# openai/robogym

Hardware: AMD Instinct MI355X
Metric: env-steps/sec (whole node) dactyl/locked batch 8192; qpos L∞ vs MuJoCo (as restated by the in-repo CPU oracle: parity unpinned) (higher is better)
Workload: dtype f32

## Files before the change

### include/rgstep.h

```cpp
#ifndef RGSTEP_H
#define RGSTEP_H
#include <stddef.h>
#include <stdint.h>

#ifdef __cplusplus
extern "C" {
#endif

typedef struct rg_model rg_model;
typedef struct rg_batch rg_batch;

enum {
  RG_F_QPOS = 0,
  RG_F_QVEL = 1,
  RG_F_CTRL = 2,
  RG_F_PID = 3,
  RG_F_WARMSTART = 4,
  RG_F_TIME = 5,
  RG_F_STATUS = 6,
  RG_F_STATS = 7,
  RG_F_DEBUG = 8,
  RG_F_COST = 9,
  RG_F_PAIRLB = 10,
  RG_F_ENVPRM = 11
// ... 58 lines not shown
  float* qpos_goal;
  int* preticks;
  float* reward;
  unsigned char *done, *goal_reset, *trial_success, *sub_goal_ok, *env_crash, *resetting, *episode_started;
  int* info_ssl;
  int *nticks_next, *reset_mask, *live_mask;
  float* goal_dist_before;
  float* packed;
  const float* draws;
  const float* goal_override;
  unsigned seed, step;
  const float* parallel_quats;
  const float* qpos0;
  const float* zero_ctrl;
  const float* ctrl_lo, *ctrl_hi;
  float success_threshold, success_reward, wiggle_std, cube_body_z;
  int max_timesteps_per_goal, successes_needed, use_goal_distance_reward;
  int pipelined, reset_initial_steps, n_random_initial_steps, max_pose_resets;
  int cube_pos_col, cube_quat_col;
  int stop_on_fall;
} rg_post_args;
int rg_env_post_step(rg_batch* b, const rg_post_args* args, void* stream);
int rg_post_args_size(void);
#define RG_WRAP_U_POOL 32
#define RG_WRAP_N_POOL 128
enum {
  RG_WK_CUBE_POS, RG_WK_CUBE_QUAT, RG_WK_QPOS, RG_WK_QVEL, RG_WK_HAND_ANGLE, RG_WK_FINGERTIP_POS, RG_WK_GOAL_POS, RG_WK_GOAL_QUAT, RG_WK_QPOS_GOAL,
  RG_WK_IS_GOAL_ACHIEVED, RG_WK_FELL_DOWN, RG_WK_ACTION_HISTORY, RG_WK_ACTION_DELAY, RG_WK_DELTA, RG_WK_NOISY_CUBE_POS, RG_WK_NOISY_CUBE_QUAT,
  RG_WK_NOISY_FINGERTIP_POS, RG_WK_NOISY_HAND_ANGLE, RG_WK_ACTION_EMA, RG_WK_ACH_POS, RG_WK_REL_POS, RG_WK_NACH_POS, RG_WK_NREL_POS, RG_WK_ACH_QUAT,
  RG_WK_REL_QUAT, RG_WK_NACH_QUAT, RG_WK_NREL_QUAT, RG_WK_RELATIVE_GOAL, RG_WK_NOISY_RELATIVE_GOAL, RG_WK_ACHIEVED_GOAL, RG_WK_NOISY_ACHIEVED_GOAL,
  RG_WK_GOAL, RG_WK_PREVIOUS_ACTION, RG_WK_REWARD, RG_WK_COUNT
};
typedef struct rg_wrap_dims {
  int nq, nv, nu, nh, ntip;
  int ndelta;
  int randomize, relative_goal;
} rg_wrap_dims;
typedef struct rg_wrap_lay {
  int fwidth, iwidth, W;
  int s_prev, s_ema, s_alpha, s_aema, s_hist, s_slack, s_cdown, s_cup, s_anmult, s_anadd, s_addb, s_mulb, s_ts, s_wind, s_occl, s_ffbuf, s_ffleft, s_cfleft, s_cfbuf, s_delta;
  int i_emat, i_steps, i_drops, i_first, i_delay;
  int n_action, n_wind, n_noise[4];
  int u_ts, u_wind, u_axis, u_ff, u_cf;
  int key[RG_WK_COUNT];
} rg_wrap_lay;
typedef struct rg_wrap_args {
  int B, device;
  rg_wrap_dims dims;
  rg_wrap_lay lay;
  float* fstate; int* istate;
  const float *u, *n, *e;
  const long long* action_index;
  const float* bins; int nbins;
  float* action_out;
  const float* qpos; int qpos_stride;
  const int* hand_q;
  const float* pos_to_ctrl;
  float* prm; int prm_stride;
  int p_ctrlrange, p_timestep, p_xfrc_cube, p_mass_cube;
  int relative_action, nsubsteps, fixed_wrist, wrist_act, wrist_qadr;
  float wrist_lo, wrist_hi;
  const float* obs; int obs_stride;
  const float *goal_pos, *goal_quat, *qpos_goal;
  const int* is_goal_achieved;
  const float* contact; int contact_stride, ncon_slots;
  const float* ncon; int ncon_stride;
  const float* env_reward;
  const unsigned char* env_done;
  const int* successes_so_far;
  float *out, *reward_out;
  unsigned char *done_out, *fell_out;
  int* info_out;
  float occ_geom[5]; int n_occ;
  float timestep0, cube_body_z, fall_z, occ_cutoff, ff_p, cf_p, freeze_scale, drop_reward, clip;
  int min_episode_length;
  float unc[4];
} rg_wrap_args;
int rg_wrap_layout(const rg_wrap_dims* dims, rg_wrap_lay* lay);
int rg_wrap_pre_step(const rg_wrap_args* args, void* stream);
int rg_wrap_post_step(const rg_wrap_args* args, void* stream);
int rg_wrap_args_size(void);
int rg_batch_set_constants(rg_batch* b, const int* mask_dev, void* stream);
int rg_batch_mpr_pair(rg_batch* b, int g1, int g2, float margin, float* out_dev, void* stream);
int rg_batch_items_info(const rg_batch* b, int* slots, int* queues);
int rg_obs_dim(const rg_batch* b);
int rg_debug_size(void);
int rg_lds_bytes(void);
int rg_lds_bytes_cfg(int config);
typedef struct rb_model rb_model;
typedef struct rb_batch rb_batch;
rb_model* rb_model_create(const void* blob, size_t nbytes, char* err, int errlen);
rb_model* rb_compile_mjcf(const char* xml, const char* meshdir, char* err, int errlen);
int rb_model_enable_env_params(rb_model* m);
int rb_prm_layout(const rb_model* m, int* out, int n);
int rb_model_blob_keys(const rb_model* m, char* out, int outlen);
void rb_model_free(rb_model* m);
int rb_model_info(const rb_model* m, int* out, int n);
int rb_scratch_offset(const rb_model* m, int which);
rb_batch* rb_batch_create(const rb_model* m, int B);
void rb_batch_free(rb_batch* b);
int rb_batch_reset(rb_batch* b);
int rb_batch_set_env(rb_batch* b, int hand_qposadr, int n_hand_jnt, int relative_action, const float* pos_to_ctrl);
int rb_batch_set_action_limits(rb_batch* b, float max_position_change, unsigned ctrl_centre_mask);
void* rb_batch_field_ptr(rb_batch* b, int field, int* row_words);
int rb_batch_step(rb_batch* b, const float* action_dev, const int* active_dev, int nsubsteps, int nforward_ticks, int flags, void* stream);
int rb_batch_step_ex(rb_batch* b, const float* action_dev, const int* active_dev, const int* hold_dev, const int* nticks_dev, int nsubsteps, int nforward_ticks, int flags, void* stream);
enum {
  RB_F_MOCAP = 12,
  RB_F_EQ_DATA = 13,
  RB_F_EQ_ACTIVE = 14,
  RB_F_SENSORDATA = 15
};
typedef struct rb_tcp_args {
  int arm_qposadr[6], main_arm_qposadr[6];
  int main_gripper_actuator, tcp_body, wrist_joint, reset_controller_error;
  float max_position_change, speed_roll, speed_pitch, joint_drift_threshold, gripper_ctrl_lo, gripper_ctrl_hi;
  const int* action_index; const float* bins; int nbins; float ema_alpha;
  float* ema_value; int* ema_t; float* action_out;
  const int* hold; const float* scripted;
  int wrist_only;
  int self_world, nforward_ticks;
  const int* nticks; const int* skip;
} rb_tcp_args;
int rb_batch_step_tcp(rb_batch* solver, rb_batch* main, const float* action_dev, const int* active_dev , const rb_tcp_args* args, int nsubsteps, int flags, void* stream);
int rb_tcp_args_size(void);
int rb_multi_begin(void);
int rb_multi_launch(void* stream);
#define RA_MAXOBJ 16
typedef struct ra_post_args {
  float* obs; int obs_dim;
  int num_objects;
  int *t, *steps, *steps_since_last_goal, *successes_so_far, *consecutive;
  float* prev_nsucc; int* prev_valid;
  const float* goal;
  const float* goal_rot;
  const float* qpos_goal;
  const float* static_obs;
  float* reward;
  float* goal_dist;
  unsigned char *done, *goal_reset, *trial_success, *sub_goal_ok, *env_crash, *objects_off_table;
  int* info_ssl;
  int obj_body[RA_MAXOBJ], tcp_body, arm_qposadr[6], grip_qposadr, grip_dofadr, grip_act, finger_geom[2], table_plane_geom, force_adr, torque_adr;
  unsigned long long gripper_geom_mask;
  float table_min[2], table_max[2], table_height, pos_threshold, rot_threshold, goal_pos_offset, goal_rot_weight, goal_reward_per_object, success_reward,
      penalty_table_collision, penalty_objects_off_table, penalty_safety_stop, safety_stop_force;
  int max_timesteps_per_goal, successes_needed, use_goal_distance_reward;
  float *solver_qpos, *solver_ctrl;
  int solver_nq, solver_nu, solver_grip_qposadr, solver_grip_act;
  const unsigned char* frozen;
  float reward_clip;
  int goal_kind;
  int grip_site;
  float* goal_dist_extra;
  const int* obj_group;
  const float *parallel_quats, *parallel_quats_180;
  int rot_dist_type;
} ra_post_args;
int ra_env_post_step(rb_batch* main, rb_batch* solver, const ra_post_args* args, void* stream);
int ra_post_args_size(void);
typedef struct ra_recipe_args {
  int num_objects, action_dim;
  int *stage, *left;
  float* yaw;
  const unsigned char *done, *goal_reset;
  int *hold, *hold_ctrl, *solver_active, *nticks;
  float* scripted;
// ... 75 lines not shown
```

### robogym_amd/_native.py

```python
import ctypes
import os

import numpy as np

_HERE = os.path.dirname(os.path.abspath(__file__))
LIB_PATH = os.environ.get("RGSTEP_LIB") or os.path.join(_HERE, "csrc", "librgstep.so")

RG_F_QPOS, RG_F_QVEL, RG_F_CTRL, RG_F_PID, RG_F_WARMSTART, RG_F_TIME, RG_F_STATUS, RG_F_STATS, RG_F_DEBUG, RG_F_COST, RG_F_PAIRLB, RG_F_ENVPRM = range(12)
RB_F_MOCAP, RB_F_EQ_DATA, RB_F_EQ_ACTIVE, RB_F_SENSORDATA = 12, 13, 14, 15
RG_STATUS_BAD_STATE, RG_STATUS_CON_FULL, RG_STATUS_CAND_FULL, RG_STATUS_ROW_FULL, RG_STATUS_BAD_FACTOR, RG_STATUS_BAD_ACTION = 1, 2, 4, 8, 16, 32


class StepArgs(ctypes.Structure):

    _fields_ = [("action_dev", ctypes.c_void_p), ("goal_quat_dev", ctypes.c_void_p), ("obs_dev", ctypes.c_void_p), ("goal_dist_dev", ctypes.c_void_p),
                ("active_dev", ctypes.c_void_p), ("hold_dev", ctypes.c_void_p), ("nticks_dev", ctypes.c_void_p), ("order_dev", ctypes.c_void_p),
                ("nsubsteps", ctypes.c_int), ("nforward_ticks", ctypes.c_int), ("flags", ctypes.c_int), ("stream", ctypes.c_void_p),
                ("config", ctypes.c_int), ("redo_dev", ctypes.c_void_p), ("preticks_dev", ctypes.c_void_p), ("xdata_dev", ctypes.c_void_p)]


RG_CFG_ROLLOUT, RG_CFG_LARGE = 0, 1
RG_POST_NDRAW = 2 + 4 + 3 + 20


# ... 50 lines not shown
def _ra_post_fields():
    _p, _i, _f = ctypes.c_void_p, ctypes.c_int, ctypes.c_float
    return ([("obs", _p), ("obs_dim", _i), ("num_objects", _i)]
            + [(n, _p) for n in ("t", "steps", "steps_since_last_goal", "successes_so_far", "consecutive", "prev_nsucc", "prev_valid", "goal", "goal_rot", "qpos_goal", "static_obs",
                                 "reward", "goal_dist", "done", "goal_reset", "trial_success", "sub_goal_ok", "env_crash", "objects_off_table", "info_ssl")]
            + [("obj_body", _i * RA_MAXOBJ), ("tcp_body", _i), ("arm_qposadr", _i * 6), ("grip_qposadr", _i), ("grip_dofadr", _i), ("grip_act", _i), ("finger_geom", _i * 2),
               ("table_plane_geom", _i), ("force_adr", _i), ("torque_adr", _i), ("gripper_geom_mask", ctypes.c_ulonglong), ("table_min", _f * 2), ("table_max", _f * 2)]
            + [(n, _f) for n in ("table_height", "pos_threshold", "rot_threshold", "goal_pos_offset", "goal_rot_weight", "goal_reward_per_object", "success_reward",
                                 "penalty_table_collision", "penalty_objects_off_table", "penalty_safety_stop", "safety_stop_force")]
            + [(n, _i) for n in ("max_timesteps_per_goal", "successes_needed", "use_goal_distance_reward")]
            + [("solver_qpos", _p), ("solver_ctrl", _p), ("solver_nq", _i), ("solver_nu", _i), ("solver_grip_qposadr", _i), ("solver_grip_act", _i), ("frozen", _p), ("reward_clip", _f)]
            + [("goal_kind", _i), ("grip_site", _i), ("goal_dist_extra", _p)]
            + [("obj_group", _p)]
            + [("parallel_quats", _p), ("parallel_quats_180", _p), ("rot_dist_type", _i)])


class RaPostArgs(ctypes.Structure):

    _fields_ = _ra_post_fields()


def _ra_recipe_fields():
    _p, _i, _f = ctypes.c_void_p, ctypes.c_int, ctypes.c_float
    return ([("num_objects", _i), ("action_dim", _i)]
            + [(n, _p) for n in ("stage", "left", "yaw", "done", "goal_reset", "hold", "hold_ctrl", "solver_active", "nticks", "scripted", "frozen", "resetting", "episode_started",
                                 "reobserve", "ended", "stabilised", "placement_failed", "t", "steps", "steps_since_last_goal", "successes_so_far", "consecutive", "prev_valid",
                                 "ema_t", "ema_value", "action_ema", "goal", "goal_rot", "qpos_goal", "static_obs")]
            + [("obj_qposadr", _i * RA_MAXOBJ), ("arm_qposadr", _i * 6), ("solver_arm_qposadr", _i * 6), ("arm_start", _f * 6), ("obj_center", (_f * 3) * RA_MAXOBJ),
               ("obj_half", (_f * 3) * RA_MAXOBJ), ("area_offset", _f * 2), ("area_size", _f * 2), ("table_pos", _f * 3), ("table_size", _f * 3), ("stabilize_steps", _i),
               ("n_random_initial_steps", _i), ("settle_steps", _i), ("seed", ctypes.c_uint), ("step", ctypes.c_uint)]
            + [("goal_kind", _i), ("height_range", _f * 2), ("object_size", _f), ("fixed_order", _i), ("target_height", _f), ("det_points", (_f * 3) * 2), ("goal_index", _p)]
            + [("obj_group", _p), ("group_mode", _i), ("sample_lam", _f * 2)]
            + [("goal_distance_ratio", _p), ("goal_distance_min", _f), ("pickup_proba", _f), ("stacking_proba", _f)]
            + [("randomize_goal_rot", _i), ("domino_distance_mul", _f)]
            + [("fixed_xy", (_f * 2) * RA_MAXOBJ), ("fixed_yaw", _f * RA_MAXOBJ)])


class RaRecipeArgs(ctypes.Structure):

    _fields_ = _ra_recipe_fields()


RG_WRAP_U_POOL, RG_WRAP_N_POOL = 32, 128
RG_WRAP_KEYS = ["cube_pos", "cube_quat", "qpos", "qvel", "hand_angle", "fingertip_pos", "goal_pos", "goal_quat", "qpos_goal", "is_goal_achieved", "fell_down", "action_history",
                "action_delay", "_delta", "noisy_cube_pos", "noisy_cube_quat", "noisy_fingertip_pos", "noisy_hand_angle", "action_ema", "achieved_goal_pos", "relative_goal_pos",
                "noisy_achieved_goal_pos", "noisy_relative_goal_pos", "achieved_goal_quat", "relative_goal_quat", "noisy_achieved_goal_quat", "noisy_relative_goal_quat",
                "relative_goal", "noisy_relative_goal", "achieved_goal", "noisy_achieved_goal", "goal", "previous_action", "reward"]


class WrapDims(ctypes.Structure):

    _fields_ = [(n, ctypes.c_int) for n in ("nq", "nv", "nu", "nh", "ntip", "ndelta", "randomize", "relative_goal")]


class WrapLay(ctypes.Structure):

    _fields_ = ([(n, ctypes.c_int) for n in ("fwidth", "iwidth", "W", "s_prev", "s_ema", "s_alpha", "s_aema", "s_hist", "s_slack", "s_cdown", "s_cup", "s_anmult", "s_anadd", "s_addb",
                                             "s_mulb", "s_ts", "s_wind", "s_occl", "s_ffbuf", "s_ffleft", "s_cfleft", "s_cfbuf", "s_delta", "i_emat", "i_steps", "i_drops", "i_first",
                                             "i_delay", "n_action", "n_wind")]
                + [("n_noise", ctypes.c_int * 4)] + [(n, ctypes.c_int) for n in ("u_ts", "u_wind", "u_axis", "u_ff", "u_cf")] + [("key", ctypes.c_int * len(RG_WRAP_KEYS))])


def _wrap_fields():
    p_, i_, f_ = ctypes.c_void_p, ctypes.c_int, ctypes.c_float
    return ([("B", i_), ("device", i_), ("dims", WrapDims), ("lay", WrapLay), ("fstate", p_), ("istate", p_), ("u", p_), ("n", p_), ("e", p_),
             ("action_index", p_), ("bins", p_), ("nbins", i_), ("action_out", p_), ("qpos", p_), ("qpos_stride", i_), ("hand_q", p_), ("pos_to_ctrl", p_),
             ("prm", p_), ("prm_stride", i_)]
            + [(n, i_) for n in ("p_ctrlrange", "p_timestep", "p_xfrc_cube", "p_mass_cube", "relative_action", "nsubsteps", "fixed_wrist", "wrist_act", "wrist_qadr")]
            + [("wrist_lo", f_), ("wrist_hi", f_), ("obs", p_), ("obs_stride", i_), ("goal_pos", p_), ("goal_quat", p_), ("qpos_goal", p_), ("is_goal_achieved", p_),
               ("contact", p_), ("contact_stride", i_), ("ncon_slots", i_), ("ncon", p_), ("ncon_stride", i_), ("env_reward", p_), ("env_done", p_), ("successes_so_far", p_),
               ("out", p_), ("reward_out", p_), ("done_out", p_), ("fell_out", p_), ("info_out", p_), ("occ_geom", f_ * 5), ("n_occ", i_)]
            + [(n, f_) for n in ("timestep0", "cube_body_z", "fall_z", "occ_cutoff", "ff_p", "cf_p", "freeze_scale", "drop_reward", "clip")]
            + [("min_episode_length", i_), ("unc", f_ * 4)])


class WrapArgs(ctypes.Structure):

    _fields_ = _wrap_fields()


EXPORTS = [
    "rg_model_create", "rg_model_free", "rg_model_dims", "rg_batch_create", "rg_batch_free", "rg_batch_set_env",
    "rg_batch_copy", "rg_batch_reset", "rg_batch_step", "rg_obs_dim", "rg_debug_size", "rg_lds_bytes", "rg_sync",
    "rg_last_error", "rg_batch_mpr_pair", "rg_batch_copy_rows", "rg_batch_step_ex", "rg_batch_field_ptr", "rg_model_create_on", "rg_model_npair",
    "rg_lds_bytes_cfg", "rg_env_post_step", "rg_post_args_size", "rg_batch_enable_env_params", "rg_prm_layout", "rg_xdata_layout", "rg_batch_set_constants", "rg_batch_items_info",
    "rb_model_create", "rb_model_free", "rb_model_info", "rb_scratch_offset", "rb_batch_create", "rb_batch_free", "rb_batch_reset", "rb_batch_set_env",
    "rb_batch_field_ptr", "rb_batch_step", "rb_batch_step_ex", "rb_env_post_step", "rb_post_args_size", "rb_cube_ops", "rb_batch_step_tcp", "ra_env_post_step", "ra_post_args_size",
    "rg_blob_entry", "rg_model_blob_keys", "rb_model_blob_keys", "rg_compile_mjcf", "rb_compile_mjcf", "rg_compile_mjcf_blob", "rg_blob_free",
    "rb_model_enable_env_params", "rb_prm_layout", "rb_batch_set_action_limits", "ra_env_recipe_step", "ra_recipe_args_size", "rb_tcp_args_size", "rb_multi_begin", "rb_multi_launch",
    "rg_wrap_layout", "rg_wrap_pre_step", "rg_wrap_post_step", "rg_wrap_args_size",
]
EXPORTS_SETCONST = ["rb_batch_set_constants"]



class NativeError(RuntimeError):
    pass


def bind(path):
    if not os.path.exists(path):
        raise NativeError(
            "%s not found: build it with `python -c 'import __graft_entry__ as g; g.build()'` "
            "(hipcc --offload-arch=gfx950). There is no CPU fallback." % path
        )
    L = ctypes.CDLL(path)
    vp, ci, cf = ctypes.c_void_p, ctypes.c_int, ctypes.c_float
    L.rg_model_create.restype = vp
    L.rg_model_create.argtypes = [ctypes.c_char_p, ctypes.c_size_t, ctypes.c_char_p, ci]
    L.rg_model_free.argtypes = [vp]
    L.rg_model_create_on.restype = vp
    L.rg_model_create_on.argtypes = [ctypes.c_char_p, ctypes.c_size_t, ci, ctypes.c_char_p, ci]
    L.rg_model_npair.argtypes = [vp]
    L.rg_batch_step_ex.argtypes = [vp, ctypes.POINTER(StepArgs)]
    L.rg_batch_field_ptr.restype = vp
    L.rg_batch_field_ptr.argtypes = [vp, ci, ctypes.POINTER(ci)]
    L.rg_model_dims.argtypes = [vp, ctypes.POINTER(ci)]
    L.rg_batch_create.restype = vp
    L.rg_batch_create.argtypes = [vp, ci, ci]
    L.rg_batch_free.argtypes = [vp]
    L.rg_batch_set_env.argtypes = [vp, ctypes.POINTER(ci), ci, ctypes.POINTER(cf), cf]
    L.rg_batch_copy.argtypes = [vp, ci, vp, ci, ci]
    L.rg_batch_reset.argtypes = [vp]
    L.rg_batch_copy_rows.argtypes = [vp, ci, vp, vp, ci, ci, vp]
    L.rg_batch_step.argtypes = [vp, vp, vp, vp, vp, vp, ci, ci, ci, vp]
    L.rg_batch_mpr_pair.argtypes = [vp, ci, ci, cf, vp, vp]
    L.rg_obs_dim.argtypes = [vp]
    L.rg_debug_size.restype = ci
    L.rg_lds_bytes.restype = ci
    L.rg_lds_bytes_cfg.restype = ci
    L.rg_lds_bytes_cfg.argtypes = [ci]
    L.rg_batch_enable_env_params.argtypes = [vp]
    L.rg_prm_layout.argtypes = [ctypes.POINTER(ci), ci]
    L.rg_xdata_layout.argtypes = [ctypes.POINTER(ci), ci]
    L.rg_env_post_step.argtypes = [vp, ctypes.POINTER(PostArgs), vp]
    L.rg_post_args_size.restype = ci
    if L.rg_post_args_size() != ctypes.sizeof(PostArgs):
        raise NativeError("rg_post_args layout mismatch between include/rgstep.h and robogym_amd/_native.py")
    L.rg_wrap_layout.argtypes = [ctypes.POINTER(WrapDims), ctypes.POINTER(WrapLay)]
    L.rg_wrap_pre_step.argtypes = [ctypes.POINTER(WrapArgs), vp]
    L.rg_wrap_post_step.argtypes = [ctypes.POINTER(WrapArgs), vp]
    L.rg_wrap_args_size.restype = ci
    if L.rg_wrap_args_size() != ctypes.sizeof(WrapArgs):
        raise NativeError("rg_wrap_args layout mismatch between include/rgstep.h and robogym_amd/_native.py")
    L.rg_batch_set_constants.argtypes = [vp, vp, vp]
    L.rg_batch_items_info.argtypes = [vp, ctypes.POINTER(ci), ctypes.POINTER(ci)]
    L.rb_model_create.restype = vp
    L.rb_model_create.argtypes = [ctypes.c_char_p, ctypes.c_size_t, ctypes.c_char_p, ci]
    L.rb_model_free.argtypes = [vp]
    L.rb_model_info.argtypes = [vp, ctypes.POINTER(ci), ci]
    L.rg_blob_entry.argtypes = [ctypes.c_char_p, ctypes.c_size_t, ci, ctypes.c_char_p, ctypes.POINTER(ci), ctypes.POINTER(ctypes.c_uint)]
    L.rg_model_blob_keys.argtypes = [vp, ctypes.c_char_p, ci]
    L.rb_model_blob_keys.argtypes = [vp, ctypes.c_char_p, ci]
    L.rg_compile_mjcf.restype = vp
    L.rg_compile_mjcf.argtypes = [ctypes.c_char_p, ctypes.c_char_p, ctypes.c_char_p, ci]
    L.rb_compile_mjcf.restype = vp
    L.rb_compile_mjcf.argtypes = [ctypes.c_char_p, ctypes.c_char_p, ctypes.c_char_p, ci]
    L.rg_compile_mjcf_blob.argtypes = [ctypes.c_char_p, ctypes.c_char_p, ci, ctypes.POINTER(vp), ctypes.POINTER(ctypes.c_size_t), ctypes.c_char_p, ci]
    L.rg_blob_free.argtypes = [vp]
    L.rb_model_enable_env_params.argtypes = [vp]
    L.rb_prm_layout.argtypes = [vp, ctypes.POINTER(ci), ci]
    L.rb_scratch_offset.argtypes = [vp, ci]
    L.rb_batch_create.restype = vp
    L.rb_batch_create.argtypes = [vp, ci]
    L.rb_batch_free.argtypes = [vp]
    L.rb_batch_reset.argtypes = [vp]
    L.rb_batch_set_env.argtypes = [vp, ci, ci, ci, ctypes.POINTER(cf)]
    L.rb_batch_set_action_limits.argtypes = [vp, cf, ctypes.c_uint]
    L.rb_batch_field_ptr.restype = vp
    L.rb_batch_field_ptr.argtypes = [vp, ci, ctypes.POINTER(ci)]
    L.rb_batch_step.argtypes = [vp, vp, vp, ci, ci, ci, vp]
    L.rb_batch_step_ex.argtypes = [vp, vp, vp, vp, vp, ci, ci, ci, vp]
    L.rb_batch_step_tcp.argtypes = [vp, vp, vp, vp, ctypes.POINTER(RbTcpArgs), ci, ci, vp]
    L.rb_multi_launch.argtypes = [vp]
    L.rb_batch_set_constants.argtypes = [vp, vp, vp]
    L.rb_tcp_args_size.restype = ci
    if L.rb_tcp_args_size() != ctypes.sizeof(RbTcpArgs):
        raise NativeError("rb_tcp_args layout mismatch between include/rgstep.h and robogym_amd/_native.py")
    L.ra_env_post_step.argtypes = [vp, vp, ctypes.POINTER(RaPostArgs), vp]
    L.ra_post_args_size.restype = ci
    if L.ra_post_args_size() != ctypes.sizeof(RaPostArgs):
        raise NativeError("ra_post_args layout mismatch between include/rgstep.h and robogym_amd/_native.py")
    L.ra_env_recipe_step.argtypes = [vp, vp, ctypes.POINTER(RaRecipeArgs), vp]
    L.ra_recipe_args_size.restype = ci
    if L.ra_recipe_args_size() != ctypes.sizeof(RaRecipeArgs):
        raise NativeError("ra_recipe_args layout mismatch between include/rgstep.h and robogym_amd/_native.py")
    L.rb_env_post_step.argtypes = [vp, ctypes.POINTER(RbPostArgs), vp]
    L.rb_post_args_size.restype = ci
    if L.rb_post_args_size() != ctypes.sizeof(RbPostArgs):
        raise NativeError("rb_post_args layout mismatch between include/rgstep.h and robogym_amd/_native.py")
    L.rb_cube_ops.argtypes = [vp, ci, vp, vp, ci, vp, vp]
    L.rg_sync.argtypes = [vp]
    L.rg_last_error.restype = ctypes.c_char_p
    return L


_LIB = None


def lib():
    global _LIB
    if _LIB is None:
        _LIB = bind(LIB_PATH)
    return _LIB


def check(L, rc, what):
    if rc != 0:
        raise NativeError("%s failed: %s" % (what, L.rg_last_error().decode()))


RG_FLAG_MPR_PLANE_DEPTH = 16
RG_FLAG_SENSORS = 32
RG_FLAG_SEPARATE_FORWARD_SUBSTITUTION = 64
RG_FLAG_SUBSTEP_ITEMS = 128
RG_FLAG_CAPACITY_TEST_HOOK = 512
RG_FLAG_DESERT_QUEUE0 = 1024
RG_STATUS_SCHED = 64
RG_FLAG_RESUME = 256

RB_PRM_NAMES = ["gravity", "dof_damping", "dof_armature", "dof_frictionloss", "dof_invweight0", "jnt_stiffness", "jnt_margin", "jnt_range", "body_pos", "body_mass", "body_inertia",
                "body_invweight0", "actuator_gainprm", "actuator_forcerange", "actuator_ctrlrange", "geom_pos", "geom_margin", "geom_gap", "geom_friction", "geom_solref", "geom_solimp",
                "tendon_range", "tendon_invweight0", "timestep", "xfrc_applied", "site_pos", "geom_scale"]
PRM_NAMES = ["row", "gravity", "timestep", "dof_damping", "dof_armature", "dof_frictionloss", "dof_invweight0", "body_mass", "body_inertia", "body_invweight0",
             "jnt_range", "tendon_range", "tendon_invweight0", "actuator_gainprm", "actuator_ctrlrange", "actuator_forcerange", "geom_friction", "xfrc_applied", "site_pos", "geom_scale", "jnt_margin", "geom_solref", "geom_solimp"]


def prm_layout(L):
    buf = (ctypes.c_int * 32)()
    n = L.rg_prm_layout(buf, 32)
    assert n == len(PRM_NAMES), "rg_prm_layout and robogym_amd/_native.py disagree"
    return {k: int(buf[i]) for i, k in enumerate(PRM_NAMES)}
```

### robogym_amd/csrc/rb_kernel.h

```cpp
#include "rb_types.h"
#if !defined(RB_NS) || !defined(RB_T) || !defined(RB_MAXGROUP) || !defined(RB_MAXNV) || !defined(RB_MAXNQ)
#error "rb_kernel.h: define RB_NS, RB_T, RB_MAXGROUP, RB_MAXNV, RB_MAXNQ before including"
#endif
#ifndef RB_MAXNU
#define RB_MAXNU 32
#endif

namespace RB_NS {
using namespace rgl;

#ifdef RG_EMUL
typedef const RbModelDev& RbM;
typedef const RbLaunch& RbLRef;
#define RB_S() (*(RbLds*)emul_lds())
#else
typedef const RG_AS4 RbModelDev& RbM;
typedef const RG_AS4 RbLaunch& RbLRef;
#define RB_S() (*(RbLds*)rg_lds_raw)
#endif
#define TID ((int)threadIdx.x)
#define WID (TID >> 6)
#define WL (TID & 63)
#define BFOR(i, n) for (int i = TID; i < (n); i += RB_T)
#define BSYNC() __syncthreads()
// ... 1152 lines not shown
  if (!m.prm_on) { for (int k = 0; k < 12; k++) out[k] = m.b_pair_prm[12 * p + k]; return; }
  const int a = m.b_pair_geom[3 * p], b = m.b_pair_geom[3 * p + 1];
  const float *gm = S + m.prm_off[RB_P_GEOM_MARGIN], *gg = S + m.prm_off[RB_P_GEOM_GAP], *gf = S + m.prm_off[RB_P_GEOM_FRICTION];
  const float *gr = S + m.prm_off[RB_P_GEOM_SOLREF], *gi = S + m.prm_off[RB_P_GEOM_SOLIMP];
  out[0] = fmaxf(gm[a], gm[b]); out[1] = fmaxf(gg[a], gg[b]);
  for (int k = 0; k < 3; k++) out[2 + k] = fmaxf(gf[3 * a + k], gf[3 * b + k]);
  const float m1 = m.geom_solmix[a], m2 = m.geom_solmix[b];
  const float mix = (m1 >= 1e-15f && m2 >= 1e-15f) ? m1 / (m1 + m2) : ((m1 < 1e-15f && m2 < 1e-15f) ? 0.5f : (m1 < 1e-15f ? 0.f : 1.f));
  if (gr[2 * a] > 0.f && gr[2 * b] > 0.f) { out[5] = mix * gr[2 * a] + (1.f - mix) * gr[2 * b]; out[6] = mix * gr[2 * a + 1] + (1.f - mix) * gr[2 * b + 1]; }
  else { out[5] = fminf(gr[2 * a], gr[2 * b]); out[6] = fminf(gr[2 * a + 1], gr[2 * b + 1]); }
  for (int k = 0; k < 5; k++) out[7 + k] = mix * gi[5 * a + k] + (1.f - mix) * gi[5 * b + k];
}
__device__ __forceinline__ void rb_broadphase(RbM m, RbLds& s, float* S, int flags) {
  int* cand = (int*)SC(CAND);
  const float *gpos = SC(GPOS), *gquat = SC(GQUAT);
  if (TID == 0) { s.ncand = 0; s.ncand2 = 0; s.ncon = s.neqcon; }
  BSYNC();
  const bool multipoint = !(flags & 16);
  const bool obb = !(flags & 2048);
  const int halfcand = m.maxcand >> 1;
  for (int base = 0; base < m.npair; base += RB_T) {
    const int p = base + TID;
    bool keep = false, special = false;
    if (p < m.npair) {
      const int g1 = m.b_pair_geom[3 * p], g2 = m.b_pair_geom[3 * p + 1], t1 = m.geom_type[g1];
      const float margin = rb_pair_margin(m, S, p);
      const v3 P1 = ld3(gpos + 3 * g1), P2 = ld3(gpos + 3 * g2), dif = P2 - P1;
      const float* bb = m.b_geom_aabb + 6 * g2;
      const float s1 = rb_geom_scale(m, s, g1), s2 = rb_geom_scale(m, s, g2);
      if (t1 == RG_GEOM_PLANE) {
        const v3 pn = qrot(ldq(gquat + 4 * g1), mk3(0, 0, 1));
        keep = dot(dif, pn) <= m.geom_rbound[g2] * s2 + margin;
        if (keep && obb) {
          const q4 q2 = ldq(gquat + 4 * g2);
          const v3 c2 = dif + qrot(q2, ld3(bb) * s2), nl = qrotT(q2, pn);
          keep = dot(c2, pn) - s2 * (bb[3] * fabsf(nl.x) + bb[4] * fabsf(nl.y) + bb[5] * fabsf(nl.z)) <= margin + 1e-5f;
        }
      } else {
        const float bound = m.geom_rbound[g1] * s1 + m.geom_rbound[g2] * s2 + margin;
        keep = dot(dif, dif) <= bound * bound;
        if (keep && obb) {
          const float* ba = m.b_geom_aabb + 6 * g1;
          const q4 q1 = ldq(gquat + 4 * g1), q2 = ldq(gquat + 4 * g2);
          keep = !rb_obb_apart(qrot(q1, ld3(ba) * s1), q1, ld3(ba + 3) * s1, dif + qrot(q2, ld3(bb) * s2), q2, ld3(bb + 3) * s2, margin);
        }
      }
      special = multipoint && m.geom_type[g2] == RG_GEOM_BOX && (t1 == RG_GEOM_BOX || t1 == RG_GEOM_PLANE);
    }
    const int slot = rb_slot(s, keep && !special, &s.ncand, halfcand, RG_STATUS_CAND_FULL);
    if (slot >= 0) cand[slot] = p;
    const int slot2 = rb_slot(s, keep && special, &s.ncand2, halfcand, RG_STATUS_CAND_FULL);
    if (slot2 >= 0) cand[m.maxcand - 1 - slot2] = p;
  }
  BSYNC();
}
__device__ __forceinline__ void rb_narrow_convex(RbM m, RbLds& s, float* S, int flags) {
  const int* cand = (const int*)SC(CAND);
  const float *gpos = SC(GPOS), *gquat = SC(GQUAT);
  const bool multipoint = !(flags & 16);
  (void)multipoint;
  MprEnv E; E.mesh_vert = m.b_mesh_rec; E.cell_adr = m.b_cell_adr; E.cell_blk = (const rgf4*)m.b_cell_blk; E.cell_ovf = (const rgf4*)m.b_cell_ovf; E.prof = 0; E.cells = !(flags & 8); E.plane_depth = (flags & 16) != 0;
  const int ncand = s.ncand;
  float* con = SC(CON);
  for (int base = 0; base < ncand; base += RB_T / 4) {
    const int ci = base + (TID >> 2);
    const bool active = ci < ncand;
    bool hit = false; float dist = 0; v3 pos = mk3(0, 0, 0), nrm = mk3(0, 0, 1); int p = 0;
    MprGeom A, B; A.type = RG_GEOM_SPHERE; B.type = RG_GEOM_SPHERE; A.quat = B.quat = gquat; A.size = B.size = mk3(0, 0, 0); A.pos = B.pos = mk3(0, 0, 0);
    A.margin = B.margin = 0; A.mesh = B.mesh = -1; A.vertadr = B.vertadr = 0; A.nvert = B.nvert = 0;
    float margin = 0;
    v3 p1 = mk3(0, 0, 0);
    bool plane = false; const bool special = false;
    if (active) {
      p = cand[ci];
      const int g1 = m.b_pair_geom[3 * p], g2 = m.b_pair_geom[3 * p + 1];
      margin = rb_pair_margin(m, S, p);
      rb_geom(m, s, S, g1, A); rb_geom(m, s, S, g2, B);
      p1 = ld3(gpos + 3 * g1);
      A.pos = mk3(0, 0, 0); B.pos = ld3(gpos + 3 * g2) - p1;
      plane = A.type == RG_GEOM_PLANE;
      A.margin = B.margin = plane ? 0.f : 0.5f * margin;
    }
    v3 sep, dir = mk3(0, 0, 0); float depth = 0;
    const bool mh = rg_mpr<4>(E, A, B, m.mpr_iterations, m.mpr_tolerance, depth, dir, pos, sep, active && !plane && !special);
    if (active && !plane && !special) {
      hit = mh && dot(dir, dir) > 0.25f;
      dist = margin - depth; nrm = normalized(dir); pos = pos + p1;
    }
    const v3 pn = qrot(ldq(A.quat), mk3(0, 0, 1));
    MprGeom Bs = B;
    if (!(active && plane && !special)) { Bs.type = RG_GEOM_SPHERE; Bs.mesh = -1; Bs.size = mk3(0, 0, 0); }
    const v3 sp = rg_support<4>(E, Bs, (active && plane && !special) ? pn * -1.0f : mk3(0, 0, 1));
    if (active && plane && !special) {
      dist = dot(sp, pn);
      hit = dist <= margin;
      pos = sp + p1 - pn * (0.5f * dist); nrm = pn;
    }
    const int slot = rb_slot(s, hit && (TID & 3) == 0, &s.ncon, m.maxcon, RG_STATUS_CON_FULL);
    if (slot >= 0) {
      float* c = con + RB_CONREC * slot;
      float pr[12]; rb_pair_prm(m, S, p, pr);
      c[RB_CR_DIST] = dist; st3(c + RB_CR_POS, pos);
      float fr[9]; fr[0] = nrm.x; fr[1] = nrm.y; fr[2] = nrm.z; rb_make_frame(fr);
      for (int k = 0; k < 9; k++) c[RB_CR_FRAME + k] = fr[k];
      c[RB_CR_INCL] = pr[0] - pr[1];
      c[RB_CR_FRIC] = pr[2]; c[RB_CR_FRIC + 1] = pr[2]; c[RB_CR_FRIC + 2] = pr[3]; c[RB_CR_FRIC + 3] = pr[4]; c[RB_CR_FRIC + 4] = pr[4];
      c[RB_CR_SOLREF] = pr[5]; c[RB_CR_SOLREF + 1] = pr[6];
      for (int k = 0; k < 5; k++) c[RB_CR_SOLIMP + k] = pr[7 + k];
      c[RB_CR_DIM] = (float)m.b_pair_geom[3 * p + 2]; c[RB_CR_G1] = (float)m.b_pair_geom[3 * p]; c[RB_CR_G2] = (float)m.b_pair_geom[3 * p + 1];
      c[RB_CR_ADR] = -1.f; c[RB_CR_NNZ] = 0.f; c[RB_CR_KIND] = (float)((m.cone == 1 && m.b_pair_geom[3 * p + 2] > 1) ? RB_KIND_ELLIPTIC : RB_KIND_PYRAMID);
    }
  }
  BSYNC();
}
__device__ __forceinline__ void rb_narrow_box(RbM m, RbLds& s, float* S, int flags) {
  const int* cand = (const int*)SC(CAND);
  const float *gpos = SC(GPOS), *gquat = SC(GQUAT);
  float* con = SC(CON);
  const bool multipoint = !(flags & 16);
  if (multipoint) {
    const int ncand2 = s.ncand2;
    for (int base = 0; base < ncand2; base += RB_T / 32) {
      const int ci = base + (TID >> 5), l = TID & 31;
      bool hit = false, planebox = false; float dist = 0; v3 pos = mk3(0, 0, 0), nrm = mk3(0, 0, 1); int p = 0;
      if (ci < ncand2) {
        p = cand[m.maxcand - 1 - ci];
        const int g1 = m.b_pair_geom[3 * p], g2 = m.b_pair_geom[3 * p + 1], t1 = m.geom_type[g1];
        if (m.geom_type[g2] == RG_GEOM_BOX && (t1 == RG_GEOM_BOX || t1 == RG_GEOM_PLANE)) {
          const float margin = rb_pair_margin(m, S, p);
          const v3 P1 = ld3(gpos + 3 * g1), t = ld3(gpos + 3 * g2) - P1;
          const float s2 = rb_geom_scale(m, s, g2);
          if (t1 == RG_GEOM_BOX) {
            const float s1 = rb_geom_scale(m, s, g1);
            const float A[3] = {m.geom_size[3 * g1] * s1, m.geom_size[3 * g1 + 1] * s1, m.geom_size[3 * g1 + 2] * s1}, B[3] = {m.geom_size[3 * g2] * s2, m.geom_size[3 * g2 + 1] * s2, m.geom_size[3 * g2 + 2] * s2};
            hit = box_box_lane(A, B, ldq(gquat + 4 * g1), ldq(gquat + 4 * g2), P1, t, margin, l, dist, pos, nrm);
          } else {
            nrm = qrot(ldq(gquat + 4 * g1), mk3(0, 0, 1));
            hit = rb_plane_box_lane(nrm, t, ldq(gquat + 4 * g2), ld3(m.geom_size + 3 * g2) * s2, margin, l, dist, pos);
            pos = pos + P1; planebox = true;
          }
        }
      }
      const unsigned long long balpb = __ballot(hit && planebox);
      if (hit && planebox && __popc((unsigned)((balpb >> (TID & 32)) & 0xffull) & ((1u << l) - 1u)) >= 4) hit = false;
      const int slot = rb_slot(s, hit, &s.ncon, m.maxcon, RG_STATUS_CON_FULL);
      if (slot >= 0) {
        float* c = con + RB_CONREC * slot;
        float pr[12]; rb_pair_prm(m, S, p, pr);
        c[RB_CR_DIST] = dist; st3(c + RB_CR_POS, pos);
        const v3 nn = normalized(nrm);
        float fr[9]; fr[0] = nn.x; fr[1] = nn.y; fr[2] = nn.z; rb_make_frame(fr);
        for (int k = 0; k < 9; k++) c[RB_CR_FRAME + k] = fr[k];
        c[RB_CR_INCL] = pr[0] - pr[1];
        c[RB_CR_FRIC] = pr[2]; c[RB_CR_FRIC + 1] = pr[2]; c[RB_CR_FRIC + 2] = pr[3]; c[RB_CR_FRIC + 3] = pr[4]; c[RB_CR_FRIC + 4] = pr[4];
        c[RB_CR_SOLREF] = pr[5]; c[RB_CR_SOLREF + 1] = pr[6];
        for (int k = 0; k < 5; k++) c[RB_CR_SOLIMP + k] = pr[7 + k];
        c[RB_CR_DIM] = (float)m.b_pair_geom[3 * p + 2]; c[RB_CR_G1] = (float)m.b_pair_geom[3 * p]; c[RB_CR_G2] = (float)m.b_pair_geom[3 * p + 1];
        c[RB_CR_ADR] = -1.f; c[RB_CR_NNZ] = 0.f; c[RB_CR_KIND] = (float)((m.cone == 1 && m.b_pair_geom[3 * p + 2] > 1) ? RB_KIND_ELLIPTIC : RB_KIND_PYRAMID);
      }
    }
  }
  BSYNC();
}

__device__ __forceinline__ float rb_impedance(const float* si, float pos, float margin) { return impedance(si, pos, margin); }
__device__ __forceinline__ void rb_KB(float timestep, const float* solref, const float* solimp, float& K, float& B) {
  const float dmax = clampf(solimp[1], 1e-4f, 0.9999f);
  if (solref[0] > 0) {
    const float tc = fmaxf(solref[0], 2.f * timestep), dr = solref[1];
    K = 1.f / fmaxf(RB_MINVAL, dmax * dmax * tc * tc * dr * dr); B = 2.f / fmaxf(RB_MINVAL, dmax * tc);
  } else { K = -solref[0] / fmaxf(RB_MINVAL, dmax * dmax); B = -solref[1] / fmaxf(RB_MINVAL, dmax); }
}
__device__ __forceinline__ int rb_npyr(int dim) { return dim == 1 ? 1 : 2 * (dim - 1); }
__device__ __forceinline__ int rb_nrows(int kind, int dim) { return kind == RB_KIND_PYRAMID ? rb_npyr(dim) : dim; }
__device__ __forceinline__ float rb_srow_dot(RbM m, const float* S, int type, int id, float aux, const float* x) {
// ... 1404 lines not shown
```

### robogym_amd/csrc/rb_types.h

```cpp
#pragma once
#include <stdint.h>

#define RB_T_LARGE 256
#define RB_MAXGROUP_LARGE 96
#define RB_MAXNV_LARGE 192
#define RB_MAXNQ_LARGE 192
#define RB_T_SMALL 64
#define RB_MAXGROUP_SMALL 40
#define RB_MAXNV_SMALL 40
#define RB_MAXNQ_SMALL 48
#define RB_T_MEDIUM 64
#define RB_MAXGROUP_MEDIUM 56
#define RB_MAXNV_MEDIUM 56
#define RB_MAXNQ_MEDIUM 64
#define RB_TENW 8
#define RB_CONW 24
#define RB_STARB 5
#define RB_MLONG 8
#define RB_NW 22

#define RB_INT_ARRAYS(X) \
  X(body_parentid) X(body_rootid) X(body_weldid) X(body_jntadr) X(body_jntnum) X(body_dofadr) X(body_dofnum) \
  X(jnt_type) X(jnt_qposadr) X(jnt_dofadr) X(jnt_bodyid) \
  X(dof_bodyid) X(dof_jntid) X(dof_parentid) \
  X(geom_type) X(geom_bodyid) X(geom_dataid) X(site_bodyid) \
  X(mesh_vertadr) X(mesh_vertnum) \
  X(tendon_adr) X(tendon_num) X(wrap_type) X(wrap_objid) \
  X(actuator_trntype) X(actuator_trnid) X(actuator_forcelimited) X(actuator_biastype) \
  X(body_mocapid) X(eq_type) X(eq_obj1id) X(eq_obj2id) X(sensor_type) X(sensor_objid) X(sensor_adr) \
  X(b_lvl_body) X(b_lvl_adr) X(b_body_level) X(b_body_lastdof) X(b_subtree_adr) X(b_subtree) X(b_root_list) X(b_M_i) X(b_M_j) X(b_M_adr) \
  X(b_group_adr) X(b_group_dofs) X(b_dof_group) X(b_dof_local) X(b_pair_geom) X(b_ten_dofs) X(b_fric_dof) X(b_fric_ten) X(b_lim_jnt) X(b_lim_ten) X(b_cell_adr) X(b_Mdesc_adr) X(b_Mdesc_ent) X(b_Mdesc_dof) X(b_dof_fricrow) X(b_star_grp) X(b_tree_adr) X(b_tree_desc) X(b_tree_branch) X(b_tree_brn_end) X(b_Mlong) X(b_tree8)
#define RB_FLT_ARRAYS(X) \
  X(body_pos) X(body_quat) X(body_ipos) X(body_iquat) X(body_mass) X(body_inertia) X(body_subtreemass) X(body_invweight0) \
  X(jnt_pos) X(jnt_axis) X(jnt_stiffness) X(jnt_range) X(jnt_margin) X(jnt_solref) X(jnt_solimp) \
  X(dof_armature) X(dof_damping) X(dof_frictionloss) X(dof_solref) X(dof_solimp) X(dof_invweight0) \
  X(qpos0) X(qpos_spring) \
  X(geom_size) X(geom_rbound) X(geom_pos) X(geom_quat) X(site_pos) \
  X(wrap_prm) X(tendon_range) X(tendon_margin) X(tendon_stiffness) X(tendon_damping) X(tendon_frictionloss) X(tendon_lengthspring) \
  X(tendon_solref_lim) X(tendon_solimp_lim) X(tendon_solref_fri) X(tendon_solimp_fri) X(tendon_invweight0) \
  X(actuator_gear) X(actuator_ctrlrange) X(actuator_forcerange) X(actuator_gainprm) X(actuator_user) \
  X(eq_solref) X(eq_solimp) X(site_quat) \
  X(geom_margin) X(geom_gap) X(geom_friction) X(geom_solref) X(geom_solimp) X(geom_solmix) X(opt_gravity) \
  X(b_pair_prm) X(b_geom_aabb) X(b_mesh_rec) X(b_cell_blk) X(b_cell_ovf)

enum {
  RB_O_XPOS, RB_O_XQUAT, RB_O_XIPOS, RB_O_XIQUAT, RB_O_XANCHOR, RB_O_XAXIS, RB_O_GPOS, RB_O_GQUAT, RB_O_SPOS, RB_O_ROOTCOM,
  RB_O_CINERT, RB_O_CRB, RB_O_CDOF, RB_O_CDOFDOT, RB_O_CVEL, RB_O_CACC, RB_O_CFRC,
  RB_O_TENLEN, RB_O_TENJ, RB_O_TENVEL, RB_O_MSP,
  RB_O_CAND, RB_O_CON, RB_O_CONJ, RB_O_CONIDX, RB_O_ROW, RB_O_DOFCON_ADR, RB_O_DOFCON, RB_O_CONF,
  RB_O_DBG, RB_O_CFRCEXT, RB_O_CONLOC, RB_O_PRM, RB_NOFF
};
enum {
  RB_P_GRAVITY, RB_P_DOF_DAMPING, RB_P_DOF_ARMATURE, RB_P_DOF_FRICTIONLOSS, RB_P_DOF_INVWEIGHT0, RB_P_JNT_STIFFNESS, RB_P_JNT_MARGIN, RB_P_JNT_RANGE,
  RB_P_BODY_POS, RB_P_BODY_MASS, RB_P_BODY_INERTIA, RB_P_BODY_INVWEIGHT0, RB_P_ACT_GAINPRM, RB_P_ACT_FORCERANGE, RB_P_ACT_CTRLRANGE,
  RB_P_GEOM_POS, RB_P_GEOM_MARGIN, RB_P_GEOM_GAP, RB_P_GEOM_FRICTION, RB_P_GEOM_SOLREF, RB_P_GEOM_SOLIMP, RB_P_TENDON_RANGE, RB_P_TENDON_INVWEIGHT0,
  RB_P_TIMESTEP, RB_P_XFRC, RB_P_SITE_POS, RB_P_GEOM_SCALE, RB_NPRMF
};
#define RB_CONREC 32
#define RB_CR_KIND 31
#define RB_KIND_PYRAMID 0
#define RB_KIND_ELLIPTIC 1
#define RB_KIND_EQUALITY 2
#define RB_CR_DIST 0
#define RB_CR_POS 1
#define RB_CR_FRAME 4
#define RB_CR_INCL 13
#define RB_CR_FRIC 14
#define RB_CR_SOLREF 19
#define RB_CR_SOLIMP 21
#define RB_CR_DIM 26
#define RB_CR_G1 27
#define RB_CR_G2 28
#define RB_CR_ADR 29
#define RB_CR_NNZ 30
#define RB_ROWREC 12
#define RB_RR_FORCE 8
#define RB_RR_ZONE 9
#define RB_RR_COST 10
#define RB_RR_D 0
#define RB_RR_AREF 1
#define RB_RR_JAR 2
#define RB_RR_JV 3
#define RB_RR_FLOSS 4
#define RB_RR_TYPE 5
#define RB_RR_ID 6
#define RB_RR_AUX 7

struct RbModelDev {
  int nq, nv, nu, nbody, njnt, ngeom, nsite, ntendon, nmesh;
  int nlevel, nM, npair, ngroup, gmax, nroot, conw;
  int nfric_dof, nfric_ten, nlim_jnt, nlim_ten;
  int maxcon, maxrow, maxcand;
  int iterations, mpr_iterations, ls_iterations;
  int cone, neq, nmocap, nsensor, nsensordata;
  float timestep, gravity[3], tolerance, impratio, mpr_tolerance, meaninertia;
  int off[RB_NOFF];
  int scratch_words;
  int prm_on;
  int prm_off[RB_NPRMF];
  int prm_words;
  const int* b_geom_scaled;
// ... 53 lines not shown
```

### robogym_amd/csrc/rg_api.hip

```cpp
#include "../../include/rgstep.h"
typedef rg_post_args RgPostArgs;
typedef rb_post_args RbPostArgs;
typedef ra_post_args RaPostArgs;
typedef ra_recipe_args RaRecipeArgs;
#define RG_NS rgs
#define RG_MAXCON 24
#define RG_CPOOL 768
#define RG_MAXCAND 128
#define RG_MAXCAND2 64
#include "rg_kernel.h"
#undef RG_NS
#undef RG_MAXCON
#undef RG_CPOOL
#undef RG_MAXCAND
#undef RG_MAXCAND2
#define RG_NS rgl
#define RG_SETCONST 1
#define RG_MAXCON 64
#define RG_CPOOL 2048
#define RG_MAXCAND 256
#define RG_MAXCAND2 128
#include "rg_kernel.h"
#undef RG_NS
#undef RG_MAXCON
// ... 287 lines not shown
    std::vector<float> rec((lb.size() ? lb.size() : 1) * RG_KINREC, 0.f);
    for (size_t k = 0; k < lb.size(); k++) {
      int b = lb[k], j = jn[b] > 0 ? ja[b] : 0, t = jn[b] > 0 ? jt[j] : 0, qa = jn[b] > 0 ? jq[j] : 0;
      float* r = rec.data() + k * RG_KINREC;
      int w0 = b | (par[b] << 8) | (jn[b] << 16) | (t << 20), w1 = j | (qa << 16);
      memcpy(r, &w0, 4); memcpy(r + 1, &w1, 4);
      for (int c = 0; c < 3; c++) { r[2 + c] = bp[3 * b + c]; r[9 + c] = bi[3 * b + c]; r[12 + c] = jn[b] > 0 ? jp[3 * j + c] : 0.f; r[15 + c] = jn[b] > 0 ? jx[3 * j + c] : 0.f; }
      for (int c = 0; c < 4; c++) r[5 + c] = bq[4 * b + c];
      r[18] = jn[b] > 0 ? q0[qa] : 0.f;
    }
    {
      static_assert(RG_MAXDEPTH <= 8 && RG_MAXBODY <= 256, "body chain: 8 bytes per body");
      std::vector<int> slot(d.nbody, -1), depth(d.nbody, 0), chainw((size_t)(d.nbody ? d.nbody : 1) * 2, 0);
      for (size_t k = 0; k < lb.size(); k++) if (lb[k] >= 0 && lb[k] < d.nbody) slot[lb[k]] = (int)k;
      std::vector<float> brec((size_t)(d.nbody ? d.nbody : 1) * RG_KINREC, 0.f);
      for (int b0 = 0; b0 < d.nbody; b0++) {
        if (slot[b0] < 0) continue;
        memcpy(brec.data() + (size_t)b0 * RG_KINREC, rec.data() + (size_t)slot[b0] * RG_KINREC, RG_KINREC * 4);
        int chain[RG_MAXDEPTH + 1], n = 0, a0 = b0;
        for (; a0 > 0 && slot[a0] >= 0; a0 = par[a0]) { if (n >= RG_MAXDEPTH) return bail("kinematic chain deeper than RG_MAXDEPTH", m); chain[n++] = a0; }
        unsigned long long cw = 0; int absmask = 0;
        for (int i = 0; i < n; i++) {
          int a = chain[n - 1 - i];
          cw |= (unsigned long long)(a & 255) << (8 * i);
          for (int jj = 0; jj < jn[a]; jj++) if (jt[ja[a] + jj] == RG_JNT_FREE) absmask |= 1 << i;
        }
        depth[b0] = n | (absmask << 8) | ((a0 & 255) << 16);
        chainw[2 * b0] = (int)(unsigned)(cw & 0xFFFFFFFFull); chainw[2 * b0 + 1] = (int)(unsigned)(cw >> 32);
      }
      if (!upload<float>(m, brec, &d.body_rec) || !upload<int>(m, depth, &d.body_depth) || !upload<int>(m, chainw, &d.body_chain)) return bail("hipMalloc failed", m);
    }
    {
      std::vector<int> os, rid, rob; std::vector<float> roc;
      if (!get_i(B, "k_body_orgslot", os, e) || !get_i(B, "body_rootid", rid, e) || !get_i(B, "k_root_origin_body", rob, e) || !get_f(B, "k_root_origin_const", roc, e)) return bail(e, m);
      std::vector<float> orec(16, 0.f);
      for (int sl = 0; sl < 4; sl++) { int unused = -2; memcpy(&orec[4 * sl], &unused, 4); }
      for (int b0 = 0; b0 < d.nbody; b0++) {
        int sl = os[b0], r = rid[b0], ob = rob[r];
        if (sl < 0 || sl > 3) return bail("com-frame slot out of range", m);
        memcpy(&orec[4 * sl], &ob, 4);
        for (int c = 0; c < 3; c++) orec[4 * sl + 1 + c] = ob >= 0 ? bi[3 * ob + c] : roc[3 * r + c];
      }
      if (!upload<float>(m, orec, &d.org_rec)) return bail("hipMalloc failed", m);
    }
  }
  UPI(lvl_dof, "k_lvl_dof"); UPI(lvl_dof_adr, "k_lvl_dof_adr"); UPI(M_i, "k_M_i"); UPI(M_j, "k_M_j"); { std::vector<int> mi0, mj0, db0; if (!get_i(B, "k_M_i", mi0, e) || !get_i(B, "k_M_j", mj0, e) || !get_i(B, "dof_bodyid", db0, e)) return bail(e, m); std::vector<int> w(mi0.size() ? mi0.size() : 1, 0); for (size_t q = 0; q < mi0.size(); q++) w[q] = mi0[q] | (mj0[q] << 8) | (db0[mi0[q]] << 16); if (!upload<int>(m, w, &d.M_ijb)) return bail("hipMalloc failed", m); }    UPI(M_lvl_adr, "k_M_lvl_adr");
  UPI(desc_adr, "k_desc_adr"); UPI(desc, "k_desc");
  {
    std::vector<int> mi, mj, blk, d2c;
    if (!get_i(B, "k_M_i", mi, e) || !get_i(B, "k_M_j", mj, e) || !get_i(B, "k_dof_blk", blk, e) || !get_i(B, "k_d2c", d2c, e)) return bail(e, m);
    if ((int)mi.size() > RG_MAXNM || mi.size() != mj.size()) return bail("inertia matrix has more non-zeros than RG_MAXNM", m);
    std::vector<int> ent(2 * (mi.size() ? mi.size() : 1), 0);
    for (size_t k = 0; k < mi.size(); k++) {
      int i = mi[k], j = mj[k], s0 = (blk[i] >> 16) & 255;
      int aij = (blk[i] & 0xFFFF) + (j - s0), aji = (blk[j] & 0xFFFF) + (i - s0);
      if (aij >= RG_HWORDS || aji >= RG_HWORDS || aij < 0 || aji < 0) return bail("inertia block layout exceeds RG_HWORDS", m);
      ent[2 * k] = aij | (aji << 16);
      ent[2 * k + 1] = (d2c[i] >= 0 && d2c[j] >= 0) ? (d2c[i] | (d2c[j] << 8) | (1 << 16)) : 0;
    }
    if (!upload<int>(m, ent, &d.M_ent)) return bail("hipMalloc failed", m);
  }
  UPI(geom_type, "geom_type"); UPI(geom_bodyid, "geom_bodyid"); UPI(geom_dataid, "geom_dataid"); UPI(body_geomadr, "body_geomadr"); UPI(body_geomnum, "body_geomnum");
  UPF(geom_size, "geom_size"); UPF(geom_rbound, "geom_rbound"); UPF(geom_pos, "geom_pos"); UPF(geom_quat, "geom_quat"); UPF(geom_aabb, "k_geom_aabb");
  UPI(site_bodyid, "site_bodyid"); UPF(site_pos, "site_pos");
  UPI(site_type, "site_type"); UPF(site_size, "site_size"); UPF(site_quat, "site_quat");
  { std::vector<int> st, so, sty;
    if (!get_i(B, "sensor_type", st, e) || !get_i(B, "sensor_objid", so, e) || !get_i(B, "site_type", sty, e)) return bail(e, m);
    if (st.size() > RG_MAXSENSOR) return bail("more than RG_MAXSENSOR sensors", m);
    for (size_t k = 0; k < st.size(); k++) {
      if (st[k] != 0) return bail("only touch sensors are implemented", m);
      int t = sty[so[k]];
      if (t != RG_GEOM_SPHERE && t != RG_GEOM_CAPSULE && t != RG_GEOM_ELLIPSOID && t != RG_GEOM_CYLINDER && t != RG_GEOM_BOX) return bail("touch sensor on a site of unsupported shape", m);
    }
    d.nsensor = (int)st.size();
    if (so.empty()) so.push_back(0);
    if (!upload<int>(m, so, &d.sensor_site)) return bail("hipMalloc failed", m); }
  UPI(mesh_vertadr, "mesh_vertadr"); UPI(mesh_vertnum, "mesh_vertnum");
  { GF("mesh_vert"); std::vector<float> v4(fv.size() / 3 * 4, 0.f);
    for (size_t i = 0; i < fv.size() / 3; i++) { v4[4 * i] = fv[3 * i]; v4[4 * i + 1] = fv[3 * i + 1]; v4[4 * i + 2] = fv[3 * i + 2]; }
    if (!upload<float>(m, v4, &d.mesh_vert)) return bail("hipMalloc failed", m);
    std::vector<int> vadr, cadr, vidx;
    if (!get_i(B, "mesh_vertadr", vadr, e) || !get_i(B, "k_mesh_cell_adr", cadr, e) || !get_i(B, "k_mesh_cell_vidx", vidx, e)) return bail(e, m);
    if (cadr.size() != (size_t)d.nmesh * RG_NCELL) return bail("k_mesh_cell_adr has the wrong size (RG_CELLN mismatch?)", m);
    std::vector<float> blk((size_t)d.nmesh * RG_NCELL * 16, 0.f), ovf(4, 0.f);
    for (int mi = 0; mi < d.nmesh; mi++) for (int c = 0; c < RG_NCELL; c++) {
      size_t ce = (size_t)mi * RG_NCELL + c;
      int e = cadr[ce], start = e >> 8, cnt = e & 255;
      if (cnt < 1 || (size_t)(start + cnt) > vidx.size()) return bail("bad support cell", m);
      cadr[ce] = (int)((ovf.size() / 4) << 8) | cnt;
      for (int k = 0; k < (cnt > 4 ? cnt : 4); k++) {
        int vi = vidx[start + (k < cnt ? k : cnt - 1)]; size_t src = (size_t)(vadr[mi] + vi);
        if (vi < 0 || src * 3 + 2 >= fv.size()) return bail("bad support cell vertex", m);
        float o[4] = {fv[3 * src], fv[3 * src + 1], fv[3 * src + 2], 0.f}; memcpy(o + 3, &vi, 4);
        if (k < 4) memcpy(blk.data() + ce * 16 + 4 * k, o, 16); else ovf.insert(ovf.end(), o, o + 4);
      }
    }
    if (!upload<int>(m, cadr, &d.mesh_cell_adr) || !upload<float>(m, blk, &d.mesh_cell_blk) || !upload<float>(m, ovf, &d.mesh_cell_ovf)) return bail("hipMalloc failed", m); }
  UPI(pair_geom, "k_pair_geom"); UPF(pair_prm, "k_pair_prm"); UPF(pair_mix, "k_pair_mix");
  {
    std::vector<int> pg, gt, gd, va, vn, gb, bdm; std::vector<float> pp, gs, gr, ga;
    if (!get_i(B, "geom_bodyid", gb, e) || !get_i(B, "k_body_dofmask", bdm, e)) return bail(e, m);
    if (!get_i(B, "k_pair_geom", pg, e) || !get_i(B, "geom_type", gt, e) || !get_i(B, "geom_dataid", gd, e) || !get_i(B, "mesh_vertadr", va, e) || !get_i(B, "mesh_vertnum", vn, e) ||
        !get_f(B, "k_pair_prm", pp, e) || !get_f(B, "geom_size", gs, e) || !get_f(B, "geom_rbound", gr, e) || !get_f(B, "k_geom_aabb", ga, e)) return bail(e, m);
    std::vector<int> gsc;
    if (B.find("k_geom_scaled") && !get_i(B, "k_geom_scaled", gsc, e)) return bail(e, m);
    for (size_t g = 0; g < gsc.size(); g++) if (gsc[g] && (g >= gt.size() || gt[g] != RG_GEOM_BOX)) return bail("k_geom_scaled flags a geom that is not a box", m);
    size_t np = pg.size() / 3;
    std::vector<int> gg(np ? np : 1, 0); std::vector<float> rec((np ? np : 1) * RG_PAIRREC, 0.f);
    for (size_t p = 0; p < np; p++) {
      int g[2] = {pg[3 * p], pg[3 * p + 1]};
      if (g[0] < 0 || g[1] < 0 || g[0] > 255 || g[1] > 255 || g[0] >= d.ngeom || g[1] >= d.ngeom) return bail("pair geom id out of range", m);
      gg[p] = g[0] | (g[1] << 8);
      float* r = rec.data() + p * RG_PAIRREC;
      int hdr = g[0] | (g[1] << 8) | (pg[3 * p + 2] << 16) | (gt[g[0]] << 20) | (gt[g[1]] << 24);
      if ((size_t)g[0] < gsc.size() && gsc[g[0]]) hdr |= RG_PAIR_SCALED1;
      if ((size_t)g[1] < gsc.size() && gsc[g[1]]) hdr |= RG_PAIR_SCALED2;
      memcpy(r, &hdr, 4); r[1] = pp[12 * p];
      for (int k = 0; k < 2; k++) {
        int id = gt[g[k]] == RG_GEOM_MESH ? gd[g[k]] : -1, nvert = id >= 0 ? vn[id] : 0, vadr0 = id >= 0 ? va[id] : 0;
        memcpy(r + 2 + k, &id, 4);
        for (int c = 0; c < 3; c++) { r[4 + 4 * k + c] = gs[3 * g[k] + c]; r[16 + 4 * k + c] = ga[3 * g[k] + c]; }
        memcpy(r + 7 + 4 * k, &nvert, 4); memcpy(r + 12 + k, &vadr0, 4);
        r[14 + k] = gr[g[k]];
      }
      int b1 = gb[g[0]], b2 = gb[g[1]], bb = b1 | (b2 << 8), lo = bdm[2 * b1] | bdm[2 * b2], hi = bdm[2 * b1 + 1] | bdm[2 * b2 + 1];
      if (b1 > 255 || b2 > 255) return bail("pair body id out of range", m);
      memcpy(r + 19, &bb, 4); memcpy(r + 23, &lo, 4); memcpy(r + 24, &hi, 4);
    }
    if (!upload<int>(m, gg, &d.pair_gg) || !upload<float>(m, rec, &d.pair_rec)) return bail("hipMalloc failed", m);
  }
  UPI(tendon_adr, "tendon_adr"); UPI(tendon_num, "tendon_num"); UPI(wrap_type, "wrap_type"); UPI(wrap_objid, "wrap_objid"); UPI(ten_dofs, "k_ten_dofs");
  UPI(ten_path, "k_ten_path"); UPI(ten_path_adr, "k_ten_path_adr");
  UPF(wrap_prm, "wrap_prm"); UPF(tendon_range, "tendon_range"); UPF(tendon_margin, "tendon_margin"); UPF(tendon_stiffness, "tendon_stiffness");
  UPF(tendon_damping, "tendon_damping"); UPF(tendon_frictionloss, "tendon_frictionloss"); UPF(tendon_lengthspring, "tendon_lengthspring");
  UPF(tendon_solref_lim, "tendon_solref_lim"); UPF(tendon_solimp_lim, "tendon_solimp_lim"); UPF(tendon_solref_fri, "tendon_solref_fri");
  UPF(tendon_solimp_fri, "tendon_solimp_fri"); UPF(tendon_invweight0, "tendon_invweight0");
  UPI(dof_ten_adr, "k_dof_ten_adr"); UPI(dof_ten, "k_dof_ten"); UPI(dof_act_adr, "k_dof_act_adr"); UPI(dof_act, "k_dof_act");
  {
    std::vector<int> db, dj, jt, jq, ta, aa; std::vector<float> js, qs;
    if (!get_i(B, "dof_bodyid", db, e) || !get_i(B, "dof_jntid", dj, e) || !get_i(B, "jnt_type", jt, e) || !get_i(B, "jnt_qposadr", jq, e) ||
        !get_i(B, "k_dof_ten_adr", ta, e) || !get_i(B, "k_dof_act_adr", aa, e) || !get_f(B, "jnt_stiffness", js, e) || !get_f(B, "qpos_spring", qs, e)) return bail(e, m);
    std::vector<float> drec((size_t)(d.nv ? d.nv : 1) * 8, 0.f);
    for (int i = 0; i < d.nv; i++) {
      int j = dj[i], t = jt[j], qa = jq[j];
      if (ta[i + 1] > 255 || aa[i + 1] > 255 || db[i] > 255) return bail("dof record: table index out of range", m);
      int w0 = db[i] | (ta[i] << 8) | (ta[i + 1] << 16), w1 = aa[i] | (aa[i + 1] << 8);
      float* r = drec.data() + 8 * (size_t)i;
      memcpy(r, &w0, 4); memcpy(r + 1, &w1, 4);
      r[2] = (t == RG_JNT_HINGE || t == RG_JNT_SLIDE) ? js[j] : 0.f;
      memcpy(r + 3, &qa, 4); r[4] = qs[qa];
    }
    if (!upload<float>(m, drec, &d.dof_rec)) return bail("hipMalloc failed", m);
  }
  UPI(actuator_trntype, "actuator_trntype"); UPI(actuator_trnid, "actuator_trnid"); UPI(actuator_ctrllimited, "actuator_ctrllimited");
  UPI(actuator_forcelimited, "actuator_forcelimited"); UPI(actuator_biastype, "actuator_biastype");
  UPF(actuator_gear, "actuator_gear"); UPF(actuator_ctrlrange, "actuator_ctrlrange"); UPF(actuator_forcerange, "actuator_forcerange");
  UPF(actuator_gainprm, "actuator_gainprm"); UPF(actuator_biasprm, "actuator_biasprm");
  GI("k_fric_dof"); d.nfric_dof = (int)iv.size(); if (!upload<int>(m, iv, &d.fric_dof)) return bail("hipMalloc failed", m);
  GI("k_fric_ten"); d.nfric_ten = (int)iv.size(); if (!upload<int>(m, iv, &d.fric_ten)) return bail("hipMalloc failed", m);
  GI("k_lim_jnt"); d.nlim_jnt = (int)iv.size(); if (!upload<int>(m, iv, &d.lim_jnt)) return bail("hipMalloc failed", m);
  GI("k_lim_ten"); d.nlim_ten = (int)iv.size(); if (!upload<int>(m, iv, &d.lim_ten)) return bail("hipMalloc failed", m);
  if (d.nfric_dof + d.nfric_ten + 2 * d.nlim_jnt + 2 * d.nlim_ten > RG_MAXSROW || d.nfric_dof + d.nfric_ten > RG_MAXFRIC) return bail("too many friction/limit rows for RG_MAXSROW / RG_MAXFRIC", m);
  {
    std::vector<int> fd, ft, lj, lt, d2c, jq, jd; std::vector<float> tfl, jm, tm, dsr, dsi, tsrf, tsif, jsr, jsi, tsrl, tsil;
    if (!get_i(B, "k_fric_dof", fd, e) || !get_i(B, "k_fric_ten", ft, e) || !get_i(B, "k_lim_jnt", lj, e) || !get_i(B, "k_lim_ten", lt, e) || !get_i(B, "k_d2c", d2c, e) ||
        !get_i(B, "jnt_qposadr", jq, e) || !get_i(B, "jnt_dofadr", jd, e) || !get_f(B, "tendon_frictionloss", tfl, e) || !get_f(B, "jnt_margin", jm, e) || !get_f(B, "tendon_margin", tm, e) ||
        !get_f(B, "dof_solref", dsr, e) || !get_f(B, "dof_solimp", dsi, e) || !get_f(B, "tendon_solref_fri", tsrf, e) || !get_f(B, "tendon_solimp_fri", tsif, e) ||
        !get_f(B, "jnt_solref", jsr, e) || !get_f(B, "jnt_solimp", jsi, e) || !get_f(B, "tendon_solref_lim", tsrl, e) || !get_f(B, "tendon_solimp_lim", tsil, e)) return bail(e, m);
    const int ns = d.nfric_dof + d.nfric_ten + 2 * d.nlim_jnt + 2 * d.nlim_ten;
    std::vector<float> srec((size_t)(ns ? ns : 1) * 16, 0.f);
    for (int r = 0; r < ns; r++) {
      float* o = srec.data() + 16 * (size_t)r;
      int rr = r, kind, dof = 0, ten = 31, neg = 0, src = 0, odiag, ofl = -1, olim = 0, omargin = -1; float cfl = 0.f, margin = 0.f; const float *sr, *si;
      if (rr < d.nfric_dof) { int q = fd[rr]; kind = 0; dof = d2c[q]; ofl = RG_PRM_DOF_FRICTIONLOSS + q; odiag = RG_PRM_DOF_INVWEIGHT0 + q; sr = &dsr[2 * q]; si = &dsi[5 * q]; }
      else if ((rr -= d.nfric_dof) < d.nfric_ten) { int t = ft[rr]; kind = 1; ten = t; cfl = tfl[t]; odiag = RG_PRM_TENDON_INVWEIGHT0 + t; sr = &tsrf[2 * t]; si = &tsif[5 * t]; }
      else if ((rr -= d.nfric_ten) < 2 * d.nlim_jnt) { int j = lj[rr >> 1]; kind = 2; dof = d2c[jd[j]]; neg = rr & 1; src = jq[j]; olim = RG_PRM_JNT_RANGE + 2 * j + (rr & 1); margin = 0.f; omargin = RG_PRM_JNT_MARGIN + j; (void)jm; odiag = RG_PRM_DOF_INVWEIGHT0 + jd[j]; sr = &jsr[2 * j]; si = &jsi[5 * j]; }
      else { rr -= 2 * d.nlim_jnt; int t = lt[rr >> 1]; kind = 3; ten = t; neg = rr & 1; src = t; olim = RG_PRM_TENDON_RANGE + 2 * t + (rr & 1); margin = tm[t]; odiag = RG_PRM_TENDON_INVWEIGHT0 + t; sr = &tsrl[2 * t]; si = &tsil[5 * t]; }
// ... 214 lines not shown
  return p;
}
int rg_batch_copy(rg_batch* b, int field, void* ptr, int to_batch, int ptr_is_device) {
  if (!b || !ptr) return fail("rg_batch_copy: null argument");
  DeviceGuard g(b->device);
  const RgModelDev& d = b->model->dev;
  RgBatchDev& s = b->dev;
  size_t n = 0; void* p = field_ptr(b, field, &n);
  if (!p) return fail("rg_batch_copy: unknown field");
  size_t bytes = n * 4 * (size_t)s.B;
  HIPCHK(hipDeviceSynchronize());
  if (to_batch) {
    HIPCHK(hipMemcpy(p, ptr, bytes, ptr_is_device ? hipMemcpyDeviceToDevice : hipMemcpyHostToDevice));
    if (field == RG_F_QPOS) HIPCHK(hipMemset(s.pairlb, 0, (size_t)s.B * (d.npair > 0 ? d.npair : 1) * 4));
  }
  else HIPCHK(hipMemcpy(ptr, p, bytes, ptr_is_device ? hipMemcpyDeviceToDevice : hipMemcpyDeviceToHost));
  return 0;
}

int rg_batch_copy_rows(rg_batch* b, int field, const void* src_dev, const int* mask_dev, int col0, int ncols, void* stream) {
  if (!b || !src_dev || !mask_dev) return fail("rg_batch_copy_rows: null argument");
  DeviceGuard g(b->device);
  const RgModelDev& d = b->model->dev;
  RgBatchDev& s = b->dev;
  const bool rowwise = field == RG_F_QPOS || field == RG_F_QVEL || field == RG_F_CTRL || field == RG_F_PID || field == RG_F_WARMSTART || field == RG_F_TIME || field == RG_F_STATUS;
  size_t words = 0; void* p = rowwise ? field_ptr(b, field, &words) : nullptr;
  if (!p) return fail("rg_batch_copy_rows: field cannot be written row-wise");
  const int n = (int)words;
  if (ncols <= 0) { col0 = 0; ncols = n; }
  if (col0 < 0 || col0 + ncols > n) return fail("rg_batch_copy_rows: column range outside the row");
  float* lb = field == RG_F_QPOS ? s.pairlb : nullptr;
  return launch(rgs::rg_copy_rows_kernel, s.B, RG_WAVE, 0, 0, stream, (float*)p, (const float*)src_dev, mask_dev, n, col0, ncols, lb, d.npair);
}

int rg_batch_items_info(const rg_batch* b, int* slots, int* queues) {
  if (!b) return fail("null batch");
  if (slots) *slots = b->items_slots;
  if (queues) *queues = b->items_queues;
  return 0;
}

int rg_batch_step_ex(rg_batch* b, const rg_step_args* a) {
  if (!b || !a) return fail("null argument");
  if ((a->action_dev || a->obs_dev) && !b->has_env) return fail("rg_batch_set_env must be called before stepping with actions/observations");
  if (a->nsubsteps < 0 || a->nforward_ticks < 0) return fail("rg_batch_step: negative step counts");
  DeviceGuard g(b->device);
  RgBatchDev bt = b->dev;
  bt.action = a->action_dev; bt.goal_quat = a->goal_quat_dev; bt.obs = a->obs_dev; bt.goal_dist = a->goal_dist_dev; bt.active = a->active_dev;
  bt.hold = a->hold_dev; bt.nticks = a->nticks_dev; bt.order = a->order_dev;
  const bool sens = (a->flags & 32) != 0 && a->xdata_dev && b->model->dev.nsensor > 0;
  const bool large = a->config == RG_CFG_LARGE || sens, prof = (a->flags & 2) != 0;
  if (a->config != RG_CFG_LARGE && a->config != RG_CFG_ROLLOUT) return fail("rg_batch_step: unknown kernel configuration");
  bt.redo = large ? nullptr : a->redo_dev;
  bt.preticks = a->preticks_dev;
  bt.xdata = a->xdata_dev;
  const bool items = (a->flags & 128) && !large && !(a->flags & (1 | 2 | 256)) && a->nsubsteps >= 2 && b->items_slots > 0;
  RgLaunch launch_args{b->model->aux, b->env, bt, a->nsubsteps, a->nforward_ticks, a->flags, items ? b->items_queues : 1};
  if (items) {
    const long long nitems = (long long)bt.B * a->nsubsteps;
    const int grid = (int)(nitems < b->items_slots ? nitems : b->items_slots);
    const size_t ldsi = rgi::rg_lds_launch_bytes(false);
    HIPCHK(hipMemsetAsync(bt.sched, 0, ((size_t)RG_SCHED_PROG + bt.B) * 4, (hipStream_t)a->stream));
    return launch(rgi::rg_step_items_kernel, grid, RG_WAVE, ldsi, 0, a->stream, b->model->dev_copy, launch_args);
  }
  const size_t lds = sens ? rgx::rg_lds_launch_bytes(prof) : (large ? rgl::rg_lds_launch_bytes(prof) : rgs::rg_lds_launch_bytes(prof));
  return launch(sens ? rgx::rg_step_kernel : large ? rgl::rg_step_kernel : rgs::rg_step_kernel, bt.B, RG_WAVE, lds, 0, a->stream, b->model->dev_copy, launch_args);
}
int rg_batch_step(rg_batch* b, const float* action_dev, const float* goal_quat_dev, float* obs_dev, float* goal_dist_dev,
                  const int* active_dev, int nsubsteps, int nforward_ticks, int flags, void* stream) {
  rg_step_args a;
  memset(&a, 0, sizeof a);
  a.action_dev = action_dev; a.goal_quat_dev = goal_quat_dev; a.obs_dev = obs_dev; a.goal_dist_dev = goal_dist_dev; a.active_dev = active_dev;
  a.nsubsteps = nsubsteps; a.nforward_ticks = nforward_ticks; a.flags = flags; a.stream = stream;
  return rg_batch_step_ex(b, &a);
}

int rg_batch_mpr_pair(rg_batch* b, int g1, int g2, float margin, float* out_dev, void* stream) {
  if (!b || !out_dev) return fail("null argument");
  const RgModelDev& d = b->model->dev;
  if (g1 < 0 || g2 < 0 || g1 >= d.ngeom || g2 >= d.ngeom) return fail("geom id out of range");
  DeviceGuard g(b->device);
  RgLaunch launch_args{b->model->aux, b->env, b->dev, 0, 0, 0, 1};
  return launch(rgs::rg_mpr_pair_kernel, b->dev.B, RG_WAVE, sizeof(rgs::RgLds), 0, stream, b->model->dev_copy, launch_args, g1, g2, margin, out_dev);
}

int rg_post_args_size(void) { return (int)sizeof(rg_post_args); }
int rg_env_post_step(rg_batch* b, const rg_post_args* args, void* stream) {
  if (!b || !args) return fail("null argument");
  if (!b->has_env) return fail("rg_batch_set_env must be called first");
  const rg_post_args& a = *args;
  if (!a.goal_dist || !a.obs || !a.t || !a.phase || !a.tries || !a.steps || !a.steps_since_last_goal || !a.successes_so_far || !a.goals_so_far || !a.consecutive ||
      !a.prev_dist || !a.prev_valid || !a.is_successful || !a.goal_quat || !a.qpos_goal || !a.preticks || !a.reward || !a.done || !a.goal_reset || !a.trial_success ||
      !a.sub_goal_ok || !a.env_crash || !a.resetting || !a.episode_started || !a.info_ssl || !a.nticks_next || !a.reset_mask || !a.live_mask || !a.goal_dist_before || !a.parallel_quats || !a.qpos0 || !a.zero_ctrl ||
      !a.ctrl_lo || !a.ctrl_hi) return fail("rg_env_post_step: a required array is NULL");
  const RgModelDev& d = b->model->dev;
  if (d.nu > 20) return fail("rg_env_post_step: nu exceeds RG_POST_NDRAW's action slots");
  DeviceGuard g(b->device);
  return launch(rg_post_step_kernel, b->dev.B, RG_WAVE, 0, sizeof(RgPostFlags), stream, b->dev, a, d.nq, d.nv, d.nu, d.npair);
}

int rg_wrap_args_size(void) { return (int)sizeof(rg_wrap_args); }
int rg_wrap_layout(const rg_wrap_dims* dims, rg_wrap_lay* lay) {
  if (!dims || !lay) return fail("rg_wrap_layout: null argument");
  const rg_wrap_dims& d = *dims;
  if (d.nq < 0 || d.nv < 0 || d.nu < 1 || d.nh < 0 || d.ntip < 0 || d.ndelta < 0) return fail("rg_wrap_layout: negative width");
  const int rnd = d.randomize != 0, rel = d.relative_goal != 0, nb = 4 + d.ntip + d.nh;
  rg_wrap_lay& L = *lay;
  int at = 0;
  const struct { int* off; int n; } fstate[] = {
    {&L.s_prev, d.nu}, {&L.s_ema, d.nu}, {&L.s_alpha, 1}, {&L.s_aema, d.nu}, {&L.s_hist, d.nu}, {&L.s_slack, d.nu}, {&L.s_cdown, d.nu}, {&L.s_cup, d.nu},
    {&L.s_anmult, d.nu}, {&L.s_anadd, d.nu}, {&L.s_addb, nb}, {&L.s_mulb, nb}, {&L.s_ts, 5}, {&L.s_wind, 1}, {&L.s_occl, d.ntip}, {&L.s_ffbuf, d.ntip},
    {&L.s_ffleft, 5}, {&L.s_cfleft, 1}, {&L.s_cfbuf, 17}, {&L.s_delta, d.ndelta}};
  for (const auto& f : fstate) { *f.off = at; at += f.n; }
  L.fwidth = at;
  at = 0;
  const struct { int* off; int n; } istate[] = {{&L.i_emat, 1}, {&L.i_steps, 1}, {&L.i_drops, 1}, {&L.i_first, 1}, {&L.i_delay, d.nu}};
  for (const auto& f : istate) { *f.off = at; at += f.n; }
  L.iwidth = at;
  at = 0;
  if (rnd) { L.n_action = at; at += d.nu; L.n_wind = at; at += 3; } else { L.n_action = L.n_wind = -1; }
  const int nw[4] = {3, 1, d.ntip, d.nh};
  for (int k = 0; k < 4; k++) { L.n_noise[k] = at; at += nw[k]; }
  if (at > RG_WRAP_N_POOL) return fail("rg_wrap_layout: the step's normal draws exceed RG_WRAP_N_POOL");
  at = 0;
  if (rnd) { L.u_ts = at; at += 2; L.u_wind = at; at += 1; } else { L.u_ts = L.u_wind = -1; }
  L.u_axis = at; at += 3;
  if (rnd) { L.u_ff = at; at += 10; L.u_cf = at; at += 2; } else { L.u_ff = L.u_cf = -1; }
  const struct { int key, n, on; } keys[] = {
    {RG_WK_CUBE_POS, 3, 1}, {RG_WK_CUBE_QUAT, 4, 1}, {RG_WK_QPOS, d.nq, 1}, {RG_WK_QVEL, d.nv, 1}, {RG_WK_HAND_ANGLE, 2 * d.nh, 1}, {RG_WK_FINGERTIP_POS, d.ntip, 1},
    {RG_WK_GOAL_POS, 3, 1}, {RG_WK_GOAL_QUAT, 4, 1}, {RG_WK_QPOS_GOAL, d.nq, 1}, {RG_WK_IS_GOAL_ACHIEVED, 1, 1}, {RG_WK_FELL_DOWN, 1, 1},
    {RG_WK_ACTION_HISTORY, d.nu, rnd}, {RG_WK_ACTION_DELAY, d.nu, rnd}, {RG_WK_DELTA, d.ndelta, rnd},
    {RG_WK_NOISY_CUBE_POS, 3, 1}, {RG_WK_NOISY_CUBE_QUAT, 4, 1}, {RG_WK_NOISY_FINGERTIP_POS, d.ntip, 1}, {RG_WK_NOISY_HAND_ANGLE, 2 * d.nh, 1}, {RG_WK_ACTION_EMA, d.nu, 1},
    {RG_WK_ACH_POS, 3, rel}, {RG_WK_REL_POS, 3, rel}, {RG_WK_NACH_POS, 3, rel}, {RG_WK_NREL_POS, 3, rel}, {RG_WK_ACH_QUAT, 4, rel}, {RG_WK_REL_QUAT, 4, rel},
    {RG_WK_NACH_QUAT, 4, rel}, {RG_WK_NREL_QUAT, 4, rel}, {RG_WK_RELATIVE_GOAL, 7, rel}, {RG_WK_NOISY_RELATIVE_GOAL, 7, rel}, {RG_WK_ACHIEVED_GOAL, 7, rel},
    {RG_WK_NOISY_ACHIEVED_GOAL, 7, rel}, {RG_WK_GOAL, 7, 1}, {RG_WK_PREVIOUS_ACTION, d.nu, 1}, {RG_WK_REWARD, 2, 1}};
  static_assert(sizeof keys / sizeof keys[0] == RG_WK_COUNT, "one table entry per key");
  at = 0;
  for (const auto& k : keys) { L.key[k.key] = k.on ? at : -1; at += k.on ? k.n : 0; }
  L.W = at;
  return 0;
}
static int rg_wrap_check(const rg_wrap_args* args, bool post) {
  if (!args) return fail("rg_wrap: null argument");
  const rg_wrap_args& a = *args;
  rg_wrap_lay want;
  if (rg_wrap_layout(&a.dims, &want) != 0) return -1;
  if (memcmp(&want, &a.lay, sizeof want) != 0) return fail("rg_wrap: args.lay is not rg_wrap_layout(args.dims)");
  if (a.B < 1 || !a.fstate || !a.istate || !a.n || !a.u) return fail("rg_wrap: B, the state rows and the draw blocks u, n are required");
  const int rnd = a.dims.randomize != 0;
  if (rnd && (!a.prm || !a.qpos || !a.hand_q || !a.pos_to_ctrl)) return fail("rg_wrap: randomize needs prm, qpos, hand_q and pos_to_ctrl");
  if (!post) {
    if (!a.action_index || !a.bins || a.nbins < 1 || !a.action_out) return fail("rg_wrap_pre_step: action_index, bins and action_out are required");
    if (a.fixed_wrist && (!a.qpos || a.wrist_act < 0 || a.wrist_act >= a.dims.nu)) return fail("rg_wrap_pre_step: fixed_wrist needs qpos and a wrist actuator below nu");
    return 0;
  }
  if (!a.obs || !a.goal_quat || !a.qpos_goal || !a.is_goal_achieved || !a.env_reward || !a.env_done || !a.successes_so_far || !a.out || !a.reward_out || !a.done_out ||
      !a.fell_out || !a.info_out) return fail("rg_wrap_post_step: a required array is NULL");
  if (a.obs_stride < 7 + a.dims.nq + a.dims.nv + a.dims.nh + a.dims.ntip) return fail("rg_wrap_post_step: obs_stride is shorter than the observation row of dims");
  if (rnd && a.n_occ > 0 && (a.n_occ > 5 || !a.contact || !a.ncon || a.ncon_slots < 0 || a.contact_stride < 3 * a.ncon_slots)) return fail("rg_wrap_post_step: the occlusion check needs contact, ncon and at most 5 geoms");
  return 0;
}
int rg_wrap_pre_step(const rg_wrap_args* args, void* stream) {
  if (rg_wrap_check(args, false) != 0) return -1;
  DeviceGuard g(args->device);
  return launch(rg_wrap_pre_kernel, args->B, RG_WAVE, 0, 0, stream, *args);
}
// ... 655 lines not shown
```

### robogym_amd/csrc/rg_kernel.h

```cpp
#ifndef RG_KERNEL_COMMON_H
#define RG_KERNEL_COMMON_H
#include "rg_types.h"

#ifdef RG_EMUL
#include "hip_emul.h"
#else
#include <hip/hip_runtime.h>
#endif

#ifdef RG_EMUL
typedef const RgModelDev& RgM;
#else
typedef const __attribute__((address_space(4))) RgModelDev& RgM;
#endif
#ifdef RG_FINE_PROF
#define RG_NPROF 56
#else
#define RG_NPROF 24
#endif
struct RgAux {
  const int *subtree_adr, *subtree;
  const uint32_t* dof_velmask;
};

struct RgLaunch { RgAux x; RgEnvDev env; RgBatchDev bt; int nsubsteps, nforward_ticks, flags, nqueues; };

struct RgCtx { const void* km; const void* kl; };
#ifdef RG_EMUL
#define RG_M(c) (*(const RgModelDev*)(c).km)
#define RG_L(c) (*(const RgLaunch*)(c).kl)
#define RG_S() (*(RgLds*)emul_lds())
#define RG_STAGE static inline
typedef const RgLaunch& RgLRef;
#else
extern __shared__ __attribute__((aligned(16))) unsigned char rg_lds_raw[];
#define RG_AS4 __attribute__((address_space(4)))
__device__ __forceinline__ unsigned long long rg_uniform(const void* p) {
  unsigned long long v = (unsigned long long)p;
  unsigned int lo = __builtin_amdgcn_readfirstlane((unsigned int)v), hi = __builtin_amdgcn_readfirstlane((unsigned int)(v >> 32));
  return ((unsigned long long)hi << 32) | lo;
}
#define RG_M(c) (*(const RG_AS4 RgModelDev*)rg_uniform((c).km))
#define RG_L(c) (*(const RG_AS4 RgLaunch*)rg_uniform((c).kl))
#define RG_S() (*(RgLds*)rg_lds_raw)
#define RG_STAGE __device__ __attribute__((noinline))
typedef const RG_AS4 RgLaunch& RgLRef;
#endif
#ifdef RG_EMUL
#define RG_STAGE_BIG static inline
#else
#define RG_STAGE_BIG __device__ __forceinline__
#endif
#ifdef RG_EMUL
static inline int rg_env_blk(RgLRef L) { return L.bt.order ? L.bt.order[blockIdx.x] : (int)blockIdx.x; }
#else
__device__ __forceinline__ int rg_env_blk(RgLRef L) { return L.bt.order ? __builtin_amdgcn_readfirstlane(L.bt.order[blockIdx.x]) : (int)blockIdx.x; }
#endif
struct alignas(16) rgf4 { float x, y, z, w; };
struct v3 { float x, y, z; };
__device__ __forceinline__ v3 mk3(float x, float y, float z) { v3 r; r.x = x; r.y = y; r.z = z; return r; }
__device__ __forceinline__ v3 ld3(const float* p) { return mk3(p[0], p[1], p[2]); }
__device__ __forceinline__ void st3(float* p, v3 a) { p[0] = a.x; p[1] = a.y; p[2] = a.z; }
__device__ __forceinline__ v3 operator+(v3 a, v3 b) { return mk3(a.x + b.x, a.y + b.y, a.z + b.z); }
__device__ __forceinline__ v3 operator-(v3 a, v3 b) { return mk3(a.x - b.x, a.y - b.y, a.z - b.z); }
__device__ __forceinline__ v3 operator*(v3 a, float s) { return mk3(a.x * s, a.y * s, a.z * s); }
__device__ __forceinline__ float dot(v3 a, v3 b) { return a.x * b.x + a.y * b.y + a.z * b.z; }
__device__ __forceinline__ v3 cross(v3 a, v3 b) { return mk3(a.y * b.z - a.z * b.y, a.z * b.x - a.x * b.z, a.x * b.y - a.y * b.x); }
#ifdef RG_EMUL
static inline float rg_rsqrt(float x) { return 1.0f / sqrtf(x); }
static inline float rg_rcp(float x) { return 1.0f / x; }
static inline float rg_sqrt(float x) { return sqrtf(x); }
#else
__device__ __forceinline__ float rg_rsqrt(float x) { return __builtin_amdgcn_rsqf(x); }
__device__ __forceinline__ float rg_rcp(float x) { return __builtin_amdgcn_rcpf(x); }
__device__ __forceinline__ float rg_sqrt(float x) { return __builtin_amdgcn_sqrtf(x); }
#endif
__device__ __forceinline__ float norm(v3 a) { return sqrtf(dot(a, a)); }
__device__ __forceinline__ v3 normalized(v3 a) { float n2 = dot(a, a); return n2 < 1e-37f ? mk3(1, 0, 0) : a * rg_rsqrt(n2); }
__device__ __forceinline__ v3 mulm(const float* M, v3 v) { return mk3(M[0] * v.x + M[1] * v.y + M[2] * v.z, M[3] * v.x + M[4] * v.y + M[5] * v.z, M[6] * v.x + M[7] * v.y + M[8] * v.z); }
__device__ __forceinline__ v3 mulmT(const float* M, v3 v) { return mk3(M[0] * v.x + M[3] * v.y + M[6] * v.z, M[1] * v.x + M[4] * v.y + M[7] * v.z, M[2] * v.x + M[5] * v.y + M[8] * v.z); }
struct q4 { float w, x, y, z; };
__device__ __forceinline__ q4 ldq(const float* p) { q4 q; q.w = p[0]; q.x = p[1]; q.y = p[2]; q.z = p[3]; return q; }
__device__ __forceinline__ void stq(float* p, q4 q) { p[0] = q.w; p[1] = q.x; p[2] = q.y; p[3] = q.z; }
__device__ __forceinline__ q4 qmul(q4 a, q4 b) {
  q4 r;
  r.w = a.w * b.w - a.x * b.x - a.y * b.y - a.z * b.z;
  r.x = a.w * b.x + a.x * b.w + a.y * b.z - a.z * b.y;
  r.y = a.w * b.y - a.x * b.z + a.y * b.w + a.z * b.x;
  r.z = a.w * b.z + a.x * b.y - a.y * b.x + a.z * b.w;
  return r;
}
__device__ __forceinline__ q4 qnormalize(q4 q) {
  float n = sqrtf(q.w * q.w + q.x * q.x + q.y * q.y + q.z * q.z);
  if (n < 1e-30f) { q.w = 1; q.x = q.y = q.z = 0; return q; }
  float s = rg_rcp(n); q.w *= s; q.x *= s; q.y *= s; q.z *= s; return q;
}
__device__ __forceinline__ void q2mat(float* m, q4 q) {
  float w = q.w, x = q.x, y = q.y, z = q.z;
  m[0] = w * w + x * x - y * y - z * z; m[1] = 2 * (x * y - w * z); m[2] = 2 * (x * z + w * y);
// ... 138 lines not shown
  r[5] = i[7] * v[0] - i[6] * v[1] + i[9] * v[5];
}
__device__ __forceinline__ void cross_motion(float* r, const float* vel, const float* v) {
  v3 w = ld3(vel), vt = ld3(vel + 3), a = ld3(v), b = ld3(v + 3);
  st3(r, cross(w, a)); st3(r + 3, cross(w, b) + cross(vt, a));
}
__device__ __forceinline__ void cross_force(float* r, const float* vel, const float* f) {
  v3 w = ld3(vel), vt = ld3(vel + 3), a = ld3(f), b = ld3(f + 3);
  st3(r, cross(w, a) + cross(vt, b)); st3(r + 3, cross(w, b));
}

#if defined(RG_WOODBURY_CHECK) && defined(RG_EMUL)
static float rg_wchk_max = 0.f; static int rg_wchk_n = 0, rg_wchk_rows = 0;
#endif
#endif

#if !defined(RG_NS) || !defined(RG_MAXCON) || !defined(RG_CPOOL) || !defined(RG_MAXCAND) || !defined(RG_MAXCAND2)
#error "define RG_NS, RG_MAXCON, RG_CPOOL, RG_MAXCAND, RG_MAXCAND2 before including rg_kernel.h"
#endif
#ifndef RG_ITEMS
#define RG_ITEMS 0
#endif
#undef RG_ROW_LD
#undef RG_ROW_ST
#if RG_ITEMS
#define RG_ROW_LD(p) rg_ld_sc1(p)
#else
#define RG_ROW_LD(p) (*(p))
#endif
#undef RG_SEPDIR_ST
#define RG_ROW_ST(p, v) (*(p) = (v))
#define RG_SEPDIR_ST(p, cd) (*(p) = (cd))
#ifndef RG_SETCONST
#define RG_SETCONST 0
#endif
#ifndef RG_SENSORS
#define RG_SENSORS 0
#endif
namespace RG_NS {
#define RG_MAXPYR (RG_MAXCON * 6)
#define RG_PSLOTS ((RG_MAXPYR + RG_WAVE - 1) / RG_WAVE)

struct RgLds {
  alignas(16) float qpos[RG_MAXNQ], qvel[RG_MAXNV], ctrl[RG_MAXU];
  float org[4 * 3];
  float Msp[RG_MAXNM];
  float tenlen[RG_MAXTEN], tenJ[RG_MAXTEN * 4];
  float actlen[RG_MAXU], actfrc[RG_MAXU];
  float qfrc_smooth[RG_MAXNV], qacc_smooth[RG_MAXNV];
  unsigned char ten_cdof[RG_MAXTEN * 4], c2d[RG_MAXNVC], b2org[RG_MAXBODY];
  int cblk[RG_MAXNVC];
  int ncand, ncand2, ncon;
  float c_D[RG_MAXCON], c_mu[RG_MAXCON * 2];
  short c_pair[RG_MAXCON], c_off[RG_MAXCON];
  unsigned char c_dim[RG_MAXCON], c_nnz[RG_MAXCON];
#if RG_SENSORS
  unsigned char c_touch[RG_MAXCON];
#endif
  unsigned char c_idx[RG_MAXCON * RG_W];
  float c_pool[RG_CPOOL];
  float c_aref0[RG_MAXCON], c_kb[RG_MAXCON];
  unsigned int status;
  int has_xfrc;
#if RG_ITEMS
  int cur_env;
#endif
  union {
    struct {
      union {
        struct { alignas(16) float xquat[RG_MAXBODY * 4]; float xpos[RG_MAXBODY * 3], xanchor[RG_MAXJNT * 3], xaxis[RG_MAXJNT * 3], spos[RG_MAXSITE * 3]; };
        struct { float crb[RG_MAXBODY * 10]; };
        struct { float cdofdot[RG_MAXNV * 6], cacc[RG_MAXBODY * 6], tenfrc[RG_MAXTEN], tenvel[RG_MAXTEN], qfrc_passive[RG_MAXNV], qfrc_bias[RG_MAXNV], qfrc_act[RG_MAXNV]; };
      };
      alignas(16) float gquat[RG_MAXGEOM * 4]; float gpos[RG_MAXGEOM * 3];
      float cdof[RG_MAXNV * 6];
      float gspeed[RG_MAXGEOM];
      union {
        float cinert[RG_MAXBODY * 10];
        struct {
          short cand[RG_MAXCAND], cand2[RG_MAXCAND2];
          union {
            short tlist[RG_TLIST];
            struct { float c_dist[RG_MAXCON], c_pos[RG_MAXCON * 3], c_normal[RG_MAXCON * 3]; };
          };
        };
      };
    };
    struct {
      alignas(16) float H[RG_HWORDS];
      float a[RG_MAXNVC], jtf[RG_MAXNVC], Ma[RG_MAXNVC];
      union { struct { float as[RG_MAXNVC], fs[RG_MAXNVC]; }; float qfrc_con[RG_MAXNV]; };
      union { struct { float search[RG_MAXNVC], Mv[RG_MAXNVC]; }; float qacc[RG_MAXNV]; };
      float dinv[RG_MAXNV], tmpv[RG_MAXNV];
      unsigned char p_quad[RG_MAXPYR];
      float c_bdot[RG_MAXCON * 4];
    };
  };
  float prof[RG_NPROF];
};
static inline size_t rg_lds_launch_bytes(bool profiling) { return profiling ? sizeof(RgLds) : offsetof(RgLds, prof); }

#ifdef RG_EMUL
#if RG_ITEMS
static inline int rg_env(RgLRef L) { return RG_S().cur_env; }
#else
static inline int rg_env(RgLRef L) { return rg_env_blk(L); }
#endif
static inline const float* rg_prm(const RgModelDev& m, RgLRef L) { return L.bt.envprm ? L.bt.envprm + (size_t)rg_env(L) * RG_NPRM : m.prm_default; }
#else
#if RG_ITEMS
__device__ __forceinline__ int rg_env(RgLRef L) { return __builtin_amdgcn_readfirstlane(RG_S().cur_env); }
#else
__device__ __forceinline__ int rg_env(RgLRef L) { return rg_env_blk(L); }
#endif
__device__ __forceinline__ const float* rg_prm(const RG_AS4 RgModelDev& m, RgLRef L) { return L.bt.envprm ? L.bt.envprm + (size_t)rg_env(L) * RG_NPRM : m.prm_default; }
#endif
__device__ __forceinline__ v3 rg_xipos(RgM m, const RgLds& s, int b) { return ld3(s.xpos + 3 * b) + qrot(ldq(s.xquat + 4 * b), ld3(m.body_ipos + 3 * b)); }
__device__ __forceinline__ void rg_kinematics(RgM m, RgLds& s, const float* P) {
  float* lp = s.gpos; float* lq = s.gquat;
  PFOR(b, m.nbody) {
    if ((m.body_depth[b] & 255) == 0) {
      st3(s.xpos + 3 * b, ld3(m.static_xpos + 3 * b)); stq(s.xquat + 4 * b, ldq(m.static_xquat + 4 * b));
      continue;
    }
    const rgf4* R = (const rgf4*)m.body_rec + (RG_KINREC / 4) * b;
    rgf4 r0 = R[0], r1 = R[1], r2 = R[2], r3 = R[3], r4 = R[4];
    int w0 = __builtin_bit_cast(int, r0.x), w1 = __builtin_bit_cast(int, r0.y);
    int jn = (w0 >> 16) & 15, ja = w1 & 0xFFFF;
    v3 pos = mk3(r0.z, r0.w, r1.x);
    q4 quat; quat.w = r1.y; quat.x = r1.z; quat.y = r1.w; quat.z = r2.x;
    for (int jj = 0; jj < jn; jj++) {
      int j = ja + jj, t, qa; v3 jpos, jaxis; float q0;
      if (jj == 0) { t = (w0 >> 20) & 15; qa = (w1 >> 16) & 0xFFFF; jpos = mk3(r3.x, r3.y, r3.z); jaxis = mk3(r3.w, r4.x, r4.y); q0 = r4.z; }
      else { t = m.jnt_type[j]; qa = m.jnt_qposadr[j]; jpos = ld3(m.jnt_pos + 3 * j); jaxis = ld3(m.jnt_axis + 3 * j); q0 = m.qpos0[qa]; }
      if (t == RG_JNT_FREE) {
        pos = ld3(s.qpos + qa); quat = qnormalize(ldq(s.qpos + qa + 3));
        st3(s.xanchor + 3 * j, pos); st3(s.xaxis + 3 * j, mk3(0, 0, 1));
        continue;
      }
      v3 anchor = pos + qrot(quat, jpos);
      v3 axis = qrot(quat, jaxis);
      st3(s.xanchor + 3 * j, anchor); st3(s.xaxis + 3 * j, axis);
      if (t == RG_JNT_SLIDE) pos = pos + axis * (s.qpos[qa] - q0);
      else {
        q4 ql = (t == RG_JNT_BALL) ? qnormalize(ldq(s.qpos + qa)) : axisangle(jaxis, s.qpos[qa] - q0);
        quat = qmul(quat, ql);
        pos = anchor - qrot(quat, jpos);
      }
    }
    st3(lp + 3 * b, pos); stq(lq + 4 * b, quat);
  }
  SYNC();
  for (int b = 1 + LANE; b < m.nbody; b += RG_WAVE) {
    const int dw = m.body_depth[b], depth = dw & 255, absmask = (dw >> 8) & 255, p0 = (dw >> 16) & 255;
    if (depth == 0) continue;
    const unsigned c0 = (unsigned)m.body_chain[2 * b], c1 = (unsigned)m.body_chain[2 * b + 1];
    const int w0 = __builtin_bit_cast(int, m.body_rec[RG_KINREC * b]), w1 = __builtin_bit_cast(int, m.body_rec[RG_KINREC * b + 1]);
    v3 pos = ld3(m.static_xpos + 3 * p0), ppos = pos; q4 quat = ldq(m.static_xquat + 4 * p0), pq = quat;
    for (int i = 0; i < depth; i++) {
      const int a = (i < 4 ? c0 >> (8 * i) : c1 >> (8 * (i - 4))) & 255;
      ppos = pos; pq = quat;
      if ((absmask >> i) & 1) { pos = ld3(lp + 3 * a); quat = ldq(lq + 4 * a); }
      else { pos = ppos + qrot(pq, ld3(lp + 3 * a)); quat = qnormalize(qmul(pq, ldq(lq + 4 * a))); }
    }
    const bool absolute = (absmask >> (depth - 1)) & 1;
    const int jn = (w0 >> 16) & 15, ja = w1 & 0xFFFF;
    if (!absolute) for (int jj = 0; jj < jn; jj++) {
      const int j = ja + jj;
      st3(s.xanchor + 3 * j, ppos + qrot(pq, ld3(s.xanchor + 3 * j))); st3(s.xaxis + 3 * j, qrot(pq, ld3(s.xaxis + 3 * j)));
    }
    st3(s.xpos + 3 * b, pos); stq(s.xquat + 4 * b, quat);
  }
  SYNC();
  for (int g0 = 0; g0 < m.ngeom; g0 += 2 * RG_WAVE) {
    const int gA = g0 + LANE, gB = gA + RG_WAVE, last = m.ngeom - 1, iA = gA < last ? gA : last, iB = gB < last ? gB : last;
    const int bA = m.geom_bodyid[iA], bB = m.geom_bodyid[iB];
    const v3 pA = ld3(m.geom_pos + 3 * iA), pB = ld3(m.geom_pos + 3 * iB); const q4 qA = ldq(m.geom_quat + 4 * iA), qB = ldq(m.geom_quat + 4 * iB);
    if (gA < m.ngeom) { q4 xq = ldq(s.xquat + 4 * bA); st3(s.gpos + 3 * gA, ld3(s.xpos + 3 * bA) + qrot(xq, pA)); stq(s.gquat + 4 * gA, qmul(xq, qA)); }
    if (gB < m.ngeom) { q4 xq = ldq(s.xquat + 4 * bB); st3(s.gpos + 3 * gB, ld3(s.xpos + 3 * bB) + qrot(xq, pB)); stq(s.gquat + 4 * gB, qmul(xq, qB)); }
  }
  PFOR(i, m.nsite) {
    int b = m.site_bodyid[i];
// ... 156 lines not shown
        int k0 = seg ? 2 : 0, k1 = two ? (seg ? 1 : 2) : 1;
        int b0 = seg ? bg : ba, b1 = two ? (seg ? bs : bg) : bs;
        v3 dif = q1 - q0;
        float dist = rg_sqrt(dot(dif, dif));
        L += dist * idiv;
        if (b0 != b1 && dist > 1e-15f) {
          dif = dif * rg_rcp(dist);
          v3 o0 = q0 - ld3(s.org + 3 * s.b2org[b0]), o1 = q1 - ld3(s.org + 3 * s.b2org[b1]);
          for (int e = 0; e < 4; e++) {
            int d = e == 0 ? d0 : (e == 1 ? d1 : (e == 2 ? d2 : d3));
            if (d < 0) continue;
            float v = 0;
            if ((bits >> (3 * e + k1)) & 1) v += dot(dif, jac_col(s, d, o1));
            if ((bits >> (3 * e + k0)) & 1) v -= dot(dif, jac_col(s, d, o0));
            J[e] += v * idiv;
          }
        }
      }
    }
    s.tenlen[t] = L;
    for (int e = 0; e < 4; e++) s.tenJ[4 * t + e] = J[e];
  }
  SYNC();
  PFOR(u, m.nu) {
    int id = m.actuator_trnid[u];
    s.actlen[u] = m.actuator_gear[u] * (m.actuator_trntype[u] == 0 ? s.qpos[m.jnt_qposadr[id]] : s.tenlen[id]);
  }
  SYNC();
}

__device__ __forceinline__ void rg_crb(RgM m, RgLds& s, const float* P, const int* subtree_adr, const int* subtree) {
  for (int w = LANE; w < m.nbody * 10; w += RG_WAVE) {
    int b = w / 10, k = w - 10 * b;
    float acc = 0;
    for (uint32_t bits = (uint32_t)m.subtree_mask[b]; bits; bits &= bits - 1) acc += s.cinert[10 * __builtin_ctz(bits) + k];
    s.crb[w] = acc;
  }
  SYNC();
  PFOR(e, m.nM) {
    const int ijb = m.M_ijb[e], i = ijb & 255, j = (ijb >> 8) & 255;
    float buf[6];
    mul_inert_vec(buf, s.crb + 10 * (ijb >> 16), s.cdof + 6 * i);
    const float* c = s.cdof + 6 * j;
    float v = c[0] * buf[0] + c[1] * buf[1] + c[2] * buf[2] + c[3] * buf[3] + c[4] * buf[4] + c[5] * buf[5];
    if (i == j) v += P[RG_PRM_DOF_ARMATURE + i];
    s.Msp[e] = v;
  }
  SYNC();
}
__device__ __forceinline__ void rg_M_to_blocks(RgM m, RgLds& s) {
  { rgf4 z; z.x = z.y = z.z = z.w = 0.f; rgf4* H4 = (rgf4*)s.H; for (int w = LANE; w < ((m.blkwords + 3) >> 2); w += RG_WAVE) H4[w] = z; }
  SYNC();
  PFOR(e, m.nM) { int a = m.M_ent[2 * e]; float v = s.Msp[e]; s.H[a & 0xFFFF] = v; s.H[(a >> 16) & 0xFFFF] = v; }
  SYNC();
}

struct SupPt { v3 v, s; };
struct MprGeom { int type; const float* quat; v3 pos; v3 size; int vertadr, nvert, mesh; float margin; float vscale = 1.f; };
struct MprEnv { const float* mesh_vert; const int* cell_adr; const rgf4 *cell_blk, *cell_ovf; float* prof; bool cells; bool plane_depth; };

__device__ __forceinline__ float vdot(v3 d, const rgf4& a) { return __builtin_fmaf(d.z, a.z, __builtin_fmaf(d.y, a.y, d.x * a.x)); }
template <int G> __device__ __forceinline__ void scan_batch(const rgf4* vert, int nvert, int base, v3 ld, float& bv, int& bi, v3& bp) {
  int i0 = base + (LANE & (G - 1)), last = nvert - 1;
  int j0 = i0 < last ? i0 : last, j1 = i0 + G < last ? i0 + G : last, j2 = i0 + 2 * G < last ? i0 + 2 * G : last, j3 = i0 + 3 * G < last ? i0 + 3 * G : last;
  rgf4 a = vert[j0], b = vert[j1], c = vert[j2], d = vert[j3];
  float da = vdot(ld, a), db = vdot(ld, b), dc = vdot(ld, c), dd = vdot(ld, d);
  if (da > bv) { bv = da; bi = j0; bp = mk3(a.x, a.y, a.z); }
  if (db > bv) { bv = db; bi = j1; bp = mk3(b.x, b.y, b.z); }
  if (dc > bv) { bv = dc; bi = j2; bp = mk3(c.x, c.y, c.z); }
  if (dd > bv) { bv = dd; bi = j3; bp = mk3(d.x, d.y, d.z); }
}
template <int G> __device__ __forceinline__ void scan_verts(const rgf4* vert, int nvert, v3 ld, float& bv, int& bi, v3& bp) {
  for (int base = 0; base < nvert; base += 4 * G) scan_batch<G>(vert, nvert, base, ld, bv, bi, bp);
}
__device__ __forceinline__ int dir_cell(v3 ld) {
  float ax = fabsf(ld.x), ay = fabsf(ld.y), az = fabsf(ld.z);
  int axis = ax >= ay ? (ax >= az ? 0 : 2) : (ay >= az ? 1 : 2);
  float mj = axis == 0 ? ld.x : (axis == 1 ? ld.y : ld.z), a = axis == 0 ? ld.y : (axis == 1 ? ld.z : ld.x), b = axis == 0 ? ld.z : (axis == 1 ? ld.x : ld.y);
  float inv = (0.5f * RG_CELLN) * rg_rcp(fmaxf(fabsf(mj), 1e-30f));
  int iu = (int)(a * inv + 0.5f * RG_CELLN), iv = (int)(b * inv + 0.5f * RG_CELLN);
  iu = iu < 0 ? 0 : (iu > RG_CELLN - 1 ? RG_CELLN - 1 : iu); iv = iv < 0 ? 0 : (iv > RG_CELLN - 1 ? RG_CELLN - 1 : iv);
  return ((2 * axis + (mj < 0 ? 1 : 0)) * RG_CELLN + iu) * RG_CELLN + iv;
}
template <int G> __device__ __forceinline__ void scan_cell(const int* celladr, const rgf4* cellblk, const rgf4* cellovf, v3 ld, float& bv, int& bi, v3& bp) {
  int cell = dir_cell(ld), l = LANE & (G - 1);
  int e = celladr[cell];
  if (G >= 4) {
    rgf4 a = cellblk[4 * cell + (l & 3)];
    float da = vdot(ld, a);
    if (da > bv) { bv = da; bi = __builtin_bit_cast(int, a.w); bp = mk3(a.x, a.y, a.z); }
  } else {
    rgf4 a = cellblk[4 * cell + 2 * (l & 1)], a2 = cellblk[4 * cell + 2 * (l & 1) + 1];
    float da = vdot(ld, a), da2 = vdot(ld, a2);
    if (da > bv) { bv = da; bi = __builtin_bit_cast(int, a.w); bp = mk3(a.x, a.y, a.z); }
    int i2 = __builtin_bit_cast(int, a2.w);
    if (da2 > bv || (da2 == bv && i2 < bi)) { bv = da2; bi = i2; bp = mk3(a2.x, a2.y, a2.z); }
  }
  int cnt = (e & 255) - 4, last = cnt - 1;
  if (cnt > 0) {
    const rgf4* rec = cellovf + (e >> 8);
    for (int base = 0; base < cnt; base += 2 * G) {
      int i0 = base + l, j0 = i0 < last ? i0 : last, j1 = i0 + G < last ? i0 + G : last;
      rgf4 b = rec[j0], c = rec[j1];
      float db = vdot(ld, b), dc = vdot(ld, c);
      int ib = __builtin_bit_cast(int, b.w), ic = __builtin_bit_cast(int, c.w);
      if (db > bv || (db == bv && ib < bi)) { bv = db; bi = ib; bp = mk3(b.x, b.y, b.z); }
      if (dc > bv || (dc == bv && ic < bi)) { bv = dc; bi = ic; bp = mk3(c.x, c.y, c.z); }
    }
  }
}
template <int G> __device__ __forceinline__ void scan_hull(const MprEnv& E, const MprGeom& g, v3 ld, float& bv, int& bi, v3& bp) {
  if (E.cells) scan_cell<G>(E.cell_adr + g.mesh * RG_NCELL, E.cell_blk + (size_t)g.mesh * (RG_NCELL * 4), E.cell_ovf, ld, bv, bi, bp);
  else scan_verts<G>((const rgf4*)E.mesh_vert + g.vertadr, g.nvert, ld, bv, bi, bp);
}
template <int G> __device__ __forceinline__ v3 pick_vert(float bv, int bi, v3 bp) {
  if (G == 64) {
    float vm = wave_max(bv);
    int wi = wave_min_i(bv == vm ? bi : 0x7fffffff);
    int wl = wave_min_i((bv == vm && bi == wi) ? LANE : 0x7fffffff);
    return mk3(lane_bcast(bp.x, wl), lane_bcast(bp.y, wl), lane_bcast(bp.z, wl));
  } else {
    float vm = grp_max<G>(bv);
    int wi = grp_min_i<G>(bv == vm ? bi : 0x7fffffff);
    bool win = bv == vm && bi == wi;
    return mk3(grp_max<G>(win ? bp.x : -3.0e38f), grp_max<G>(win ? bp.y : -3.0e38f), grp_max<G>(win ? bp.z : -3.0e38f));
  }
}
__device__ __forceinline__ v3 support_primitive(const MprGeom& g, v3 ld) {
  v3 lr;
  if (g.type == RG_GEOM_BOX) lr = mk3(ld.x >= 0 ? g.size.x : -g.size.x, ld.y >= 0 ? g.size.y : -g.size.y, ld.z >= 0 ? g.size.z : -g.size.z);
  else if (g.type == RG_GEOM_SPHERE) lr = ld * g.size.x;
  else if (g.type == RG_GEOM_CAPSULE) { lr = ld * g.size.x; lr.z += ld.z >= 0 ? g.size.y : -g.size.y; }
  else if (g.type == RG_GEOM_CYLINDER) {
    float n = sqrtf(ld.x * ld.x + ld.y * ld.y);
    lr = n > 1e-15f ? mk3(ld.x / n * g.size.x, ld.y / n * g.size.x, 0) : mk3(0, 0, 0);
    lr.z = ld.z >= 0 ? g.size.y : -g.size.y;
  } else {
    v3 t = mk3(ld.x * g.size.x, ld.y * g.size.y, ld.z * g.size.z);
    float n = fmaxf(norm(t), 1e-15f);
    lr = mk3(t.x * g.size.x / n, t.y * g.size.y / n, t.z * g.size.z / n);
  }
  return lr;
}
template <int G> __device__ __forceinline__ v3 rg_support(const MprEnv& E, const MprGeom& g, v3 dir) {
  q4 gq = ldq(g.quat);
  v3 ld = qrotT(gq, dir), lr;
  if (g.type == RG_GEOM_MESH) {
    float bv = -3.0e38f; int bi = 0x7fffffff; v3 bp = mk3(0, 0, 0);
    scan_hull<G>(E, g, ld, bv, bi, bp);
    lr = pick_vert<G>(bv, bi, bp) * g.vscale;
  } else lr = support_primitive(g, ld);
  lr = lr + ld * g.margin;
  return qrot(gq, lr) + g.pos;
}
template <int G> __device__ __forceinline__ void mpr_support(const MprEnv& E, const MprGeom& a, const MprGeom& b, v3 dir, SupPt& p) {
  long long tt0 = E.prof ? rg_clock() : 0;
  q4 qa = ldq(a.quat), qb = ldq(b.quat);
  v3 la = qrotT(qa, dir), lb = qrotT(qb, dir * -1.0f), ra, rb;
  float av = -3.0e38f, bvv = -3.0e38f; int ai = 0x7fffffff, bi = 0x7fffffff; v3 ap = mk3(0, 0, 0), bp = mk3(0, 0, 0);
  bool am = a.type == RG_GEOM_MESH, bm = b.type == RG_GEOM_MESH;
  if (am) scan_hull<G>(E, a, la, av, ai, ap);
  if (bm) scan_hull<G>(E, b, lb, bvv, bi, bp);
  long long tt1 = E.prof ? rg_clock() : 0;
  ra = am ? pick_vert<G>(av, ai, ap) * a.vscale : support_primitive(a, la);
  rb = bm ? pick_vert<G>(bvv, bi, bp) * b.vscale : support_primitive(b, lb);
  v3 w1 = qrot(qa, ra + la * a.margin) + a.pos;
  v3 w2 = qrot(qb, rb + lb * b.margin) + b.pos;
  p.v = w1 - w2; p.s = w1 + w2;
  if (E.prof && LANE == 0) { long long tt2 = rg_clock(); E.prof[20] += 1.f; E.prof[21] += (float)(tt1 - tt0); E.prof[22] += (float)(tt2 - tt1); }
}
#define MPR_EPS 1.0e-7f
__device__ __forceinline__ bool mz(float x) { return fabsf(x) < MPR_EPS * 1e-3f; }
__device__ __forceinline__ v3 portal_dir(const SupPt& p1, const SupPt& p2, const SupPt& p3) { return normalized(cross(p2.v - p1.v, p3.v - p1.v)); }
__device__ __forceinline__ bool portal_reach_tol(const SupPt& p1, const SupPt& p2, const SupPt& p3, const SupPt& v4, v3 dir, float tol) {
  float dv4 = dot(v4.v, dir);
  float mn = fminf(fminf(dv4 - dot(p1.v, dir), dv4 - dot(p2.v, dir)), dv4 - dot(p3.v, dir));
  return mn <= tol;
}
__device__ __forceinline__ v3 sel3(bool c, v3 a, v3 b) { return mk3(c ? a.x : b.x, c ? a.y : b.y, c ? a.z : b.z); }
__device__ __forceinline__ void expand_portal(const SupPt& p0, SupPt& p1, SupPt& p2, SupPt& p3, const SupPt& v4) {
  v3 c = cross(v4.v, p0.v);
  bool a = dot(p1.v, c) > 0, b = dot(p2.v, c) > 0, d = dot(p3.v, c) > 0;
  bool to1 = a ? b : !d, to3 = a && !b, to2 = !a && d;
  p1.v = sel3(to1, v4.v, p1.v); p1.s = sel3(to1, v4.s, p1.s);
  p2.v = sel3(to2, v4.v, p2.v); p2.s = sel3(to2, v4.s, p2.s);
  p3.v = sel3(to3, v4.v, p3.v); p3.s = sel3(to3, v4.s, p3.s);
}
__device__ __forceinline__ float origin_tri_dist2(v3 a, v3 b, v3 c, v3& w) {
  v3 ab = b - a, ac = c - a, ap = a * -1.0f;
  float d1 = dot(ab, ap), d2 = dot(ac, ap);
  if (d1 <= 0 && d2 <= 0) { w = a; return dot(w, w); }
  v3 bp = b * -1.0f; float d3 = dot(ab, bp), d4 = dot(ac, bp);
  if (d3 >= 0 && d4 <= d3) { w = b; return dot(w, w); }
  float vc = d1 * d4 - d3 * d2;
  if (vc <= 0 && d1 >= 0 && d3 <= 0) { w = a + ab * (d1 / (d1 - d3)); return dot(w, w); }
  v3 cp = c * -1.0f; float d5 = dot(ab, cp), d6 = dot(ac, cp);
  if (d6 >= 0 && d5 <= d6) { w = c; return dot(w, w); }
  float vb = d5 * d2 - d1 * d6;
  if (vb <= 0 && d2 >= 0 && d6 <= 0) { w = a + ac * (d2 / (d2 - d6)); return dot(w, w); }
  float va = d3 * d6 - d5 * d4;
  if (va <= 0 && (d4 - d3) >= 0 && (d5 - d6) >= 0) { w = b + (c - b) * ((d4 - d3) / ((d4 - d3) + (d5 - d6))); return dot(w, w); }
  float den = 1.0f / (va + vb + vc);
  w = a + ab * (vb * den) + ac * (vc * den);
  return dot(w, w);
}
__device__ __forceinline__ void mpr_result(bool plane_depth, const SupPt& p0, const SupPt& p1, const SupPt& p2, const SupPt& p3, v3 dir, float& depth, v3& dir_out, v3& pos) {
  if (plane_depth) {
    depth = fmaxf((dot(p1.v, dir) + dot(p2.v, dir) + dot(p3.v, dir)) * (1.0f / 3.0f), 0.f);
    dir_out = dir;
  } else {
    v3 w; depth = sqrtf(origin_tri_dist2(p1.v, p2.v, p3.v, w));
    dir_out = mz(depth) ? mk3(0, 0, 0) : w * (1.0f / depth);
  }
  float b0 = dot(cross(p1.v, p2.v), p3.v), b1 = dot(cross(p3.v, p2.v), p0.v);
  float b2 = dot(cross(p0.v, p1.v), p3.v), b3 = dot(cross(p2.v, p1.v), p0.v);
  float sum = b0 + b1 + b2 + b3;
  if (sum <= 0) {
    v3 dd = portal_dir(p1, p2, p3);
    b0 = 0; b1 = dot(cross(p2.v, p3.v), dd); b2 = dot(cross(p3.v, p1.v), dd); b3 = dot(cross(p1.v, p2.v), dd);
    sum = b1 + b2 + b3;
  }
  float inv = 0.5f * rg_rcp(sum);
  pos = p0.s * (b0 * inv) + p1.s * (b1 * inv) + p2.s * (b2 * inv) + p3.s * (b3 * inv);
}
enum { MPR_DONE = 0, MPR_FIRST, MPR_SECOND, MPR_DISCOVER, MPR_REFINE, MPR_PENETR };
template <int G> __device__ __forceinline__ bool rg_mpr(const MprEnv& E, const MprGeom& A, const MprGeom& B, int max_iter, float tol, float& depth, v3& dir_out, v3& pos, v3& sep, bool active) {
  SupPt p0, p1, p2, p3;
  p0.v = p0.s = p1.v = p1.s = p2.v = p2.s = p3.v = p3.s = mk3(0, 0, 0);
  int state = active ? MPR_FIRST : MPR_DONE, guard = 0;
  bool result = false, finish = false;
  v3 dir = mk3(1, 0, 0);
  sep = mk3(0, 0, 0);
  if (active) {
    p0.s = A.pos + B.pos; p0.v = A.pos - B.pos;
    if (mz(p0.v.x) && mz(p0.v.y) && mz(p0.v.z)) p0.v.x += 1e-6f;
    dir = normalized(p0.v * -1.0f);
  }
  while (__ballot(state != MPR_DONE)) {
    if (state == MPR_DONE) continue;
    SupPt q;
    mpr_support<G>(E, A, B, dir, q);
    float dq = dot(q.v, dir);
    bool to_refine = false;
    if (state == MPR_FIRST) {
      p1 = q;
      if (dq <= 0) { sep = dir; state = MPR_DONE; }
      else {
        dir = cross(p0.v, p1.v);
        if (dot(dir, dir) < 1e-30f) {
          pos = p1.s * 0.5f; result = true; state = MPR_DONE;
          if (dot(p1.v, p1.v) < 1e-30f) { depth = 0; dir_out = mk3(0, 0, 0); }
          else { depth = norm(p1.v); dir_out = p1.v * (1.0f / depth); }
        } else { dir = normalized(dir); state = MPR_SECOND; }
      }
    } else if (state == MPR_SECOND) {
      p2 = q;
      if (dq <= 0) { sep = dir; state = MPR_DONE; }
      else {
        dir = normalized(cross(p1.v - p0.v, p2.v - p0.v));
        if (dot(dir, p0.v) > 0) { SupPt t = p1; p1 = p2; p2 = t; dir = dir * -1.0f; }
        state = MPR_DISCOVER; guard = 0;
      }
    } else if (state == MPR_DISCOVER) {
      p3 = q;
      if (dq <= 0) { sep = dir; state = MPR_DONE; }
      else {
        bool cont = false;
        if (dot(cross(p1.v, p3.v), p0.v) < 0) { p2 = p3; cont = true; }
        if (!cont && dot(cross(p3.v, p2.v), p0.v) < 0) { p1 = p3; cont = true; }
        if (cont) { dir = normalized(cross(p1.v - p0.v, p2.v - p0.v)); if (++guard > 64) state = MPR_DONE; }
        else { to_refine = true; guard = 0; }
      }
    } else {
      bool penetr = state == MPR_PENETR;
      bool reach = portal_reach_tol(p1, p2, p3, q, dir, tol);
      bool expand = false;
      if (!penetr) {
        if (dq < 0) { sep = dir; state = MPR_DONE; }
        else if (reach) state = MPR_DONE;
        else expand = true;
      } else if (reach || guard > max_iter) {
        finish = true; state = MPR_DONE;
      } else expand = true;
      if (expand) {
        expand_portal(p0, p1, p2, p3, q);
        guard++;
        if (!penetr && guard > 128) state = MPR_DONE;
        else to_refine = true;
      }
    }
    if (to_refine) {
      dir = portal_dir(p1, p2, p3);
      if (state != MPR_PENETR) { if (dot(dir, p1.v) >= 0) { state = MPR_PENETR; guard = 0; } else state = MPR_REFINE; }
    }
  }
  if (finish) { mpr_result(E.plane_depth, p0, p1, p2, p3, dir, depth, dir_out, pos); result = true; }
  return result;
}

__device__ __forceinline__ float obb_gap(const float* Ra, v3 ea, const float* Rb, v3 eb, v3 tw) {
  float R[9], AR[9];
  for (int i = 0; i < 3; i++) for (int j = 0; j < 3; j++) {
    R[3 * i + j] = Ra[i] * Rb[j] + Ra[3 + i] * Rb[3 + j] + Ra[6 + i] * Rb[6 + j];
    AR[3 * i + j] = fabsf(R[3 * i + j]) + 1e-6f;
  }
  v3 t = mulmT(Ra, tw);
  float ta[3] = {t.x, t.y, t.z}, a[3] = {ea.x, ea.y, ea.z}, b[3] = {eb.x, eb.y, eb.z};
  float gap = -1.f;
  for (int i = 0; i < 3; i++) gap = fmaxf(gap, fabsf(ta[i]) - (a[i] + b[0] * AR[3 * i] + b[1] * AR[3 * i + 1] + b[2] * AR[3 * i + 2]));
  for (int j = 0; j < 3; j++) gap = fmaxf(gap, fabsf(ta[0] * R[j] + ta[1] * R[3 + j] + ta[2] * R[6 + j]) - (a[0] * AR[j] + a[1] * AR[3 + j] + a[2] * AR[6 + j] + b[j]));
  if (gap > 0) return gap;
  for (int i = 0; i < 3; i++) for (int j = 0; j < 3; j++) {
    int i1 = (i + 1) % 3, i2 = (i + 2) % 3, j1 = (j + 1) % 3, j2 = (j + 2) % 3;
    float ra = a[i1] * AR[3 * i2 + j] + a[i2] * AR[3 * i1 + j];
    float rb = b[j1] * AR[3 * i + j2] + b[j2] * AR[3 * i + j1];
    if (fabsf(ta[i2] * R[3 * i1 + j] - ta[i1] * R[3 * i2 + j]) > ra + rb) return 0.f;
  }
  return -1.f;
}

__device__ __forceinline__ void make_frame(float* f) {
  v3 n = normalized(ld3(f));
  v3 y = (n.y < 0.5f && n.y > -0.5f) ? mk3(0, 1, 0) : mk3(0, 0, 1);
  y = normalized(y - n * dot(n, y));
  st3(f, n); st3(f + 3, y); st3(f + 6, cross(n, y));
}
__device__ __forceinline__ void add_contact(RgLds& s, int pair, float dist, v3 pos, v3 normal, int dim) {
  int c = s.ncon;
  SYNC();
  if (c >= RG_MAXCON) { if (LANE == 0) s.status |= RG_STATUS_CON_FULL; return; }
  if (LANE == 0) {
    s.c_dist[c] = dist; st3(s.c_pos + 3 * c, pos); st3(s.c_normal + 3 * c, normalized(normal));
    s.c_pair[c] = pair; s.c_dim[c] = dim; s.ncon = c + 1;
  }
  SYNC();
}

__device__ __forceinline__ MprEnv rg_mpr_env(RgM m, float* prof, bool cells) {
  MprEnv E;
  E.mesh_vert = m.mesh_vert; E.cell_adr = m.mesh_cell_adr; E.cell_blk = (const rgf4*)m.mesh_cell_blk; E.cell_ovf = (const rgf4*)m.mesh_cell_ovf;
  E.prof = prof; E.cells = cells; E.plane_depth = false;
  return E;
}
__device__ __forceinline__ void rg_mpr_geoms(RgM m, const RgLds& s, int p, float gscale, MprGeom& A, MprGeom& B, int& dim, float& margin) {
  const rgf4* R = (const rgf4*)m.pair_rec + (RG_PAIRREC / 4) * p;
  rgf4 r0 = R[0], r1 = R[1], r2 = R[2], r3 = R[3];
  int hdr = __builtin_bit_cast(int, r0.x), g1 = hdr & 255, g2 = (hdr >> 8) & 255;
  dim = (hdr >> 16) & 15; margin = r0.y;
  A.type = (hdr >> 20) & 15; A.quat = s.gquat + 4 * g1; A.size = mk3(r1.x, r1.y, r1.z); A.margin = 0.5f * margin; A.pos = mk3(0, 0, 0);
  B.type = (hdr >> 24) & 15; B.quat = s.gquat + 4 * g2; B.size = mk3(r2.x, r2.y, r2.z); B.margin = 0.5f * margin; B.pos = ld3(s.gpos + 3 * g2) - ld3(s.gpos + 3 * g1);
  if (hdr & RG_PAIR_SCALED1) A.size = A.size * gscale;
  if (hdr & RG_PAIR_SCALED2) B.size = B.size * gscale;
  A.mesh = __builtin_bit_cast(int, r0.z); A.vertadr = __builtin_bit_cast(int, r3.x); A.nvert = __builtin_bit_cast(int, r1.w);
  B.mesh = __builtin_bit_cast(int, r0.w); B.vertadr = __builtin_bit_cast(int, r3.y); B.nvert = __builtin_bit_cast(int, r2.w);
}
__device__ __forceinline__ v3 pick3(v3 a0, v3 a1, v3 a2, int k) { return k == 0 ? a0 : (k == 1 ? a1 : a2); }
__device__ __forceinline__ float pick3(float a0, float a1, float a2, int k) { return k == 0 ? a0 : (k == 1 ? a1 : a2); }
__device__ __forceinline__ bool box_box_lane(const float* A, const float* B, q4 q1, q4 q2, v3 P1, v3 t, float margin, int l, float& dist, v3& pos, v3& n) {
  float R1[9], R2[9]; q2mat(R1, q1); q2mat(R2, q2);
  v3 ax1[3], ax2[3];
#pragma unroll
  for (int k = 0; k < 3; k++) { ax1[k] = mk3(R1[k], R1[3 + k], R1[6 + k]); ax2[k] = mk3(R2[k], R2[3 + k], R2[6 + k]); }
  float ta[3], tb[3], Q[3][3];
#pragma unroll
  for (int i = 0; i < 3; i++) { ta[i] = dot(t, ax1[i]); tb[i] = dot(t, ax2[i]);
#pragma unroll
    for (int j = 0; j < 3; j++) Q[i][j] = fabsf(dot(ax1[i], ax2[j])); }
  float best = -3.0e38f; int code = 0; bool sep = false; n = mk3(0, 0, 0);
#pragma unroll
  for (int i = 0; i < 3; i++) {
    float sv = fabsf(ta[i]) - (A[i] + B[0] * Q[i][0] + B[1] * Q[i][1] + B[2] * Q[i][2]);
    sep = sep || sv > margin;
    if (sv > best) { best = sv; code = 1 + i; n = ax1[i] * (ta[i] < 0 ? -1.f : 1.f); }
  }
#pragma unroll
  for (int j = 0; j < 3; j++) {
    float sv = fabsf(tb[j]) - (B[j] + A[0] * Q[0][j] + A[1] * Q[1][j] + A[2] * Q[2][j]);
    sep = sep || sv > margin;
    if (sv > best) { best = sv; code = 4 + j; n = ax2[j] * (tb[j] < 0 ? -1.f : 1.f); }
// ... 44 lines not shown
  const float isgn = dot(nr, iab) > 0 ? -1.f : 1.f;
  const v3 ic = ip + iab * (isgn * pick3(is[0], is[1], is[2], ib));
  const int u = (ia + 1) % 3, v = (ia + 2) % 3, iu = (ib + 1) % 3, iv = (ib + 2) % 3;
  const v3 ru = pick3(rax[0], rax[1], rax[2], u), rv = pick3(rax[0], rax[1], rax[2], v);
  const float lu = pick3(rs[0], rs[1], rs[2], u), lv = pick3(rs[0], rs[1], rs[2], v), la = pick3(rs[0], rs[1], rs[2], ia);
  const v3 eu = pick3(iax[0], iax[1], iax[2], iu) * pick3(is[0], is[1], is[2], iu), ev = pick3(iax[0], iax[1], iax[2], iv) * pick3(is[0], is[1], is[2], iv);
  const v3 rel = ic - rp;
  const float c2x = dot(rel, ru), c2y = dot(rel, rv), e1x = dot(eu, ru), e1y = dot(eu, rv), e2x = dot(ev, ru), e2y = dot(ev, rv);
  float x = 0, y = 0; bool ok = false;
  if (l < 4) {
    const float su = (l == 0 || l == 3) ? 1.f : -1.f, sv = l < 2 ? 1.f : -1.f;
    x = c2x + su * e1x + sv * e2x; y = c2y + su * e1y + sv * e2y;
    ok = fabsf(x) <= lu && fabsf(y) <= lv;
  } else if (l < 8) {
    x = (l & 1) ? lu : -lu; y = (l & 2) ? lv : -lv;
    const float det = e1x * e2y - e1y * e2x, dx = x - c2x, dy = y - c2y;
    if (fabsf(det) > 1e-12f) { const float a = (dx * e2y - dy * e2x) / det, b = (e1x * dy - e1y * dx) / det; ok = fabsf(a) < 1.f && fabsf(b) < 1.f; }
  } else if (l < 24) {
    const int ea = (l - 8) >> 2, eb = (l - 8) & 3, k0 = ea, k1 = (ea + 1) & 3;
    const float su0 = (k0 == 0 || k0 == 3) ? 1.f : -1.f, sv0 = k0 < 2 ? 1.f : -1.f, su1 = (k1 == 0 || k1 == 3) ? 1.f : -1.f, sv1 = k1 < 2 ? 1.f : -1.f;
    const float ax_ = c2x + su0 * e1x + sv0 * e2x, ay_ = c2y + su0 * e1y + sv0 * e2y, bx_ = c2x + su1 * e1x + sv1 * e2x, by_ = c2y + su1 * e1y + sv1 * e2y;
    const bool xedge = eb < 2; const float sg = (eb & 1) ? -1.f : 1.f, lim = xedge ? lu : lv, olim = xedge ? lv : lu;
    const float da = sg * (xedge ? ax_ : ay_) - lim, db = sg * (xedge ? bx_ : by_) - lim;
    if ((da < 0 && db > 0) || (da > 0 && db < 0)) {
      const float tt = da / (da - db);
      x = ax_ + tt * (bx_ - ax_); y = ay_ + tt * (by_ - ay_);
      ok = fabsf(xedge ? y : x) <= olim;
    }
  }
  if (!ok) return false;
  const v3 base = rp + ru * x + rv * y, inorm = iab * isgn;
  const float dn = dot(nr, inorm), hh = fabsf(dn) > 1e-12f ? dot(ic - base, inorm) / dn : dot(ic - base, nr);
  dist = hh - la;
  if (dist > margin) return false;
  pos = base + nr * (la + 0.5f * dist) + P1;
  return true;
}
__device__ __forceinline__ bool rg_box_box_lane(RgM m, const RgLds& s, int p, float gscale, int l, float& dist, v3& pos, v3& n, int& dim) {
  const rgf4* Rc = (const rgf4*)m.pair_rec + (RG_PAIRREC / 4) * p;
  rgf4 r0 = Rc[0], r1 = Rc[1], r2 = Rc[2];
  const int hdr = __builtin_bit_cast(int, r0.x), g1 = hdr & 255, g2 = (hdr >> 8) & 255;
  dim = (hdr >> 16) & 15;
  const float margin = r0.y;
  const float sc1 = (hdr & RG_PAIR_SCALED1) ? gscale : 1.f, sc2 = (hdr & RG_PAIR_SCALED2) ? gscale : 1.f;
  const float A[3] = {r1.x * sc1, r1.y * sc1, r1.z * sc1}, B[3] = {r2.x * sc2, r2.y * sc2, r2.z * sc2};
  const v3 P1 = ld3(s.gpos + 3 * g1), t = ld3(s.gpos + 3 * g2) - P1;
  return box_box_lane(A, B, ldq(s.gquat + 4 * g1), ldq(s.gquat + 4 * g2), P1, t, margin, l, dist, pos, n);
}
RG_STAGE void rg_narrow_boxbox(RgCtx c, int ncand) {
  RgM m = RG_M(c); RgLRef L = RG_L(c); RgLds& s = RG_S();
  const float gscale = rg_prm(m, L)[RG_PRM_GEOM_SCALE];
  const int l = LANE & 31, grp = LANE >> 5;
  for (int cbase = 0; cbase < ncand; cbase += RG_WAVE) {
    bool is_bb = false;
    if (cbase + LANE < ncand) { const int hdr = __builtin_bit_cast(int, m.pair_rec[RG_PAIRREC * s.cand[cbase + LANE]]); is_bb = ((hdr >> 20) & 15) == RG_GEOM_BOX && ((hdr >> 24) & 15) == RG_GEOM_BOX; }
    unsigned long long bits = __ballot(is_bb);
    while (bits) {
      const int ci0 = cbase + __builtin_ctzll(bits); bits &= bits - 1;
      int ci1 = -1; if (bits) { ci1 = cbase + __builtin_ctzll(bits); bits &= bits - 1; }
      const int ci = grp == 0 ? ci0 : ci1;
      bool hit = false; float dist = 0; v3 pos = mk3(0, 0, 0), nrm = mk3(0, 0, 1); int p = 0, dim = 3;
      if (ci >= 0) { p = s.cand[ci]; hit = rg_box_box_lane(m, s, p, gscale, l, dist, pos, nrm, dim); }
      unsigned long long bal = __ballot(hit);
      int cb = s.ncon;
      SYNC();
      if (hit) {
        int cc = cb + __popcll(bal & ((1ull << LANE) - 1ull));
        if (cc < RG_MAXCON) { s.c_dist[cc] = dist; st3(s.c_pos + 3 * cc, pos); st3(s.c_normal + 3 * cc, normalized(nrm)); s.c_pair[cc] = p; s.c_dim[cc] = dim; }
        else s.status |= RG_STATUS_CON_FULL;
      }
      if (LANE == 0) { int nn = cb + __popcll(bal); s.ncon = nn < RG_MAXCON ? nn : RG_MAXCON; }
      SYNC();
    }
  }
}
template <int G> RG_STAGE void rg_narrow_phase1(RgCtx c, int ncand) {
  RgM m = RG_M(c); RgLRef L = RG_L(c); RgLds& s = RG_S();
  bool cells = !(L.flags & 8);
  rgf4* sepdir = L.bt.sepdir ? (rgf4*)L.bt.sepdir + (size_t)rg_env(L) * m.npair : (rgf4*)0;
  float* pairlb = (L.bt.pairlb && !(L.flags & 4)) ? L.bt.pairlb + (size_t)rg_env(L) * m.npair : (float*)0;
  const float gscale = rg_prm(m, L)[RG_PRM_GEOM_SCALE];
  MprEnv E = rg_mpr_env(m, (float*)0, cells);
  const bool boxbox = !(L.flags & 16);
  for (int base = 0; base < ncand; base += RG_WAVE / G) {
    int ci = base + LANE / G;
    bool keep = false; int p = 0;
    if (ci < ncand) {
      p = s.cand[ci];
      MprGeom A, B; int dim; float margin;
      rg_mpr_geoms(m, s, p, gscale, A, B, dim, margin);
      if (A.type != RG_GEOM_PLANE && !(boxbox && A.type == RG_GEOM_BOX && B.type == RG_GEOM_BOX)) {
        v3 c0 = A.pos - B.pos;
        if (mz(c0.x) && mz(c0.y) && mz(c0.z)) c0.x += 1e-6f;
        v3 dir = normalized(c0 * -1.0f);
        if (sepdir) { rgf4 cd; const float* sp_ = (const float*)(sepdir + p); cd.x = RG_ROW_LD(sp_); cd.y = RG_ROW_LD(sp_ + 1); cd.z = RG_ROW_LD(sp_ + 2); cd.w = 0.f; if (cd.x * cd.x + cd.y * cd.y + cd.z * cd.z > 0.5f) dir = mk3(cd.x, cd.y, cd.z); }
        SupPt p1; mpr_support<G>(E, A, B, dir, p1);
        float d = dot(p1.v, dir);
        keep = d > 0;
        if (!keep && pairlb && (LANE & (G - 1)) == 0) RG_ROW_ST(pairlb + p, fmaxf(-d - 1e-6f, 0.f));
      }
    }
    bool lead = keep && (LANE & (G - 1)) == 0;
    unsigned long long bal = __ballot(lead);
    int cbase = s.ncand2;
    SYNC();
    if (lead) {
      int slot = cbase + __popcll(bal & ((1ull << LANE) - 1ull));
      if (slot < RG_MAXCAND2) s.cand2[slot] = p; else s.status |= RG_STATUS_CAND_FULL;
    }
    if (LANE == 0) { int n = cbase + __popcll(bal); s.ncand2 = n < RG_MAXCAND2 ? n : RG_MAXCAND2; }
    SYNC();
  }
}
template <int G> RG_STAGE_BIG void rg_narrow_phase2(RgCtx c, int ncand2) {
  RgM m = RG_M(c); RgLRef L = RG_L(c); RgLds& s = RG_S();
  bool cells = !(L.flags & 8);
  float* prof = (L.flags & 2) ? s.prof : (float*)0;
  rgf4* sepdir = L.bt.sepdir ? (rgf4*)L.bt.sepdir + (size_t)rg_env(L) * m.npair : (rgf4*)0;
  const float gscale = rg_prm(m, L)[RG_PRM_GEOM_SCALE];
  MprEnv E = rg_mpr_env(m, prof, cells);
  E.plane_depth = (L.flags & 16) != 0;
  for (int base = 0; base < ncand2; base += RG_WAVE / G) {
    int ci = base + LANE / G;
    bool hit = false;
    float depth = 0, margin = 0; v3 dir = mk3(0, 0, 0), pos = mk3(0, 0, 0); int p = 0, dim = 3;
    bool active = ci < ncand2;
    MprGeom A, B;
    if (active) {
      p = s.cand2[ci];
      rg_mpr_geoms(m, s, p, gscale, A, B, dim, margin);
    }
    v3 sep;
    hit = rg_mpr<G>(E, A, B, m.mpr_iterations, m.mpr_tolerance, depth, dir, pos, sep, active);
    if (active) {
      if (sepdir && (LANE & (G - 1)) == 0) { rgf4 cd; cd.x = hit ? 0.f : sep.x; cd.y = hit ? 0.f : sep.y; cd.z = hit ? 0.f : sep.z; cd.w = 0.f; RG_SEPDIR_ST(sepdir + p, cd); }
      hit = hit && dot(dir, dir) > 0.25f;
      pos = pos + ld3(s.gpos + 3 * (m.pair_gg[p] & 255));
    }
    bool lead = hit && (LANE & (G - 1)) == 0;
    unsigned long long bal = __ballot(lead);
    int cbase = s.ncon;
    SYNC();
    if (lead) {
      int c = cbase + __popcll(bal & ((1ull << LANE) - 1ull));
      if (c < RG_MAXCON) {
        s.c_dist[c] = margin - depth; st3(s.c_pos + 3 * c, pos); st3(s.c_normal + 3 * c, normalized(dir));
        s.c_pair[c] = p; s.c_dim[c] = dim;
      } else s.status |= RG_STATUS_CON_FULL;
    }
    if (LANE == 0) { int n = cbase + __popcll(bal); s.ncon = n < RG_MAXCON ? n : RG_MAXCON; }
    SYNC();
  }
}
__device__ __forceinline__ void rg_collision(RgCtx c, RgM m, RgLds& s, const float* P, float* prof, rgf4* sepdir, float* pairlb, bool cells) {
  long long tb0 = rg_clock();
  const float gscale = P[RG_PRM_GEOM_SCALE];
  if (LANE == 0) { s.ncand = 0; s.ncon = 0; }
  SYNC();
  int nround = (m.npair + RG_WAVE - 1) / RG_WAVE;
  float hb = 1.5f * P[RG_PRM_TIMESTEP];
  int nt = 0; bool bbany = false, plany = false;
  int gg_next[4]; float lb_next[4];
#pragma unroll
  for (int k = 0; k < 4; k++) { int p = k * RG_WAVE + LANE, pc = p < m.npair ? p : m.npair - 1; gg_next[k] = m.pair_gg[pc]; lb_next[k] = pairlb ? RG_ROW_LD(pairlb + pc) : 0.f; }
  for (int r0 = 0; r0 < nround; r0 += 4) {
    int gg[4]; float lbv[4];
#pragma unroll
    for (int k = 0; k < 4; k++) { gg[k] = gg_next[k]; lbv[k] = lb_next[k]; }
    if (r0 + 4 < nround) {
#pragma unroll
      for (int k = 0; k < 4; k++) { int p = (r0 + 4 + k) * RG_WAVE + LANE, pc = p < m.npair ? p : m.npair - 1; gg_next[k] = m.pair_gg[pc]; lb_next[k] = pairlb ? RG_ROW_LD(pairlb + pc) : 0.f; }
    }
#pragma unroll
    for (int k = 0; k < 4; k++) {
      int p = (r0 + k) * RG_WAVE + LANE;
      bool need = false;
      if (p < m.npair) {
        int g1 = gg[k] & 255, g2 = gg[k] >> 8;
        float lb = lbv[k] - (hb * (s.gspeed[g1] + s.gspeed[g2]) + 1e-7f);
        need = !(lb > 0.f);
        if (!need) RG_ROW_ST(pairlb + p, lb);
      }
      unsigned long long nb = __ballot(need);
      if (need) s.tlist[nt + __popcll(nb & ((1ull << LANE) - 1ull))] = (short)p;
      nt += __popcll(nb);
    }
    if (nt <= RG_TLIST - 4 * RG_WAVE && r0 + 4 < nround) continue;
    SYNC();
#ifdef RG_FINE_PROF
    const long long tref0 = rg_clock();
    if (prof && LANE == 0) { prof[42] += (float)nt; prof[43] += (float)((nt + RG_WAVE - 1) / RG_WAVE); }
#endif
    for (int i0 = 0; i0 < nt; i0 += RG_WAVE) {
      int i = i0 + LANE, q = 0;
      bool hit = false, isbb = false, ispl = false;
      if (i < nt) {
        q = s.tlist[i];
        const rgf4* R = (const rgf4*)m.pair_rec + (RG_PAIRREC / 4) * q;
        rgf4 r0 = R[0], r3 = R[3], r4 = R[4], r5 = R[5];
        int hdr = __builtin_bit_cast(int, r0.x), g1 = hdr & 255, g2 = (hdr >> 8) & 255;
        float margin = r0.y, newlb = 0.f;
        const float sc1 = (hdr & RG_PAIR_SCALED1) ? gscale : 1.f, sc2 = (hdr & RG_PAIR_SCALED2) ? gscale : 1.f;
        r3.z *= sc1; r3.w *= sc2;
        v3 p1 = ld3(s.gpos + 3 * g1), p2 = ld3(s.gpos + 3 * g2), dif = p2 - p1;
        isbb = ((hdr >> 20) & 255) == (RG_GEOM_BOX | (RG_GEOM_BOX << 4)); ispl = ((hdr >> 20) & 15) == RG_GEOM_PLANE;
        if (((hdr >> 20) & 15) == RG_GEOM_PLANE) {
          float d = dot(dif, qrot(ldq(s.gquat + 4 * g1), mk3(0, 0, 1))) - (r3.w + margin);
          hit = d <= 0; newlb = fmaxf(d, 0.f);
        } else {
          float d = sqrtf(dot(dif, dif)) - (r3.z + r3.w + margin);
          if (d <= 0) {
            float hm = 0.5f * margin + 1e-6f;
            v3 ea = mk3(r4.x * sc1 + hm, r4.y * sc1 + hm, r4.z * sc1 + hm), eb = mk3(r5.x * sc2 + hm, r5.y * sc2 + hm, r5.z * sc2 + hm);
            float Ra[9], Rb[9]; q2mat(Ra, ldq(s.gquat + 4 * g1)); q2mat(Rb, ldq(s.gquat + 4 * g2));
            float og = obb_gap(Ra, ea, Rb, eb, dif);
            hit = og < 0; newlb = fmaxf(og, 0.f);
          } else newlb = d;
        }
        if (pairlb) RG_ROW_ST(pairlb + q, fmaxf(newlb - 1e-6f, 0.f));
      }
      unsigned long long bal = __ballot(hit);
      bbany = bbany || (hit && isbb); plany = plany || (hit && ispl);
      int base = s.ncand;
      SYNC();
      if (hit) {
        int slot = base + __popcll(bal & ((1ull << LANE) - 1ull));
        if (slot < RG_MAXCAND) s.cand[slot] = q; else s.status |= RG_STATUS_CAND_FULL;
      }
      if (LANE == 0) { int n = base + __popcll(bal); s.ncand = n < RG_MAXCAND ? n : RG_MAXCAND; }
      SYNC();
    }
#ifdef RG_FINE_PROF
    if (prof && LANE == 0) prof[44] += (float)(rg_clock() - tref0);
#endif
    nt = 0;
  }
  if (prof && LANE == 0) prof[5] += (float)(rg_clock() - tb0);
  int ncand = s.ncand;
  if (LANE == 0) s.ncand2 = 0;
  SYNC();
  if (ncand > 16) rg_narrow_phase1<2>(c, ncand); else rg_narrow_phase1<4>(c, ncand);
  int ncand2 = s.ncand2;
  if (prof && LANE == 0) { prof[16] += (float)(rg_clock() - tb0); prof[17] += ncand; prof[18] += ncand2; }
  rg_narrow_phase2<4>(c, ncand2);
  if (prof && LANE == 0) prof[19] += (float)(rg_clock() - tb0);
  if (!(RG_L(c).flags & 16) && __ballot(bbany) != 0) rg_narrow_boxbox(c, ncand);
  if (__ballot(plany) != 0)
  for (int cbase = 0; cbase < ncand; cbase += RG_WAVE) {
  bool is_plane = false;
  if (cbase + LANE < ncand) is_plane = ((__builtin_bit_cast(int, m.pair_rec[RG_PAIRREC * s.cand[cbase + LANE]]) >> 20) & 15) == RG_GEOM_PLANE;
  unsigned long long plane_bits = __ballot(is_plane);
  while (plane_bits) {
    int ci = cbase + __builtin_ctzll(plane_bits); plane_bits &= plane_bits - 1;
    int p = s.cand[ci];
    int g1 = m.pair_geom[3 * p], g2 = m.pair_geom[3 * p + 1], dim = m.pair_geom[3 * p + 2];
    float margin = m.pair_prm[12 * p];
    int t2 = m.geom_type[g2];
    v3 p1 = ld3(s.gpos + 3 * g1), p2 = ld3(s.gpos + 3 * g2);
    MprGeom B;
    B.type = t2; B.quat = s.gquat + 4 * g2; B.size = ld3(m.geom_size + 3 * g2); B.margin = 0; B.mesh = -1; B.vertadr = 0; B.nvert = 0;
    if (__builtin_bit_cast(int, m.pair_rec[RG_PAIRREC * p]) & RG_PAIR_SCALED2) B.size = B.size * gscale;
    if (t2 == RG_GEOM_MESH) { B.mesh = m.geom_dataid[g2]; B.vertadr = m.mesh_vertadr[B.mesh]; B.nvert = m.mesh_vertnum[B.mesh]; }
    v3 n = qrot(ldq(s.gquat + 4 * g1), mk3(0, 0, 1));
    if (t2 == RG_GEOM_BOX) {
      int cnt = 0;
      for (int i = 0; i < 8 && cnt < 4; i++) {
        v3 lc = mk3((i & 1) ? B.size.x : -B.size.x, (i & 2) ? B.size.y : -B.size.y, (i & 4) ? B.size.z : -B.size.z);
        v3 c = qrot(ldq(B.quat), lc) + p2;
        float dist = dot(c - p1, n);
        if (dist > margin) continue;
        add_contact(s, p, dist, c - n * (0.5f * dist), n, dim); cnt++;
      }
    } else {
      B.pos = p2 - p1;
      v3 sp = rg_support<64>(rg_mpr_env(m, (float*)0, false), B, n * -1.0f);
      float dist = dot(sp, n);
      if (dist <= margin) add_contact(s, p, dist, sp + p1 - n * (0.5f * dist), n, dim);
    }
  }
  }
  SYNC();
}

__device__ __forceinline__ void rg_velocity(RgM m, RgLds& s, const float* P, const uint32_t* dof_velmask, const int* subtree_adr, const int* subtree) {
  PFOR(d, m.nv) {
    float cv[6] = {0, 0, 0, 0, 0, 0};
    for (int h = 0; h < 2; h++) {
      uint32_t bits = dof_velmask[2 * d + h];
      while (bits) { int a = __builtin_ctz(bits) + 32 * h; bits &= bits - 1; float q = s.qvel[a]; for (int e = 0; e < 6; e++) cv[e] += s.cdof[6 * a + e] * q; }
    }
    int j = m.dof_jntid[d];
    if (m.jnt_type[j] == RG_JNT_FREE && d - m.jnt_dofadr[j] < 3) { for (int e = 0; e < 6; e++) s.cdofdot[6 * d + e] = 0; }
    else cross_motion(s.cdofdot + 6 * d, cv, s.cdof + 6 * d);
  }
  PFOR(t, m.ntendon) {
    float v = 0;
    for (int e = 0; e < 4; e++) { int d = m.ten_dofs[4 * t + e]; if (d >= 0) v += s.tenJ[4 * t + e] * s.qvel[d]; }
    s.tenvel[t] = v;
    s.tenfrc[t] = m.tendon_stiffness[t] * (m.tendon_lengthspring[t] - s.tenlen[t]) - m.tendon_damping[t] * v;
  }
  SYNC();
  PFOR(k, m.body_geomnum[0]) s.gspeed[m.body_geomadr[0] + k] = 0;
  for (int b = 1 + LANE; b < m.nbody; b += RG_WAVE) {
    float cv[6] = {0, 0, 0, 0, 0, 0}, ca[6] = {0, 0, 0, -P[RG_PRM_GRAVITY], -P[RG_PRM_GRAVITY + 1], -P[RG_PRM_GRAVITY + 2]};
    for (int h = 0; h < 2; h++) {
      uint32_t bits = m.body_dofmask[2 * b + h];
      while (bits) {
        int a = __builtin_ctz(bits) + 32 * h; bits &= bits - 1; float q = s.qvel[a];
        for (int e = 0; e < 6; e++) { cv[e] += s.cdof[6 * a + e] * q; ca[e] += s.cdofdot[6 * a + e] * q; }
      }
    }
    {
      const float gsmax = fmaxf(P[RG_PRM_GEOM_SCALE], 1.f);
      v3 w = mk3(cv[0], cv[1], cv[2]), vo = mk3(cv[3], cv[4], cv[5]), og = ld3(s.org + 3 * s.b2org[b]);
      float wn = norm(w);
      int ga = m.body_geomadr[b], gn = m.body_geomnum[b];
      for (int k = 0; k < gn; k++) s.gspeed[ga + k] = norm(vo + cross(w, ld3(s.gpos + 3 * (ga + k)) - og)) + wn * (m.geom_rbound[ga + k] * gsmax);
    }
    float t1[6], t2[6], t3[6];
    mul_inert_vec(t1, s.cinert + 10 * b, ca);
    mul_inert_vec(t2, s.cinert + 10 * b, cv);
    cross_force(t3, cv, t2);
    for (int e = 0; e < 6; e++) s.cacc[6 * b + e] = t1[e] + t3[e];
  }
  SYNC();
  {
    float acc[(RG_MAXBODY * 6 + RG_WAVE - 1) / RG_WAVE];
#pragma unroll
    for (int k0 = 0; k0 < (RG_MAXBODY * 6 + RG_WAVE - 1) / RG_WAVE; k0++) {
      int w = LANE + RG_WAVE * k0, b = w / 6, k = w - 6 * b; float a = 0;
      if (w < m.nbody * 6 && b > 0) for (uint32_t bits = (uint32_t)m.subtree_mask[b]; bits; bits &= bits - 1) a += s.cacc[6 * __builtin_ctz(bits) + k];
      acc[k0] = a;
    }
    SYNC();
#pragma unroll
    for (int k0 = 0; k0 < (RG_MAXBODY * 6 + RG_WAVE - 1) / RG_WAVE; k0++) { int w = LANE + RG_WAVE * k0; if (w < m.nbody * 6) s.cacc[w] = acc[k0]; }
  }
  SYNC();
  PFOR(d, m.nv) {
    const rgf4 dr0 = ((const rgf4*)m.dof_rec)[2 * d]; const float spring_ref = m.dof_rec[8 * d + 4];
    const int w0 = __builtin_bit_cast(int, dr0.x);
    const float *c = s.cdof + 6 * d, *f = s.cacc + 6 * (w0 & 255);
    s.qfrc_bias[d] = c[0] * f[0] + c[1] * f[1] + c[2] * f[2] + c[3] * f[3] + c[4] * f[4] + c[5] * f[5];
    float pas = -P[RG_PRM_DOF_DAMPING + d] * s.qvel[d];
    if (dr0.z != 0) pas -= dr0.z * (s.qpos[__builtin_bit_cast(int, dr0.w)] - spring_ref);
    for (int q = (w0 >> 8) & 255; q < ((w0 >> 16) & 255); q++) { int tt = m.dof_ten[2 * q], sl = m.dof_ten[2 * q + 1]; pas += s.tenJ[4 * tt + sl] * s.tenfrc[tt]; }
    s.qfrc_passive[d] = pas;
  }
  SYNC();
}

static_assert(RG_MAXU <= RG_WAVE && RG_MAXNV <= RG_WAVE, "controller state / warm start: one lane per actuator / dof");
__device__ __forceinline__ void rg_pid(RgM m, RgLds& s, const float* P, float* st ) {
  float dt = P[RG_PRM_TIMESTEP];
  PFOR(u, m.nu) {
    const float* gp = P + RG_PRM_ACT_GAINPRM + 10 * u;
    float force;
    float lo = P[RG_PRM_ACT_FORCERANGE + 2 * u], hi = P[RG_PRM_ACT_FORCERANGE + 2 * u + 1];
// ... 1487 lines not shown
        if (LANE == 0) L.bt.redo[e] = sub + 1;
        rg_item_publish(prog, e, sub + 1);
        continue;
      }
      st_pid(c, pidr);
      st_smooth(c);
      st_factor_smooth(c);
      const int packed = st_solve(c, warmr), iters = packed & 255, nefc = packed >> 8;
      st_ncon = (float)s.ncon; st_nefc = (float)nefc; st_iter = (float)iters;
      float bd = 0; PFOR(i, m.nv) bd += (fabsf(s.qacc[i]) < 1e10f) ? 0.f : 1.f;
      if (wave_sum(bd) > 0) bad = newly_bad = true;
      else warmr = st_euler(c, warmr);
    }
    if (newly_bad && LANE == 0) s.status |= RG_STATUS_BAD_STATE;
    if (last) {
      const int nticks = L.bt.nticks ? L.bt.nticks[e] : nforward_ticks;
      if (nticks > 0 || L.bt.obs || L.bt.xdata) {
        st_kinematics(c);
        if (L.bt.xdata) {
          float* xd = L.bt.xdata + (size_t)e * RG_XDATA;
          PFOR(i, 3 * m.nbody) xd[RG_XD_XPOS + i] = s.xpos[i];
          PFOR(i, 4 * m.nbody) xd[RG_XD_XQUAT + i] = s.xquat[i];
          PFOR(i, 3 * m.nsite) xd[RG_XD_SITE_XPOS + i] = s.spos[i];
        }
        st_com_pos(c); st_tendon(c);
        for (int q = 0; q < nticks; q++) st_pid(c, pidr);
        if (L.bt.xdata) PFOR(u, m.nu) L.bt.xdata[(size_t)e * RG_XDATA + RG_XD_ACT_FORCE + u] = s.actfrc[u];
      }
    }
    PFOR(i, m.nq) RG_ROW_ST(L.bt.qpos + (size_t)e * m.nq + i, s.qpos[i]);
    if (LANE < m.nv) { RG_ROW_ST(L.bt.qvel + (size_t)e * m.nv + LANE, s.qvel[LANE]); RG_ROW_ST(L.bt.qacc_warmstart + (size_t)e * m.nv + LANE, warmr); }
    if (LANE < m.nu) for (int q = 0; q < 3; q++) RG_ROW_ST(L.bt.pid + (size_t)e * 3 * m.nu + 3 * LANE + q, pidr[q]);
    if (sub == 0) PFOR(u, m.nu) RG_ROW_ST(L.bt.ctrl + (size_t)e * m.nu + u, s.ctrl[u]);
    if (LANE == 0) {
      if (cleared_preticks) L.bt.preticks[e] = 0;
      if (s.status != status0) RG_ROW_ST(L.bt.status + e, s.status);
      if (last) L.bt.time[e] += nsub * P[RG_PRM_TIMESTEP];
      if (L.bt.cost) { const float cy = (float)(rg_clock() - tk0); RG_ROW_ST(L.bt.cost + e, sub == 0 ? cy : RG_ROW_LD(L.bt.cost + e) + cy); }
      if (L.bt.stats) { float* st = L.bt.stats + 4 * (size_t)e; RG_ROW_ST(st, RG_ROW_LD(st) + st_ncon); RG_ROW_ST(st + 1, RG_ROW_LD(st + 1) + st_nefc); RG_ROW_ST(st + 2, RG_ROW_LD(st + 2) + st_iter); RG_ROW_ST(st + 3, RG_ROW_LD(st + 3) + 1.f); }
    }
    if (last && L.bt.obs) {
      int od = 3 + 4 + m.nq + m.nv + L.env.n_hand_jnt + 15;
      float* o = L.bt.obs + (size_t)e * od;
      PFOR(i, 3) o[i] = s.qpos[L.env.cube_pos_qposadr + i];
      { float sg = s.qpos[L.env.cube_quat_qposadr] < 0 ? -1.f : 1.f; PFOR(i, 4) o[3 + i] = sg * s.qpos[L.env.cube_quat_qposadr + i]; }
      PFOR(i, m.nq) o[7 + i] = (i >= L.env.target_qposadr && i < L.env.target_qposadr + L.env.target_nq) ? 0.f : s.qpos[i];
      PFOR(i, m.nv) o[7 + m.nq + i] = (i >= L.env.target_dofadr && i < L.env.target_dofadr + L.env.target_nv) ? 0.f : s.qvel[i];
      PFOR(i, L.env.n_hand_jnt) o[7 + m.nq + m.nv + i] = s.qpos[L.env.hand_qposadr + i];
      PFOR(i, 5) {
        v3 r0 = ld3(s.spos + 3 * L.env.ref_site[0]), r1 = ld3(s.spos + 3 * L.env.ref_site[1]), r2 = ld3(s.spos + 3 * L.env.ref_site[2]);
        v3 a = normalized(r0 - r1), cc = normalized(r2 - r1), b = cross(a, cc);
        v3 tt = ld3(s.spos + 3 * L.env.tip_site[i]) - r1;
        float* ot = o + 7 + m.nq + m.nv + L.env.n_hand_jnt + 3 * i;
        ot[0] = dot(tt, a); ot[1] = dot(tt, b); ot[2] = dot(tt, cc);
      }
      if (L.bt.goal_quat && L.bt.goal_dist && LANE == 0) {
        q4 g = ldq(L.bt.goal_quat + 4 * (size_t)e), cq = ldq(s.qpos + L.env.cube_quat_qposadr);
        cq.x = -cq.x; cq.y = -cq.y; cq.z = -cq.z;
        q4 dq = qmul(g, cq);
        L.bt.goal_dist[e] = 2.0f * acosf(clampf(fabsf(dq.w), -1.f, 1.f));
      }
    }
    rg_item_publish(prog, e, (sub + 1) | (bad ? RG_SCHED_BAD : 0));
  }
  int g = 0;
  if (LANE == 0) g = rg_ticket(sched + RG_SCHED_FIN);
  g = rg_first(g);
  if (g == (int)gridDim.x - 1) {
    int ok = 1;
    if (LANE == 0) for (int x = 0; x < nq_; x++) { const int n = (B - x + nq_ - 1) / nq_ * nsub; if (rg_ld_sc1(sched + 16 * x) < n) ok = 0; }
    ok = rg_first(ok);
    if (!ok) {
      PFOR(e, B) {
        if (L.bt.active && !L.bt.active[e]) continue;
        const int p = rg_ld_sc1(prog + e) & 0xFFFF;
        if (p < nsub) { if (L.bt.redo) L.bt.redo[e] = p + 1; L.bt.status[e] |= RG_STATUS_SCHED; }
      }
    }
  }
}
#endif

#if !RG_ITEMS
__global__ void __launch_bounds__(RG_WAVE) rg_mpr_pair_kernel(const RgModelDev* mp, RgLaunch launch, int g1, int g2, float margin, float* out) {
  RG_MAKE_CTX();
  RgM m = RG_M(c);
  RgLRef L = RG_L(c);
  RgLds& s = RG_S();
  int e = blockIdx.x;
  PFOR(i, m.nq) s.qpos[i] = L.bt.qpos[(size_t)e * m.nq + i];
  SYNC();
  st_kinematics(c);
  MprGeom A, B;
  v3 p1 = ld3(s.gpos + 3 * g1), p2 = ld3(s.gpos + 3 * g2);
  A.type = m.geom_type[g1]; A.quat = s.gquat + 4 * g1; A.size = ld3(m.geom_size + 3 * g1); A.margin = 0.5f * margin; A.pos = mk3(0, 0, 0);
  B.type = m.geom_type[g2]; B.quat = s.gquat + 4 * g2; B.size = ld3(m.geom_size + 3 * g2); B.margin = 0.5f * margin; B.pos = p2 - p1;
  A.mesh = B.mesh = -1; A.vertadr = B.vertadr = 0; A.nvert = B.nvert = 0;
  if (A.type == RG_GEOM_MESH) { A.mesh = m.geom_dataid[g1]; A.vertadr = m.mesh_vertadr[A.mesh]; A.nvert = m.mesh_vertnum[A.mesh]; }
  if (B.type == RG_GEOM_MESH) { B.mesh = m.geom_dataid[g2]; B.vertadr = m.mesh_vertadr[B.mesh]; B.nvert = m.mesh_vertnum[B.mesh]; }
  MprEnv E = rg_mpr_env(m, (float*)0, true);
  E.plane_depth = true;
  float depth = 0; v3 dir = mk3(0, 0, 0), pos = mk3(0, 0, 0);
  v3 sep; bool hit = rg_mpr<64>(E, A, B, m.mpr_iterations, m.mpr_tolerance, depth, dir, pos, sep, true);
  if (LANE == 0) {
    float* o = out + 8 * (size_t)e;
    o[0] = hit ? 1.f : 0.f; o[1] = depth; o[2] = dir.x; o[3] = dir.y; o[4] = dir.z; o[5] = pos.x + p1.x; o[6] = pos.y + p1.y; o[7] = pos.z + p1.z;
  }
}

#if RG_SETCONST
struct RgSetconstX { float cdof[6 * RG_MAXNV], off[3 * RG_MAXBODY], x[RG_MAXNV], y[RG_MAXNV], dg[RG_MAXNV]; };
static inline size_t rg_lds_setconst_bytes() { return sizeof(RgLds) + sizeof(RgSetconstX); }
__global__ void __launch_bounds__(RG_WAVE) rg_setconst_kernel(const RgModelDev* mp, RgLaunch launch, float* envprm) {
  RG_MAKE_CTX();
  RgM m = RG_M(c);
  RgLRef L = RG_L(c);
  RgLds& s = RG_S();
  RgSetconstX& X = *(RgSetconstX*)((char*)&s + sizeof(RgLds));
  const int e = blockIdx.x;
  if (e >= L.bt.B) return;
  if (L.bt.active && !L.bt.active[e]) return;
  PFOR(i, m.nq) s.qpos[i] = m.qpos0[i];
  if (LANE == 0) { s.has_xfrc = 0; s.status = 0; }
  st_build_row_desc(c);
  SYNC();
  st_kinematics(c); st_com_pos(c); st_tendon(c);
  PFOR(i, 6 * m.nv) X.cdof[i] = s.cdof[i];
  for (int b = 1 + LANE; b < m.nbody; b += RG_WAVE) st3(X.off + 3 * b, rg_xipos(m, s, b) - ld3(s.org + 3 * s.b2org[b]));
  SYNC();
  st_crb(c);
  LtdlDesc D;
  rg_ltdl_load(m.ltdl_tri, m.ltdl_pair, m.n_tri_rounds, m.n_pair_rounds, D);
  rg_M_to_blocks(m, s);
  const int d = LANE; const bool on = d < m.nv;
  const int blk = on ? m.dof_blk[d] : 0, akk = (blk & 0xFFFF) + d - ((blk >> 16) & 255);
  rg_ltdl_factor(s, D);
  float* P = envprm + (size_t)e * RG_NPRM;
  for (int i = 0; i < m.nv; i++) {
    if (on) X.x[d] = d == i ? 1.f : 0.f;
    SYNC();
    rg_ltdl_solve(s, D, X.x, d, on, akk);
    if (LANE == 0) X.dg[i] = X.x[i];
    SYNC();
  }
  PFOR(j, m.njnt) {
    const int da = m.jnt_dofadr[j], t = m.jnt_type[j];
    if (t == RG_JNT_FREE || t == RG_JNT_BALL) {
      for (int h = 0; h < (t == RG_JNT_FREE ? 2 : 1); h++) {
        const float a = (X.dg[da + 3 * h] + X.dg[da + 3 * h + 1] + X.dg[da + 3 * h + 2]) * (1.f / 3.f);
        for (int k = 0; k < 3; k++) P[RG_PRM_DOF_INVWEIGHT0 + da + 3 * h + k] = a;
      }
    } else P[RG_PRM_DOF_INVWEIGHT0 + da] = X.dg[da];
  }
  for (int b = 1; b < m.nbody; b++) {
    if ((m.body_depth[b] & 255) == 0) { if (LANE == 0) { P[RG_PRM_BODY_INVWEIGHT0 + 2 * b] = 0.f; P[RG_PRM_BODY_INVWEIGHT0 + 2 * b + 1] = 0.f; } continue; }
    float tr[2] = {0.f, 0.f};
    const v3 off = ld3(X.off + 3 * b);
    for (int k = 0; k < 6; k++) {
      float v = 0.f;
      if (on && in_chain(m, b, d)) {
        const v3 ang = ld3(X.cdof + 6 * d), jc = k < 3 ? ld3(X.cdof + 6 * d + 3) + cross(ang, off) : ang;
        const int kk = k < 3 ? k : k - 3;
        v = kk == 0 ? jc.x : (kk == 1 ? jc.y : jc.z);
      }
      if (on) { X.x[d] = v; X.y[d] = v; }
      SYNC();
      rg_ltdl_solve(s, D, X.x, d, on, akk);
      tr[k < 3 ? 0 : 1] += wave_sum(on ? X.x[d] * X.y[d] : 0.f);
      SYNC();
    }
    if (LANE == 0) { P[RG_PRM_BODY_INVWEIGHT0 + 2 * b] = fmaxf(1e-15f, tr[0] * (1.f / 3.f)); P[RG_PRM_BODY_INVWEIGHT0 + 2 * b + 1] = fmaxf(1e-15f, tr[1] * (1.f / 3.f)); }
  }
  for (int t = 0; t < m.ntendon; t++) {
    float v = 0.f;
    if (on) for (int q = 0; q < 4; q++) if (m.ten_dofs[4 * t + q] == d) v += s.tenJ[4 * t + q];
    if (on) { X.x[d] = v; X.y[d] = v; }
    SYNC();
    rg_ltdl_solve(s, D, X.x, d, on, akk);
    const float w = wave_sum(on ? X.x[d] * X.y[d] : 0.f);
    SYNC();
    if (LANE == 0) P[RG_PRM_TENDON_INVWEIGHT0 + t] = fmaxf(1e-15f, w);
  }
  if (LANE == 0 && s.status) L.bt.status[e] |= s.status;
}
#endif

__global__ void rg_copy_rows_kernel(float* dst, const float* src, const int* mask, int n, int col0, int ncols, float* pairlb, int npair) {
  int e = blockIdx.x;
  if (!mask[e]) return;
  for (int i = LANE; i < ncols; i += RG_WAVE) dst[(size_t)e * n + col0 + i] = src[(size_t)e * ncols + i];
// ... 14 lines not shown
```

### robogym_amd/csrc/rg_types.h

```cpp
#pragma once
#include <stdint.h>

#define RG_MAXNQ 40
#define RG_MAXNV 36
#define RG_MAXBODY 32
#define RG_MAXJNT 32
#define RG_MAXGEOM 66
#define RG_MAXSITE 40
#define RG_MAXTEN 12
#define RG_MAXU 20
#define RG_MAXFRIC 32
#define RG_MAXSROW 96
#define RG_MAXNVC 32
#define RG_HWORDS 1124
#define RG_MAXNM 160
#define RG_CELLN 8
#define RG_NCELL (6 * RG_CELLN * RG_CELLN)
#define RG_LTDL_TRI_ROUNDS 12
#define RG_LTDL_PAIR_ROUNDS 8
#define RG_KINREC 20
#define RG_MAXDEPTH 8
#define RG_MAXSENSOR 8
#define RG_PAIRREC 28
#define RG_PAIR_SCALED1 (1 << 28)
#define RG_PAIR_SCALED2 (1 << 29)
#define RG_TLIST 320
#define RG_MAXROW 64
#define RG_W 14
#define RG_WAVE 64

enum {
  RG_PRM_GRAVITY = 0,
  RG_PRM_TIMESTEP = 3,
  RG_PRM_DOF_DAMPING = 4,
  RG_PRM_DOF_ARMATURE = RG_PRM_DOF_DAMPING + RG_MAXNV,
  RG_PRM_DOF_FRICTIONLOSS = RG_PRM_DOF_ARMATURE + RG_MAXNV,
  RG_PRM_DOF_INVWEIGHT0 = RG_PRM_DOF_FRICTIONLOSS + RG_MAXNV,
  RG_PRM_BODY_MASS = RG_PRM_DOF_INVWEIGHT0 + RG_MAXNV,
  RG_PRM_BODY_INERTIA = RG_PRM_BODY_MASS + RG_MAXBODY,
  RG_PRM_BODY_INVWEIGHT0 = RG_PRM_BODY_INERTIA + 3 * RG_MAXBODY,
  RG_PRM_JNT_RANGE = RG_PRM_BODY_INVWEIGHT0 + 2 * RG_MAXBODY,
  RG_PRM_TENDON_RANGE = RG_PRM_JNT_RANGE + 2 * RG_MAXJNT,
  RG_PRM_TENDON_INVWEIGHT0 = RG_PRM_TENDON_RANGE + 2 * RG_MAXTEN,
  RG_PRM_ACT_GAINPRM = RG_PRM_TENDON_INVWEIGHT0 + RG_MAXTEN,
  RG_PRM_ACT_CTRLRANGE = RG_PRM_ACT_GAINPRM + 10 * RG_MAXU,
  RG_PRM_ACT_FORCERANGE = RG_PRM_ACT_CTRLRANGE + 2 * RG_MAXU,
  RG_PRM_GEOM_FRICTION = RG_PRM_ACT_FORCERANGE + 2 * RG_MAXU,
  RG_PRM_XFRC = RG_PRM_GEOM_FRICTION + 3 * RG_MAXGEOM,
  RG_PRM_SITE_POS = RG_PRM_XFRC + 6 * RG_MAXBODY,
  RG_PRM_GEOM_SCALE = RG_PRM_SITE_POS + 3 * RG_MAXSITE,
  RG_PRM_JNT_MARGIN = RG_PRM_GEOM_SCALE + 1,
  RG_PRM_GEOM_SOLREF = RG_PRM_JNT_MARGIN + RG_MAXJNT,
  RG_PRM_GEOM_SOLIMP = RG_PRM_GEOM_SOLREF + 2 * RG_MAXGEOM,
  RG_NPRM = RG_PRM_GEOM_SOLIMP + 5 * RG_MAXGEOM
};

enum {
  RG_XD_XPOS = 0,
  RG_XD_XQUAT = RG_XD_XPOS + 3 * RG_MAXBODY,
  RG_XD_SITE_XPOS = RG_XD_XQUAT + 4 * RG_MAXBODY,
  RG_XD_ACT_FORCE = RG_XD_SITE_XPOS + 3 * RG_MAXSITE,
  RG_XD_NCON = RG_XD_ACT_FORCE + RG_MAXU,
  RG_XD_CONTACT = RG_XD_NCON + 1,
  RG_XD_SENSOR = RG_XD_CONTACT + 3 * 32,
  RG_XDATA = RG_XD_SENSOR + 8
};

#define RG_STATUS_BAD_STATE 1u
#define RG_STATUS_CON_FULL 2u
#define RG_STATUS_CAND_FULL 4u
#define RG_STATUS_ROW_FULL 8u
#define RG_STATUS_BAD_FACTOR 16u
#define RG_STATUS_BAD_ACTION 32u
#define RG_STATUS_SCHED 64u

enum { RG_JNT_FREE = 0, RG_JNT_BALL = 1, RG_JNT_SLIDE = 2, RG_JNT_HINGE = 3 };
enum { RG_GEOM_PLANE = 0, RG_GEOM_SPHERE = 2, RG_GEOM_CAPSULE = 3, RG_GEOM_ELLIPSOID = 4, RG_GEOM_CYLINDER = 5, RG_GEOM_BOX = 6, RG_GEOM_MESH = 7 };
enum { RG_WRAP_JOINT = 1, RG_WRAP_PULLEY = 2, RG_WRAP_SITE = 3, RG_WRAP_SPHERE = 4, RG_WRAP_CYLINDER = 5 };

struct RgModelDev {
  int nq, nv, nu, nbody, njnt, ngeom, nsite, ntendon, nwrap, nmesh;
  int nlevel, ndoflevel, nM, npair, nstatic, nfric_dof, nfric_ten, nlim_jnt, nlim_ten;
  int nvc, hs, blkwords, ntree, maxtree;
  const int *dof_blk, *dof_blk2, *c_blk, *d2c, *c2d;
  int iterations, mpr_iterations, cone;
  float timestep, gravity[3], tolerance, impratio, mpr_tolerance, meaninertia;
  const int *body_parentid, *body_rootid, *body_jntadr, *body_jntnum, *body_dofadr, *body_dofnum, *body_lastdof;
  const float *body_pos, *body_quat, *body_ipos, *body_iquat, *body_mass, *body_inertia, *body_invweight0;
  const int *ltdl_tri, *ltdl_pair;
  int n_tri_rounds, n_pair_rounds;
  const int *ltdl_tri_c, *ltdl_pair_c;
  int n_tri_rounds_c, n_pair_rounds_c, tree_newton_ok;
  const int* subtree_mask;
  const float* body_rec;
  const int* body_depth;
  const int* body_chain;
  const float *static_xpos, *static_xquat;
  const int *root_origin_body, *body_orgslot;
  const float* root_origin_const;
  const float* org_rec;
  const uint32_t* body_dofmask;
  const int *jnt_type, *jnt_qposadr, *jnt_dofadr, *jnt_bodyid;
  const float *jnt_pos, *jnt_axis, *jnt_stiffness, *jnt_range, *jnt_margin, *jnt_solref, *jnt_solimp;
  const int *dof_bodyid, *dof_jntid, *dof_parentid;
  const float *dof_armature, *dof_damping, *dof_frictionloss, *dof_solref, *dof_solimp, *dof_invweight0;
  const float *qpos0, *qpos_spring;
  const int *lvl_dof, *lvl_dof_adr, *M_i, *M_j, *M_lvl_adr, *desc_adr, *desc;
  const float* prm_default;
// ... 88 lines not shown
```

Before: 2.010 million.

## Widen mesh support cells to eight inline records and hand over first MPR support

After: 2.003 million. Within noise of the previous version (-0.4%).

```diff
diff --git a/include/rgstep.h b/include/rgstep.h
--- a/include/rgstep.h
+++ b/include/rgstep.h
@@ -164,6 +164,7 @@
 int rg_wrap_args_size(void);
 int rg_batch_set_constants(rg_batch* b, const int* mask_dev, void* stream);
 int rg_batch_mpr_pair(rg_batch* b, int g1, int g2, float margin, float* out_dev, void* stream);
+int rg_batch_mpr_pair_ex(rg_batch* b, int g1, int g2, float margin, int flags, float* out_dev, void* stream);
 int rg_batch_items_info(const rg_batch* b, int* slots, int* queues);
 int rg_obs_dim(const rg_batch* b);
 int rg_debug_size(void);
diff --git a/robogym_amd/_native.py b/robogym_amd/_native.py
--- a/robogym_amd/_native.py
+++ b/robogym_amd/_native.py
@@ -156,7 +156,7 @@
 EXPORTS = [
     "rg_model_create", "rg_model_free", "rg_model_dims", "rg_batch_create", "rg_batch_free", "rg_batch_set_env",
     "rg_batch_copy", "rg_batch_reset", "rg_batch_step", "rg_obs_dim", "rg_debug_size", "rg_lds_bytes", "rg_sync",
-    "rg_last_error", "rg_batch_mpr_pair", "rg_batch_copy_rows", "rg_batch_step_ex", "rg_batch_field_ptr", "rg_model_create_on", "rg_model_npair",
+    "rg_last_error", "rg_batch_mpr_pair", "rg_batch_mpr_pair_ex", "rg_batch_copy_rows", "rg_batch_step_ex", "rg_batch_field_ptr", "rg_model_create_on", "rg_model_npair",
     "rg_lds_bytes_cfg", "rg_env_post_step", "rg_post_args_size", "rg_batch_enable_env_params", "rg_prm_layout", "rg_xdata_layout", "rg_batch_set_constants", "rg_batch_items_info",
     "rb_model_create", "rb_model_free", "rb_model_info", "rb_scratch_offset", "rb_batch_create", "rb_batch_free", "rb_batch_reset", "rb_batch_set_env",
     "rb_batch_field_ptr", "rb_batch_step", "rb_batch_step_ex", "rb_env_post_step", "rb_post_args_size", "rb_cube_ops", "rb_batch_step_tcp", "ra_env_post_step", "ra_post_args_size",
@@ -199,6 +199,8 @@
     L.rg_batch_copy_rows.argtypes = [vp, ci, vp, vp, ci, ci, vp]
     L.rg_batch_step.argtypes = [vp, vp, vp, vp, vp, vp, ci, ci, ci, vp]
     L.rg_batch_mpr_pair.argtypes = [vp, ci, ci, cf, vp, vp]
+    if hasattr(L, "rg_batch_mpr_pair_ex"):
+        L.rg_batch_mpr_pair_ex.argtypes = [vp, ci, ci, cf, ci, vp, vp]
     L.rg_obs_dim.argtypes = [vp]
     L.rg_debug_size.restype = ci
     L.rg_lds_bytes.restype = ci
@@ -290,6 +292,7 @@
 RG_FLAG_SUBSTEP_ITEMS = 128
 RG_FLAG_CAPACITY_TEST_HOOK = 512
 RG_FLAG_DESERT_QUEUE0 = 1024
+RG_FLAG_NO_SUPPORT_HANDOVER = 2048
 RG_STATUS_SCHED = 64
 RG_FLAG_RESUME = 256
 
diff --git a/robogym_amd/csrc/rb_kernel.h b/robogym_amd/csrc/rb_kernel.h
--- a/robogym_amd/csrc/rb_kernel.h
+++ b/robogym_amd/csrc/rb_kernel.h
@@ -1258,7 +1258,7 @@
       A.margin = B.margin = plane ? 0.f : 0.5f * margin;
     }
     v3 sep, dir = mk3(0, 0, 0); float depth = 0;
-    const bool mh = rg_mpr<4>(E, A, B, m.mpr_iterations, m.mpr_tolerance, depth, dir, pos, sep, active && !plane && !special);
+    const bool mh = rg_mpr<4, RB_CELLW>(E, A, B, m.mpr_iterations, m.mpr_tolerance, depth, dir, pos, sep, active && !plane && !special, false, SupPt());
     if (active && !plane && !special) {
       hit = mh && dot(dir, dir) > 0.25f;
       dist = margin - depth; nrm = normalized(dir); pos = pos + p1;
@@ -1266,7 +1266,7 @@
     const v3 pn = qrot(ldq(A.quat), mk3(0, 0, 1));
     MprGeom Bs = B;
     if (!(active && plane && !special)) { Bs.type = RG_GEOM_SPHERE; Bs.mesh = -1; Bs.size = mk3(0, 0, 0); }
-    const v3 sp = rg_support<4>(E, Bs, (active && plane && !special) ? pn * -1.0f : mk3(0, 0, 1));
+    const v3 sp = rg_support<4, RB_CELLW>(E, Bs, (active && plane && !special) ? pn * -1.0f : mk3(0, 0, 1));
     if (active && plane && !special) {
       dist = dot(sp, pn);
       hit = dist <= margin;
diff --git a/robogym_amd/csrc/rb_types.h b/robogym_amd/csrc/rb_types.h
--- a/robogym_amd/csrc/rb_types.h
+++ b/robogym_amd/csrc/rb_types.h
@@ -17,6 +17,7 @@
 #define RB_CONW 24
 #define RB_STARB 5
 #define RB_MLONG 8
+#define RB_CELLW 4
 #define RB_NW 22
 
 #define RB_INT_ARRAYS(X) \
diff --git a/robogym_amd/csrc/rg_api.hip b/robogym_amd/csrc/rg_api.hip
--- a/robogym_amd/csrc/rg_api.hip
+++ b/robogym_amd/csrc/rg_api.hip
@@ -393,17 +393,17 @@
     std::vector<int> vadr, cadr, vidx;
     if (!get_i(B, "mesh_vertadr", vadr, e) || !get_i(B, "k_mesh_cell_adr", cadr, e) || !get_i(B, "k_mesh_cell_vidx", vidx, e)) return bail(e, m);
     if (cadr.size() != (size_t)d.nmesh * RG_NCELL) return bail("k_mesh_cell_adr has the wrong size (RG_CELLN mismatch?)", m);
-    std::vector<float> blk((size_t)d.nmesh * RG_NCELL * 16, 0.f), ovf(4, 0.f);
+    std::vector<float> blk((size_t)d.nmesh * RG_NCELL * (4 * RG_CELLW), 0.f), ovf(4, 0.f);
     for (int mi = 0; mi < d.nmesh; mi++) for (int c = 0; c < RG_NCELL; c++) {
       size_t ce = (size_t)mi * RG_NCELL + c;
       int e = cadr[ce], start = e >> 8, cnt = e & 255;
       if (cnt < 1 || (size_t)(start + cnt) > vidx.size()) return bail("bad support cell", m);
       cadr[ce] = (int)((ovf.size() / 4) << 8) | cnt;
-      for (int k = 0; k < (cnt > 4 ? cnt : 4); k++) {
+      for (int k = 0; k < (cnt > RG_CELLW ? cnt : RG_CELLW); k++) {
         int vi = vidx[start + (k < cnt ? k : cnt - 1)]; size_t src = (size_t)(vadr[mi] + vi);
         if (vi < 0 || src * 3 + 2 >= fv.size()) return bail("bad support cell vertex", m);
         float o[4] = {fv[3 * src], fv[3 * src + 1], fv[3 * src + 2], 0.f}; memcpy(o + 3, &vi, 4);
-        if (k < 4) memcpy(blk.data() + ce * 16 + 4 * k, o, 16); else ovf.insert(ovf.end(), o, o + 4);
+        if (k < RG_CELLW) memcpy(blk.data() + (ce * RG_CELLW + k) * 4, o, 16); else ovf.insert(ovf.end(), o, o + 4);
       }
     }
     if (!upload<int>(m, cadr, &d.mesh_cell_adr) || !upload<float>(m, blk, &d.mesh_cell_blk) || !upload<float>(m, ovf, &d.mesh_cell_ovf)) return bail("hipMalloc failed", m); }
@@ -784,6 +784,14 @@
   DeviceGuard g(b->device);
   RgLaunch launch_args{b->model->aux, b->env, b->dev, 0, 0, 0, 1};
   return launch(rgs::rg_mpr_pair_kernel, b->dev.B, RG_WAVE, sizeof(rgs::RgLds), 0, stream, b->model->dev_copy, launch_args, g1, g2, margin, out_dev);
+}
+int rg_batch_mpr_pair_ex(rg_batch* b, int g1, int g2, float margin, int flags, float* out_dev, void* stream) {
+  if (!b || !out_dev) return fail("null argument");
+  const RgModelDev& d = b->model->dev;
+  if (g1 < 0 || g2 < 0 || g1 >= d.ngeom || g2 >= d.ngeom) return fail("geom id out of range");
+  DeviceGuard g(b->device);
+  RgLaunch launch_args{b->model->aux, b->env, b->dev, 0, 0, flags, 1};
+  return launch(rgs::rg_mpr_pair_quad_kernel, b->dev.B, RG_WAVE, sizeof(rgs::RgLds), 0, stream, b->model->dev_copy, launch_args, g1, g2, margin, out_dev);
 }
 
 int rg_post_args_size(void) { return (int)sizeof(rg_post_args); }
diff --git a/robogym_amd/csrc/rg_kernel.h b/robogym_amd/csrc/rg_kernel.h
--- a/robogym_amd/csrc/rg_kernel.h
+++ b/robogym_amd/csrc/rg_kernel.h
@@ -14,7 +14,7 @@
 typedef const __attribute__((address_space(4))) RgModelDev& RgM;
 #endif
 #ifdef RG_FINE_PROF
-#define RG_NPROF 56
+#define RG_NPROF 64
 #else
 #define RG_NPROF 24
 #endif
@@ -319,6 +319,7 @@
           union {
             short tlist[RG_TLIST];
             struct { float c_dist[RG_MAXCON], c_pos[RG_MAXCON * 3], c_normal[RG_MAXCON * 3]; };
+            float hand[RG_HANDQ * 7];
           };
         };
       };
@@ -335,6 +336,8 @@
   };
   float prof[RG_NPROF];
 };
+static_assert(sizeof(((RgLds*)0)->hand) <= sizeof(float) * RG_MAXCON * 7, "the hand-over slice lives inside the raw contacts' storage");
+static_assert(RG_SENSORS || offsetof(RgLds, prof) <= (RG_MAXCON <= 24 ? 12800 : 20480), "LDS launch image grew past its granule budget");
 static inline size_t rg_lds_launch_bytes(bool profiling) { return profiling ? sizeof(RgLds) : offsetof(RgLds, prof); }
 
 #ifdef RG_EMUL
@@ -657,21 +660,21 @@
   iu = iu < 0 ? 0 : (iu > RG_CELLN - 1 ? RG_CELLN - 1 : iu); iv = iv < 0 ? 0 : (iv > RG_CELLN - 1 ? RG_CELLN - 1 : iv);
   return ((2 * axis + (mj < 0 ? 1 : 0)) * RG_CELLN + iu) * RG_CELLN + iv;
 }
-template <int G> __device__ __forceinline__ void scan_cell(const int* celladr, const rgf4* cellblk, const rgf4* cellovf, v3 ld, float& bv, int& bi, v3& bp) {
+template <int G, int W> __device__ __forceinline__ void scan_cell(const int* celladr, const rgf4* cellblk, const rgf4* cellovf, v3 ld, float& bv, int& bi, v3& bp) {
+  static_assert(W == 4 || W == 8, "inline records per support cell");
+  constexpr int S = G < W ? G : W, NL = W / S;
   int cell = dir_cell(ld), l = LANE & (G - 1);
   int e = celladr[cell];
-  if (G >= 4) {
-    rgf4 a = cellblk[4 * cell + (l & 3)];
-    float da = vdot(ld, a);
-    if (da > bv) { bv = da; bi = __builtin_bit_cast(int, a.w); bp = mk3(a.x, a.y, a.z); }
-  } else {
-    rgf4 a = cellblk[4 * cell + 2 * (l & 1)], a2 = cellblk[4 * cell + 2 * (l & 1) + 1];
-    float da = vdot(ld, a), da2 = vdot(ld, a2);
-    if (da > bv) { bv = da; bi = __builtin_bit_cast(int, a.w); bp = mk3(a.x, a.y, a.z); }
-    int i2 = __builtin_bit_cast(int, a2.w);
-    if (da2 > bv || (da2 == bv && i2 < bi)) { bv = da2; bi = i2; bp = mk3(a2.x, a2.y, a2.z); }
-  }
-  int cnt = (e & 255) - 4, last = cnt - 1;
+  const rgf4* blk = cellblk + W * cell + (l & (S - 1));
+  rgf4 r[NL];
+#pragma unroll
+  for (int k = 0; k < NL; k++) r[k] = blk[k * S];
+#pragma unroll
+  for (int k = 0; k < NL; k++) {
+    float d = vdot(ld, r[k]); int i = __builtin_bit_cast(int, r[k].w);
+    if (k == 0 ? d > bv : (d > bv || (d == bv && i < bi))) { bv = d; bi = i; bp = mk3(r[k].x, r[k].y, r[k].z); }
+  }
+  int cnt = (e & 255) - W, last = cnt - 1;
   if (cnt > 0) {
     const rgf4* rec = cellovf + (e >> 8);
     for (int base = 0; base < cnt; base += 2 * G) {
@@ -684,8 +687,8 @@
     }
   }
 }
-template <int G> __device__ __forceinline__ void scan_hull(const MprEnv& E, const MprGeom& g, v3 ld, float& bv, int& bi, v3& bp) {
-  if (E.cells) scan_cell<G>(E.cell_adr + g.mesh * RG_NCELL, E.cell_blk + (size_t)g.mesh * (RG_NCELL * 4), E.cell_ovf, ld, bv, bi, bp);
+template <int G, int W> __device__ __forceinline__ void scan_hull(const MprEnv& E, const MprGeom& g, v3 ld, float& bv, int& bi, v3& bp) {
+  if (E.cells) scan_cell<G, W>(E.cell_adr + g.mesh * RG_NCELL, E.cell_blk + (size_t)g.mesh * (RG_NCELL * W), E.cell_ovf, ld, bv, bi, bp);
   else scan_verts<G>((const rgf4*)E.mesh_vert + g.vertadr, g.nvert, ld, bv, bi, bp);
 }
 template <int G> __device__ __forceinline__ v3 pick_vert(float bv, int bi, v3 bp) {
@@ -717,25 +720,25 @@
   }
   return lr;
 }
-template <int G> __device__ __forceinline__ v3 rg_support(const MprEnv& E, const MprGeom& g, v3 dir) {
+template <int G, int W> __device__ __forceinline__ v3 rg_support(const MprEnv& E, const MprGeom& g, v3 dir) {
   q4 gq = ldq(g.quat);
   v3 ld = qrotT(gq, dir), lr;
   if (g.type == RG_GEOM_MESH) {
     float bv = -3.0e38f; int bi = 0x7fffffff; v3 bp = mk3(0, 0, 0);
-    scan_hull<G>(E, g, ld, bv, bi, bp);
+    scan_hull<G, W>(E, g, ld, bv, bi, bp);
     lr = pick_vert<G>(bv, bi, bp) * g.vscale;
   } else lr = support_primitive(g, ld);
   lr = lr + ld * g.margin;
   return qrot(gq, lr) + g.pos;
 }
-template <int G> __device__ __forceinline__ void mpr_support(const MprEnv& E, const MprGeom& a, const MprGeom& b, v3 dir, SupPt& p) {
+template <int G, int W> __device__ __forceinline__ void mpr_support(const MprEnv& E, const MprGeom& a, const MprGeom& b, v3 dir, SupPt& p) {
   long long tt0 = E.prof ? rg_clock() : 0;
   q4 qa = ldq(a.quat), qb = ldq(b.quat);
   v3 la = qrotT(qa, dir), lb = qrotT(qb, dir * -1.0f), ra, rb;
   float av = -3.0e38f, bvv = -3.0e38f; int ai = 0x7fffffff, bi = 0x7fffffff; v3 ap = mk3(0, 0, 0), bp = mk3(0, 0, 0);
   bool am = a.type == RG_GEOM_MESH, bm = b.type == RG_GEOM_MESH;
-  if (am) scan_hull<G>(E, a, la, av, ai, ap);
-  if (bm) scan_hull<G>(E, b, lb, bvv, bi, bp);
+  if (am) scan_hull<G, W>(E, a, la, av, ai, ap);
+  if (bm) scan_hull<G, W>(E, b, lb, bvv, bi, bp);
   long long tt1 = E.prof ? rg_clock() : 0;
   ra = am ? pick_vert<G>(av, ai, ap) * a.vscale : support_primitive(a, la);
   rb = bm ? pick_vert<G>(bvv, bi, bp) * b.vscale : support_primitive(b, lb);
@@ -743,7 +746,18 @@
   v3 w2 = qrot(qb, rb + lb * b.margin) + b.pos;
   p.v = w1 - w2; p.s = w1 + w2;
   if (E.prof && LANE == 0) { long long tt2 = rg_clock(); E.prof[20] += 1.f; E.prof[21] += (float)(tt1 - tt0); E.prof[22] += (float)(tt2 - tt1); }
-}
+#ifdef RG_FINE_PROF
+  if (E.prof && LANE == __builtin_ctzll(__ballot(true))) E.prof[61] += (float)(rg_clock() - tt1);
+#endif
+}
+#ifdef RG_FINE_PROF
+template <int W> __device__ __forceinline__ bool mpr_cell_overflow(const MprEnv& E, const MprGeom& a, const MprGeom& b, v3 dir) {
+  bool o = false;
+  if (a.type == RG_GEOM_MESH) o = o || (E.cell_adr[a.mesh * RG_NCELL + dir_cell(qrotT(ldq(a.quat), dir))] & 255) > W;
+  if (b.type == RG_GEOM_MESH) o = o || (E.cell_adr[b.mesh * RG_NCELL + dir_cell(qrotT(ldq(b.quat), dir * -1.0f))] & 255) > W;
+  return o;
+}
+#endif
 #define MPR_EPS 1.0e-7f
 __device__ __forceinline__ bool mz(float x) { return fabsf(x) < MPR_EPS * 1e-3f; }
 __device__ __forceinline__ v3 portal_dir(const SupPt& p1, const SupPt& p2, const SupPt& p3) { return normalized(cross(p2.v - p1.v, p3.v - p1.v)); }
@@ -799,7 +813,15 @@
   pos = p0.s * (b0 * inv) + p1.s * (b1 * inv) + p2.s * (b2 * inv) + p3.s * (b3 * inv);
 }
 enum { MPR_DONE = 0, MPR_FIRST, MPR_SECOND, MPR_DISCOVER, MPR_REFINE, MPR_PENETR };
-template <int G> __device__ __forceinline__ bool rg_mpr(const MprEnv& E, const MprGeom& A, const MprGeom& B, int max_iter, float tol, float& depth, v3& dir_out, v3& pos, v3& sep, bool active) {
+__device__ __forceinline__ void mpr_first_dir(const SupPt& p0, const SupPt& p1, v3& dir, int& state, bool& result, float& depth, v3& dir_out, v3& pos) {
+  dir = cross(p0.v, p1.v);
+  if (dot(dir, dir) < 1e-30f) {
+    pos = p1.s * 0.5f; result = true; state = MPR_DONE;
+    if (dot(p1.v, p1.v) < 1e-30f) { depth = 0; dir_out = mk3(0, 0, 0); }
+    else { depth = norm(p1.v); dir_out = p1.v * (1.0f / depth); }
+  } else { dir = normalized(dir); state = MPR_SECOND; }
+}
+template <int G, int W> __device__ __forceinline__ bool rg_mpr(const MprEnv& E, const MprGeom& A, const MprGeom& B, int max_iter, float tol, float& depth, v3& dir_out, v3& pos, v3& sep, bool active, bool handed, const SupPt& hp) {
   SupPt p0, p1, p2, p3;
   p0.v = p0.s = p1.v = p1.s = p2.v = p2.s = p3.v = p3.s = mk3(0, 0, 0);
   int state = active ? MPR_FIRST : MPR_DONE, guard = 0;
@@ -810,24 +832,30 @@
     p0.s = A.pos + B.pos; p0.v = A.pos - B.pos;
     if (mz(p0.v.x) && mz(p0.v.y) && mz(p0.v.z)) p0.v.x += 1e-6f;
     dir = normalized(p0.v * -1.0f);
-  }
+    if (handed) { p1 = hp; mpr_first_dir(p0, p1, dir, state, result, depth, dir_out, pos); }
+  }
+#ifdef RG_FINE_PROF
+  const long long tl0 = rg_clock();
+#endif
   while (__ballot(state != MPR_DONE)) {
     if (state == MPR_DONE) continue;
     SupPt q;
-    mpr_support<G>(E, A, B, dir, q);
+#ifdef RG_FINE_PROF
+    const bool pf = E.prof && LANE == __builtin_ctzll(__ballot(true));
+    const unsigned long long povf = __ballot(E.cells && mpr_cell_overflow<W>(E, A, B, dir));
+    if (pf) { E.prof[58] += 1.f; E.prof[59] += povf ? 1.f : 0.f; E.prof[63] += (float)(__popcll(__ballot(true)) / G); }
+    const long long tp0 = rg_clock();
+#endif
+    mpr_support<G, W>(E, A, B, dir, q);
+#ifdef RG_FINE_PROF
+    if (pf) E.prof[60] += (float)(rg_clock() - tp0);
+#endif
     float dq = dot(q.v, dir);
     bool to_refine = false;
     if (state == MPR_FIRST) {
       p1 = q;
       if (dq <= 0) { sep = dir; state = MPR_DONE; }
-      else {
-        dir = cross(p0.v, p1.v);
-        if (dot(dir, dir) < 1e-30f) {
-          pos = p1.s * 0.5f; result = true; state = MPR_DONE;
-          if (dot(p1.v, p1.v) < 1e-30f) { depth = 0; dir_out = mk3(0, 0, 0); }
-          else { depth = norm(p1.v); dir_out = p1.v * (1.0f / depth); }
-        } else { dir = normalized(dir); state = MPR_SECOND; }
-      }
+      else mpr_first_dir(p0, p1, dir, state, result, depth, dir_out, pos);
     } else if (state == MPR_SECOND) {
       p2 = q;
       if (dq <= 0) { sep = dir; state = MPR_DONE; }
@@ -869,7 +897,13 @@
       if (state != MPR_PENETR) { if (dot(dir, p1.v) >= 0) { state = MPR_PENETR; guard = 0; } else state = MPR_REFINE; }
     }
   }
+#ifdef RG_FINE_PROF
+  const long long tl1 = rg_clock();
+#endif
   if (finish) { mpr_result(E.plane_depth, p0, p1, p2, p3, dir, depth, dir_out, pos); result = true; }
+#ifdef RG_FINE_PROF
+  if (E.prof && LANE == 0) { E.prof[23] += 1.f; E.prof[55] += (float)(tl1 - tl0); E.prof[56] += (float)(rg_clock() - tl1); }
+#endif
   return result;
 }
 
@@ -1080,9 +1114,11 @@
   const float gscale = rg_prm(m, L)[RG_PRM_GEOM_SCALE];
   MprEnv E = rg_mpr_env(m, (float*)0, cells);
   const bool boxbox = !(L.flags & 16);
+  const bool handover = !(L.flags & 2048);
   for (int base = 0; base < ncand; base += RG_WAVE / G) {
     int ci = base + LANE / G;
-    bool keep = false; int p = 0;
+    bool keep = false, centre = false; int p = 0;
+    SupPt p1; p1.v = p1.s = mk3(0, 0, 0);
     if (ci < ncand) {
       p = s.cand[ci];
       MprGeom A, B; int dim; float margin;
@@ -1091,8 +1127,9 @@
         v3 c0 = A.pos - B.pos;
         if (mz(c0.x) && mz(c0.y) && mz(c0.z)) c0.x += 1e-6f;
         v3 dir = normalized(c0 * -1.0f);
-        if (sepdir) { rgf4 cd; const float* sp_ = (const float*)(sepdir + p); cd.x = RG_ROW_LD(sp_); cd.y = RG_ROW_LD(sp_ + 1); cd.z = RG_ROW_LD(sp_ + 2); cd.w = 0.f; if (cd.x * cd.x + cd.y * cd.y + cd.z * cd.z > 0.5f) dir = mk3(cd.x, cd.y, cd.z); }
-        SupPt p1; mpr_support<G>(E, A, B, dir, p1);
+        centre = true;
+        if (sepdir) { rgf4 cd; const float* sp_ = (const float*)(sepdir + p); cd.x = RG_ROW_LD(sp_); cd.y = RG_ROW_LD(sp_ + 1); cd.z = RG_ROW_LD(sp_ + 2); cd.w = 0.f; if (cd.x * cd.x + cd.y * cd.y + cd.z * cd.z > 0.5f) { dir = mk3(cd.x, cd.y, cd.z); centre = false; } }
+        mpr_support<G, RG_CELLW>(E, A, B, dir, p1);
         float d = dot(p1.v, dir);
         keep = d > 0;
         if (!keep && pairlb && (LANE & (G - 1)) == 0) RG_ROW_ST(pairlb + p, fmaxf(-d - 1e-6f, 0.f));
@@ -1105,6 +1142,7 @@
     if (lead) {
       int slot = cbase + __popcll(bal & ((1ull << LANE) - 1ull));
       if (slot < RG_MAXCAND2) s.cand2[slot] = p; else s.status |= RG_STATUS_CAND_FULL;
+      if (slot < RG_HANDQ) { float* h = s.hand + 7 * slot; st3(h, p1.v); st3(h + 3, p1.s); h[6] = (centre && handover) ? 1.f : 0.f; }
     }
     if (LANE == 0) { int n = cbase + __popcll(bal); s.ncand2 = n < RG_MAXCAND2 ? n : RG_MAXCAND2; }
     SYNC();
@@ -1122,14 +1160,30 @@
     int ci = base + LANE / G;
     bool hit = false;
     float depth = 0, margin = 0; v3 dir = mk3(0, 0, 0), pos = mk3(0, 0, 0); int p = 0, dim = 3;
-    bool active = ci < ncand2;
-    MprGeom A, B;
+    bool active = ci < ncand2, handed = false;
+    MprGeom A, B; SupPt hp; hp.v = hp.s = mk3(0, 0, 0);
+#ifdef RG_FINE_PROF
+    const long long tg0 = rg_clock();
+#endif
     if (active) {
       p = s.cand2[ci];
       rg_mpr_geoms(m, s, p, gscale, A, B, dim, margin);
-    }
+      if (base == 0 && ci < RG_HANDQ) { const float* h = s.hand + 7 * ci; handed = h[6] != 0.f; hp.v = ld3(h); hp.s = ld3(h + 3); }
+    }
+#ifdef RG_FINE_PROF
+    if (prof) {
+      const long long tg1 = rg_clock();
+      bool nocache = active && (LANE & (G - 1)) == 0;
+      if (nocache && sepdir) { const float* sp_ = (const float*)(sepdir + p); float cx = RG_ROW_LD(sp_), cy = RG_ROW_LD(sp_ + 1), cz = RG_ROW_LD(sp_ + 2); nocache = !(cx * cx + cy * cy + cz * cz > 0.5f); }
+      const int nn = __popcll(__ballot(nocache));
+      if (LANE == 0) { prof[54] += (float)(tg1 - tg0); prof[62] += (float)nn; }
+    }
+#endif
     v3 sep;
-    hit = rg_mpr<G>(E, A, B, m.mpr_iterations, m.mpr_tolerance, depth, dir, pos, sep, active);
+    hit = rg_mpr<G, RG_CELLW>(E, A, B, m.mpr_iterations, m.mpr_tolerance, depth, dir, pos, sep, active, handed, hp);
+#ifdef RG_FINE_PROF
+    const long long tc0 = rg_clock();
+#endif
     if (active) {
       if (sepdir && (LANE & (G - 1)) == 0) { rgf4 cd; cd.x = hit ? 0.f : sep.x; cd.y = hit ? 0.f : sep.y; cd.z = hit ? 0.f : sep.z; cd.w = 0.f; RG_SEPDIR_ST(sepdir + p, cd); }
       hit = hit && dot(dir, dir) > 0.25f;
@@ -1148,6 +1202,9 @@
     }
     if (LANE == 0) { int n = cbase + __popcll(bal); s.ncon = n < RG_MAXCON ? n : RG_MAXCON; }
     SYNC();
+#ifdef RG_FINE_PROF
+    if (prof && LANE == 0) prof[57] += (float)(rg_clock() - tc0);
+#endif
   }
 }
 __device__ __forceinline__ void rg_collision(RgCtx c, RgM m, RgLds& s, const float* P, float* prof, rgf4* sepdir, float* pairlb, bool cells) {
@@ -1271,7 +1328,7 @@
       }
     } else {
       B.pos = p2 - p1;
-      v3 sp = rg_support<64>(rg_mpr_env(m, (float*)0, false), B, n * -1.0f);
+      v3 sp = rg_support<64, RG_CELLW>(rg_mpr_env(m, (float*)0, false), B, n * -1.0f);
       float dist = dot(sp, n);
       if (dist <= margin) add_contact(s, p, dist, sp + p1 - n * (0.5f * dist), n, dim);
     }
@@ -2925,8 +2982,7 @@
 #endif
 
 #if !RG_ITEMS
-__global__ void __launch_bounds__(RG_WAVE) rg_mpr_pair_kernel(const RgModelDev* mp, RgLaunch launch, int g1, int g2, float margin, float* out) {
-  RG_MAKE_CTX();
+template <int G> __device__ __forceinline__ void rg_mpr_pair_body(RgCtx c, int g1, int g2, float margin, float* out) {
   RgM m = RG_M(c);
   RgLRef L = RG_L(c);
   RgLds& s = RG_S();
@@ -2941,14 +2997,22 @@
   A.mesh = B.mesh = -1; A.vertadr = B.vertadr = 0; A.nvert = B.nvert = 0;
   if (A.type == RG_GEOM_MESH) { A.mesh = m.geom_dataid[g1]; A.vertadr = m.mesh_vertadr[A.mesh]; A.nvert = m.mesh_vertnum[A.mesh]; }
   if (B.type == RG_GEOM_MESH) { B.mesh = m.geom_dataid[g2]; B.vertadr = m.mesh_vertadr[B.mesh]; B.nvert = m.mesh_vertnum[B.mesh]; }
-  MprEnv E = rg_mpr_env(m, (float*)0, true);
+  MprEnv E = rg_mpr_env(m, (float*)0, G == 64 || !(L.flags & 8));
   E.plane_depth = true;
   float depth = 0; v3 dir = mk3(0, 0, 0), pos = mk3(0, 0, 0);
-  v3 sep; bool hit = rg_mpr<64>(E, A, B, m.mpr_iterations, m.mpr_tolerance, depth, dir, pos, sep, true);
+  v3 sep; bool hit = rg_mpr<G, RG_CELLW>(E, A, B, m.mpr_iterations, m.mpr_tolerance, depth, dir, pos, sep, LANE < G, false, SupPt());
   if (LANE == 0) {
     float* o = out + 8 * (size_t)e;
     o[0] = hit ? 1.f : 0.f; o[1] = depth; o[2] = dir.x; o[3] = dir.y; o[4] = dir.z; o[5] = pos.x + p1.x; o[6] = pos.y + p1.y; o[7] = pos.z + p1.z;
   }
+}
+__global__ void __launch_bounds__(RG_WAVE) rg_mpr_pair_kernel(const RgModelDev* mp, RgLaunch launch, int g1, int g2, float margin, float* out) {
+  RG_MAKE_CTX();
+  rg_mpr_pair_body<64>(c, g1, g2, margin, out);
+}
+__global__ void __launch_bounds__(RG_WAVE) rg_mpr_pair_quad_kernel(const RgModelDev* mp, RgLaunch launch, int g1, int g2, float margin, float* out) {
+  RG_MAKE_CTX();
+  rg_mpr_pair_body<4>(c, g1, g2, margin, out);
 }
 
 #if RG_SETCONST
diff --git a/robogym_amd/csrc/rg_types.h b/robogym_amd/csrc/rg_types.h
--- a/robogym_amd/csrc/rg_types.h
+++ b/robogym_amd/csrc/rg_types.h
@@ -16,6 +16,7 @@
 #define RG_MAXNM 160
 #define RG_CELLN 8
 #define RG_NCELL (6 * RG_CELLN * RG_CELLN)
+#define RG_CELLW 8
 #define RG_LTDL_TRI_ROUNDS 12
 #define RG_LTDL_PAIR_ROUNDS 8
 #define RG_KINREC 20
@@ -24,6 +25,7 @@
 #define RG_PAIRREC 28
 #define RG_PAIR_SCALED1 (1 << 28)
 #define RG_PAIR_SCALED2 (1 << 29)
+#define RG_HANDQ 16
 #define RG_TLIST 320
 #define RG_MAXROW 64
 #define RG_W 14
```
